# pqh22/ProxyTransformation

Hardware: AMD Instinct MI355X
Metric: scenes/sec (100k pts, 256 clusters, 64 proxies) (higher is better)
Workload: dtype f32; 1 GPU; cfg2: N=100000 pts, gs=8->M'=256 kept clusters, L=64 text + V=196 image proxies, d=256, eval forward; scenes_per_gpu=4, img_feat_dtype=bf16, input_sets_rotated=3, streams=1, lanes=1 (one forward at a time), setup_forwards=32

## Files before the change

include/proxyt.h:

```cpp
#ifndef PROXYT_H_
#define PROXYT_H_

#include <stddef.h>
#include <stdint.h>

#ifdef __cplusplus
extern "C" {
#endif

#define PTX_ABI_VERSION 13

#define PTX_API __attribute__((visibility("default")))

#define PTX_OK          0
#define PTX_EINVAL     -1
#define PTX_ELAUNCH    -2
#define PTX_ENOSPACE   -3
#define PTX_ETIMEOUT   -4
#define PTX_EGATE      -5

typedef struct PtxShape {
    int32_t B;
    int32_t N;
    int32_t grid_size;
// ... 14 lines not shown
    float   ln_eps;
} PtxShape;

typedef struct PtxSlotMlp {
    const float *conv_w;
    const float *conv_b;
    const float *bn_w, *bn_b, *bn_mean, *bn_var;
} PtxSlotMlp;

typedef struct PtxBlock {
    const float *norm1_w, *norm1_b;
    const float *pb_bias;
    const float *pc_bias;
    const float *pr_bias;
    const float *qkv_w;
    const float *qkv_b;
    const float *pp_w, *pp_b;
    const float *proj_w, *proj_b;
    const float *norm2_w, *norm2_b;
    const float *fc1_w, *fc1_b;
    const float *fc2_w, *fc2_b;
    const float *out_norm_w, *out_norm_b;
} PtxBlock;

typedef struct PtxBn1d { const float *w, *b, *mean, *var; } PtxBn1d;

typedef struct PtxWeights {
    PtxSlotMlp   offset;
    const float *offset_map_w;
    PtxSlotMlp   encoder;
    const float *cm_w, *cm_b;
    const float *pos;
    const float *q_w, *q_b, *k_w, *k_b, *v_w, *v_b, *c_w, *c_b;
    const float *norm_img_w, *norm_img_b;
    PtxBlock     text;
    PtxBlock     img;
    const float *text_trans_w, *text_trans_b;
    const float *img_trans_w, *img_trans_b;
    PtxBn1d      text_trans_norm, img_trans_norm;
} PtxWeights;

PTX_API int         ptx_abi_version(void);
PTX_API const char *ptx_last_error(void);

typedef struct PtxContext PtxContext;
PTX_API int ptx_context_create(PtxContext **ctx);
PTX_API int ptx_context_destroy(PtxContext *ctx);
PTX_API int ptx_context_check(PtxContext *ctx);
PTX_API int ptx_context_sync_check(PtxContext *ctx);
PTX_API int ptx_context_gates(const PtxContext *ctx);

PTX_API int         ptx_kernel_count(void);
PTX_API const char *ptx_kernel_name(int kid);
PTX_API int         ptx_timing_select(int kid);
PTX_API int         ptx_timing_read(int *launches, float *total_ms);
PTX_API int         ptx_timing_every(int n);
PTX_API int         ptx_timing_select_mask(uint64_t mask);
PTX_API int         ptx_timing_read_sites(int *launches, float *total_ms, int n);

PTX_API size_t ptx_prep_bytes(const PtxShape *s);
PTX_API size_t ptx_workspace_bytes(const PtxShape *s);

PTX_API int ptx_workspace_init(const PtxShape *s, void *workspace, size_t ws_bytes, void *stream);

PTX_API int ptx_prepare(const PtxShape *s, const PtxWeights *w, const float *lin,
                void *prep, size_t prep_bytes, void *stream);


PTX_API int ptx_grid_centers(const float *points, int B, int N, const float *lin, int gs, float margin,
                     float *minmax, float *centers, void *workspace, size_t ws_bytes, void *stream);

PTX_API int ptx_ball_query(const float *centers, const float *points, int B, int M, int N, int K,
                   float radius, int32_t *idx, float *cluster, int32_t *pad_count, void *stream);

PTX_API int ptx_linear(const float *x, const float *w, const float *bias, const float *residual, float *y,
               int rows, int n_out, int n_in, int gelu, void *stream);
PTX_API int ptx_linear_ln_partials(const float *x, const float *w, const float *bias, const float *residual, float *y, float *lnp,
               int rows, int n_out, int n_in, void *stream);
PTX_API size_t ptx_ln_linear_scratch_bytes(int n_out, int n_in);
PTX_API int ptx_ln_linear(const float *x, const float *lnp, const float *w, const float *gamma, const float *beta,
               const float *bias, float eps, int gelu, float *y, void *scratch, size_t scratch_bytes,
               int rows, int n_out, int n_in, void *stream);
PTX_API int ptx_gemm_policy(int min_tiles_128);

PTX_API int ptx_offset_net(const PtxShape *s, const PtxWeights *w, const void *prep,
                   const float *centers_in, const float *cluster, const float *minmax,
                   float *centers_out, float *offsets_out, void *stream);

PTX_API int ptx_select_clusters(const PtxShape *s, const int32_t *idx, const float *centers,
                        const float *cluster, const int32_t *pad_count,
                        const int32_t *order_override,
                        int32_t *order, int32_t *picks, int32_t *keep,
                        float *kcenter, float *kcluster, int32_t *kidx, int32_t *drop_idx,
                        uint32_t *tag, void *stream);

PTX_API int ptx_pointnet(const PtxShape *s, const PtxWeights *w, const void *prep, const float *kcenter,
                 const float *kcluster, float *point_proxy, void *stream);

PTX_API int ptx_img_proxy(const PtxShape *s, const PtxWeights *w, const void *prep, const void *img_feat,
                  float *img_proxy, void *workspace, size_t ws_bytes, void *stream);

PTX_API int ptx_proxy_block(const PtxShape *s, const PtxWeights *w, const void *prep, int which,
                    const float *point_proxy, const float *proxy, int Lp, const uint8_t *mask,
                    float *head_out, float *guide, void *workspace, size_t ws_bytes, void *stream);

PTX_API int ptx_affine_scatter(const PtxShape *s, const float *points, const uint32_t *tag,
                       const float *kcenter, const float *translate, const float *transform,
                       float *new_points, void *stream);

PTX_API int ptx_affine_compact(const PtxShape *s, const float *points, const uint32_t *tag,
                       const float *kcenter, const float *translate, const float *transform,
                       float *out, int32_t *counts, void *workspace, size_t ws_bytes, void *stream);

PTX_API size_t ptx_proxy_attention_scratch_bytes(int B, int n, int Lp, int heads, int C, int impl);
PTX_API int ptx_proxy_attention(const float *qkv, const float *pt, const uint8_t *mask, float *out, float *scratch, int B, int n,
                        int Lp, int heads, int C, int impl, void *stream);

typedef struct PtxDebug {
    float *centers0, *cluster1, *offsets, *centers, *cluster2;
    int32_t *idx2, *pad_count, *order, *picks, *keep, *kidx, *drop_idx;
    float *kcenter, *kcluster, *point_proxy, *img_proxy, *text_guide, *img_guide;
    float *translate, *transform;
    uint32_t *tag;
} PtxDebug;

PTX_API int ptx_forward(PtxContext *ctx, const PtxShape *s, const PtxWeights *w, const void *prep, const float *lin,
                const float *points, const float *const *points_list, const float *text_feats,
                const uint8_t *text_mask, const void *img_feat, const int32_t *order_override,
                const float *centers_override,
                float *out, int32_t *counts, void *workspace, size_t ws_bytes,
                const PtxDebug *debug, void *stream);

typedef struct PtxForwardOpts {
    const uint32_t *bbox_enc;
    int32_t compute_dtype;
    int32_t reserved[5];
} PtxForwardOpts;
PTX_API int ptx_forward_ex(PtxContext *ctx, const PtxShape *s, const PtxWeights *w, const void *prep, const float *lin,
                   const float *points, const float *const *points_list, const float *text_feats,
                   const uint8_t *text_mask, const void *img_feat, const int32_t *order_override,
                   const float *centers_override,
                   float *out, int32_t *counts, void *workspace, size_t ws_bytes,
                   const PtxDebug *debug, const PtxForwardOpts *opts, void *stream);

PTX_API int ptx_wait_counts(const int32_t *counts_host, int B, int64_t timeout_us);

PTX_API size_t ptx_ingest_workspace_bytes(int V, int H, int W);
PTX_API int ptx_ingest_index(const void *depth, int depth_dtype, int V, int H, int W, void *workspace, size_t ws_bytes,
                     int32_t *view_counts, void *stream);
PTX_API int ptx_ingest_gather(const void *depth, int depth_dtype, float depth_shift, int V, int H, int W, const float *inv_intrinsic,
                      const float *lu, const int32_t *piv, const int64_t *sel, int N, const float *aug, float *points,
                      uint32_t *bbox_enc, int32_t *status, const void *workspace, size_t ws_bytes, void *stream);

#define PTX_DRAW_EMPTY 1
#define PTX_DRAW_MAX_VIEWS 4096
PTX_API int ptx_ingest_draw(int V, int H, int W, int per_view, int N, uint64_t key, const void *workspace, size_t ws_bytes,
                    int64_t *sel, int32_t *status, void *stream);

#define PTX_VOX_BROKEN 0x7fffffff
PTX_API size_t ptx_voxel_workspace_bytes(int B, int Ncap);
PTX_API int ptx_voxelize(const float *points, const int32_t *counts, int B, int Ncap, float voxel_size, int32_t *coords,
                 float *feats, int32_t *inverse, int32_t *nvox_overflow, void *workspace, size_t ws_bytes, void *stream);
PTX_API int ptx_voxelize_ex(const float *points, const int32_t *counts, int B, int Ncap, float voxel_size, int32_t *coords,
                    float *feats, int32_t *inverse, int32_t *nvox_overflow, int32_t *scene_end, void *workspace, size_t ws_bytes,
                    void *stream);
PTX_API int ptx_voxelize_rep(const float *points, const int32_t *counts, int B, int Ncap, float voxel_size, int32_t *coords,
// ... 178 lines not shown
```

proxytransformation_amd/_abi.py:

```python
from __future__ import annotations

import ctypes as C
import os
from typing import Optional

_HERE = os.path.dirname(os.path.abspath(__file__))
LIB_PATH = os.path.join(_HERE, "libproxyt_hip.so")
ABI_VERSION = 13

c_float_p = C.c_void_p


class PtxShape(C.Structure):
    _fields_ = [(n, C.c_int32) for n in
                ("B", "N", "grid_size", "K", "Mt", "Mk", "L", "V", "C", "heads", "hidden",
                 "in_dim", "hw", "img_dtype")] + \
               [(n, C.c_float) for n in ("radius", "margin", "bn_eps", "ln_eps")]


class PtxSlotMlp(C.Structure):
    _fields_ = [(n, C.c_void_p) for n in ("conv_w", "conv_b", "bn_w", "bn_b", "bn_mean", "bn_var")]


class PtxBlock(C.Structure):
# ... 26 lines not shown
class PtxDebug(C.Structure):
    _fields_ = [(n, C.c_void_p) for n in DEBUG_FIELDS]


TB_PARAMS = ("ln1_w", "ln1_b", "pb", "pc", "pr", "qkv_w", "qkv_b", "pp_w", "pp_b", "proj_w", "proj_b", "ln2_w", "ln2_b",
             "fc1_w", "fc1_b", "fc2_w", "fc2_b", "ln3_w", "ln3_b", "head_w", "head_b", "bn_w", "bn_b")


class PtxTrainBlock(C.Structure):
    _fields_ = [(n, C.c_int32) for n in ("B", "n", "L", "C", "H", "heads", "s", "nout", "compute_dtype")] + \
               [(n, C.c_float) for n in ("eps1", "eps2", "eps3", "bn_eps", "bn_momentum", "p_attn", "p_drop", "p_path")] + \
               [("seed", C.c_uint64 * 6), ("x", C.c_void_p), ("proxy", C.c_void_p), ("mask", C.c_void_p),
                ("param", C.c_void_p * len(TB_PARAMS)), ("bn_run_mean", C.c_void_p), ("bn_run_var", C.c_void_p),
                ("out", C.c_void_p), ("save", C.c_void_p), ("save_floats", C.c_size_t), ("tmp", C.c_void_p),
                ("tmp_floats", C.c_size_t), ("dout", C.c_void_p), ("dx", C.c_void_p), ("dproxy", C.c_void_p),
                ("grad", C.c_void_p * len(TB_PARAMS)), ("dx_add", C.c_void_p)]


class PtxTrainImgPool(C.Structure):
    _fields_ = [(n, C.c_int32) for n in ("nimg", "Cin", "hw", "C", "heads", "img_dtype")] + \
               [(n, C.c_void_p) for n in ("img", "wc", "bc", "pos", "wq", "bq", "wk", "bk", "wv", "bv", "o", "save")] + \
               [("save_floats", C.c_size_t), ("tmp", C.c_void_p), ("tmp_floats", C.c_size_t)] + \
               [(n, C.c_void_p) for n in ("dout", "dimg", "dwc", "dbc", "dpos", "dwq", "dbq", "dwk", "dbk", "dwv", "dbv")] + \
               [(n, C.c_void_p) for n in ("cw", "cb", "lnw", "lnb")] + [("ln_eps", C.c_float)] + \
               [(n, C.c_void_p) for n in ("proxy", "dproxy", "dcw", "dcb", "dlnw", "dlnb")]


class PtxTrainSlotNet(C.Structure):
    _fields_ = [(n, C.c_void_p) for n in ("conv_w", "conv_b", "bn_w", "bn_b", "run_mean", "run_var")] + \
               [("eps", C.c_float), ("momentum", C.c_float), ("W", C.c_int32)]


TS_NGRAD = 9 + 13 + 2 * len(TB_PARAMS)
TS_IP0, TS_TB0, TS_IB0 = 9, 9 + 13, 9 + 13 + len(TB_PARAMS)


class PtxTrainStepLayout(C.Structure):
    _fields_ = [(n, C.c_size_t) for n in ("arena_fwd_bytes", "arena_bwd_bytes", "grads_floats", "idx2", "order", "picks", "keep", "kidx",
                                           "drop_idx", "centers", "translate", "transform", "point_proxy", "img_proxy", "kcenter",
                                           "opos")] + [("grad_off", C.c_int64 * TS_NGRAD)]


class PtxTrainStep(C.Structure):
    _fields_ = [("shape", PtxShape), ("points", C.c_void_p), ("lin", C.c_void_p), ("centers_override", C.c_void_p),
                ("order_override", C.c_void_p), ("text_feats", C.c_void_p), ("text_mask", C.c_void_p),
                ("off", PtxTrainSlotNet), ("enc", PtxTrainSlotNet), ("map_w", C.c_void_p),
                ("ip", PtxTrainImgPool), ("tb", PtxTrainBlock), ("ib", PtxTrainBlock),
                ("ws", C.c_void_p), ("ws_bytes", C.c_size_t), ("out", C.c_void_p), ("counts_host", C.c_void_p),
                ("arena_fwd", C.c_void_p), ("arena_fwd_bytes", C.c_size_t),
                ("side_stream", C.c_void_p), ("ev_fork", C.c_void_p), ("ev_join", C.c_void_p), ("ev_pp", C.c_void_p),
                ("ev_counts", C.c_void_p), ("blocks_apart", C.c_int32),
                ("douts", C.c_void_p), ("g_kcenter", C.c_void_p), ("g_translate", C.c_void_p), ("g_transform", C.c_void_p),
                ("arena_bwd", C.c_void_p), ("arena_bwd_bytes", C.c_size_t), ("grads", C.c_void_p), ("grads_floats", C.c_size_t),
                ("dtext", C.c_void_p), ("dimg", C.c_void_p)]


class PtxForwardOpts(C.Structure):
    _fields_ = [("bbox_enc", C.c_void_p), ("compute_dtype", C.c_int32), ("reserved", C.c_int32 * 5)]


_P, _I, _F, _Z = C.c_void_p, C.c_int, C.c_float, C.c_size_t
_SH, _W = C.POINTER(PtxShape), C.POINTER(PtxWeights)
SIGNATURES = {
    "ptx_abi_version": (C.c_int, []),
    "ptx_last_error": (C.c_char_p, []),
    "ptx_kernel_count": (C.c_int, []),
    "ptx_kernel_name": (C.c_char_p, [_I]),
    "ptx_timing_select": (_I, [_I]),
    "ptx_timing_every": (_I, [_I]),
    "ptx_timing_read": (_I, [C.POINTER(C.c_int), C.POINTER(C.c_float)]),
    "ptx_timing_select_mask": (_I, [C.c_uint64]),
    "ptx_timing_read_sites": (_I, [C.POINTER(C.c_int), C.POINTER(C.c_float), _I]),
    "ptx_prep_bytes": (_Z, [_SH]),
    "ptx_workspace_bytes": (_Z, [_SH]),
    "ptx_workspace_init": (_I, [_SH, _P, _Z, _P]),
    "ptx_prepare": (_I, [_SH, _W, _P, _P, _Z, _P]),
    "ptx_grid_centers": (_I, [_P, _I, _I, _P, _I, _F, _P, _P, _P, _Z, _P]),
    "ptx_ball_query": (_I, [_P, _P, _I, _I, _I, _I, _F, _P, _P, _P, _P]),
    "ptx_linear": (_I, [_P, _P, _P, _P, _P, _I, _I, _I, _I, _P]),
    "ptx_linear_ln_partials": (_I, [_P, _P, _P, _P, _P, _P, _I, _I, _I, _P]),
    "ptx_ln_linear_scratch_bytes": (_Z, [_I, _I]),
    "ptx_ln_linear": (_I, [_P, _P, _P, _P, _P, _P, _F, _I, _P, _P, _Z, _I, _I, _I, _P]),
    "ptx_gemm_policy": (_I, [_I]),
    "ptx_offset_net": (_I, [_SH, _W, _P, _P, _P, _P, _P, _P, _P]),
    "ptx_select_clusters": (_I, [_SH] + [_P] * 14),
    "ptx_pointnet": (_I, [_SH, _W, _P, _P, _P, _P, _P]),
    "ptx_img_proxy": (_I, [_SH, _W, _P, _P, _P, _P, _Z, _P]),
    "ptx_proxy_block": (_I, [_SH, _W, _P, _I, _P, _P, _I, _P, _P, _P, _P, _Z, _P]),
    "ptx_affine_scatter": (_I, [_SH, _P, _P, _P, _P, _P, _P, _P]),
    "ptx_affine_compact": (_I, [_SH, _P, _P, _P, _P, _P, _P, _P, _P, _Z, _P]),
    "ptx_wait_counts": (_I, [_P, _I, C.c_int64]),
    "ptx_context_create": (_I, [C.POINTER(C.c_void_p)]),
    "ptx_context_destroy": (_I, [_P]),
    "ptx_context_check": (_I, [_P]),
    "ptx_context_sync_check": (_I, [_P]),
    "ptx_context_gates": (_I, [_P]),
    "ptx_forward": (_I, [_P, _SH, _W, _P, _P, _P, _P, _P, _P, _P, _P, _P, _P, _P, _P, _Z,
                         C.POINTER(PtxDebug), _P]),
}

_L, _U64 = C.c_long, C.c_uint64
SIGNATURES.update({
    "ptx_forward_ex": (_I, [_P, _SH, _W, _P, _P, _P, _P, _P, _P, _P, _P, _P, _P, _P, _P, _Z,
                            C.POINTER(PtxDebug), C.POINTER(PtxForwardOpts), _P]),
    "ptx_proxy_attention": (_I, [_P, _P, _P, _P, _P, _I, _I, _I, _I, _I, _I, _P]),
    "ptx_proxy_attention_scratch_bytes": (_Z, [_I, _I, _I, _I, _I, _I]),
    "ptx_ingest_workspace_bytes": (_Z, [_I, _I, _I]),
    "ptx_ingest_index": (_I, [_P, _I, _I, _I, _I, _P, _Z, _P, _P]),
    "ptx_ingest_gather": (_I, [_P, _I, _F, _I, _I, _I, _P, _P, _P, _P, _I, _P, _P, _P, _P, _P, _Z, _P]),
    "ptx_ingest_draw": (_I, [_I, _I, _I, _I, _I, _U64, _P, _Z, _P, _P, _P]),
    "ptx_voxel_workspace_bytes": (_Z, [_I, _I]),
    "ptx_voxelize": (_I, [_P, _P, _I, _I, _F, _P, _P, _P, _P, _P, _Z, _P]),
    "ptx_voxelize_ex": (_I, [_P, _P, _I, _I, _F, _P, _P, _P, _P, _P, _P, _Z, _P]),
    "ptx_voxelize_rep": (_I, [_P, _P, _I, _I, _F, _P, _P, _P, _P, _P, _P, _P, _Z, _P]),
    "ptx_voxel_features_bwd": (_I, [_P, _I, _P, _P, _P, _I, _I, _P, _P]),
    "ptx_voxel_coarsen": (_I, [_P, _P, _I, _I, _F, _P, _P, _P, _P, _P, _Z, _P]),
    "ptx_point_sample_workspace_bytes": (_Z, [_I, _I, _I, _I]),
    "ptx_point_sample_prepare": (_I, [_P, _I, _I, _I, _I, _I, _P, _Z, _P]),
    "ptx_point_sample": (_I, [_P, _I, _P, _I, _I, _I, _I, _I, _P, _P, _F, _F, _F, _F, _I, _F, _F, _F, _I, _P, _P, _P, _Z, _P]),
    "ptx_point_sample_bwd_workspace_bytes": (_Z, [_I, _I, _I, _I, _I]),
    "ptx_point_sample_bwd": (_I, [_P, _I, _P, _P, _I, _I, _I, _I, _P, _P, _F, _F, _F, _F, _I, _F, _F, _F, _I, _P, _I, _P, _Z, _P]),
    "ptx_op_gemm": (_I, [_P, _P, _P, _I, _I, _I, _L, _L, _L, _L, _L, _L, _I, _I, _L, _L, _L, _L, _L, _L, _I, _I, _F, _I, _I, _L, _P]),
    "ptx_op_transpose": (_I, [_P, _I, _I, _P, _P]),
    "ptx_op_colsum": (_I, [_P, _P, _I, _I, _I, _F, _I, _P, _P, _I, _P]),
    "ptx_op_eltwise": (_I, [_I, _P, _P, _F, _L, _I, _P, _P]),
    "ptx_op_dropout": (_I, [_P, _L, _L, _F, _U64, _P, _P]),
    "ptx_op_layernorm_fwd": (_I, [_P, _P, _P, _P, _I, _I, _I, _F, _P, _P, _P]),
    "ptx_op_layernorm_bwd": (_I, [_P, _P, _P, _P, _I, _I, _P, _P, _P]),
    "ptx_op_bn_stats": (_I, [_P, _P, _I, _L, _F, _F, _P, _P, _P, _P]),
    "ptx_op_bn_apply": (_I, [_P, _P, _P, _P, _L, _I, _I, _P, _P]),
    "ptx_op_bn_bwd_prep": (_I, [_P, _P, _P, _P, _L, _I, _I, _P, _P, _P]),
    "ptx_op_bn_bwd_dx": (_I, [_P, _P, _P, _P, _P, _P, _L, _I, _P, _P]),
    "ptx_op_softmax_fwd": (_I, [_P, _P, _L, _I, _L, _P, _P]),
    "ptx_op_softmax_bwd": (_I, [_P, _P, _P, _L, _I, _L, _P, _P]),
    "ptx_op_slot_inputs": (_I, [_P, _P, _P, _L, _I, _P, _P, _P]),
    "ptx_op_slot_inputs_bwd": (_I, [_P, _P, _L, _I, _P, _P]),
    "ptx_op_slot_pool": (_I, [_P, _L, _I, _I, _I, _P, _P, _P]),
    "ptx_op_slot_pool_bwd": (_I, [_P, _P, _L, _I, _I, _I, _P, _P]),
    "ptx_op_slotnet_scratch_bytes": (_Z, [_I]),
    "ptx_op_slotnet_fwd": (_I, [_P, _P, _L, _I, _I, _P, _P, _P, _P, _F, _F, _P, _P, _I, _P, _P, _P, _P, _P, _Z, _P]),
    "ptx_op_slotnet_bwd": (_I, [_P, _P, _L, _I, _I, _P, _P, _P, _P, _P, _I, _P, _P, _P, _P, _P, _P, _P, _Z, _P]),
    "ptx_op_offset_apply": (_I, [_P, _P, _P, _L, _I, _F, _P, _P, _P]),
    "ptx_op_slotbias_fwd": (_I, [_P, _P, _P, _I, _I, _I, _P, _P]),
    "ptx_op_slotbias_bwd": (_I, [_P, _I, _I, _I, _P, _P, _P, _P]),
    "ptx_op_keep_rows": (_I, [_P, _P, _I, _I, _I, _I, _P, _P]),
    "ptx_op_rows_gather": (_I, [_P, _P, _L, _I, _P, _P]),
    "ptx_op_rows_scatter": (_I, [_P, _P, _L, _I, _P, _P]),
    "ptx_op_out_positions": (_I, [_P, _I, _I, _P, _P, _P, _P]),
    "ptx_op_affine_bwd": (_I, [_P, _P, _P, _P, _P, _P, _I, _I, _I, _I, _P, _P, _P, _P]),
    "ptx_op_affine_bwd_list": (_I, [_P, _P, _P, _P, _P, _P, _I, _I, _I, _I, _P, _P, _P, _P]),
    "ptx_op_tokens_finish": (_I, [_P, _P, _I, _I, _I, _P]),
    "ptx_op_tokens_finish_bwd": (_I, [_P, _I, _I, _I, _P]),
    "ptx_train_block_sizes": (_I, [C.POINTER(PtxTrainBlock), C.POINTER(_Z), C.POINTER(_Z), C.POINTER(_Z)]),
    "ptx_train_block_fwd": (_I, [C.POINTER(PtxTrainBlock), _P]),
    "ptx_train_block_bwd": (_I, [C.POINTER(PtxTrainBlock), _P]),
    "ptx_train_imgpool_sizes": (_I, [C.POINTER(PtxTrainImgPool), C.POINTER(_Z), C.POINTER(_Z), C.POINTER(_Z)]),
    "ptx_train_imgpool_fwd": (_I, [C.POINTER(PtxTrainImgPool), _P]),
    "ptx_train_imgpool_bwd": (_I, [C.POINTER(PtxTrainImgPool), _P]),
    "ptx_train_step_layout": (_I, [C.POINTER(PtxTrainStep), C.POINTER(PtxTrainStepLayout)]),
    "ptx_train_step_fwd": (_I, [C.POINTER(PtxTrainStep), _P]),
    "ptx_train_step_bwd": (_I, [C.POINTER(PtxTrainStep), _P]),
    "ptx_op_head_bwd_tmp_floats": (_Z, [_I, _I, _I]),
    "ptx_op_head_bwd": (_I, [_P, _P, _P, _P, _I, _I, _I, _P, _P, _P, _Z, _P]),
    "ptx_train_attn_tmp_floats": (_Z, [_I, _I, _I, _I, _I]),
    "ptx_train_attn_fwd": (_I, [_P, _P, _P, _I, _I, _I, _I, _I, _F, _U64, _P, _P, _P, _P, _P]),
    "ptx_train_attn_bwd": (_I, [_P, _P, _P, _I, _I, _I, _I, _I, _F, _U64, _P, _P, _P, _P, _P, _P, _P, _Z, _P]),
# ... 37 lines not shown
```

proxytransformation_amd/csrc/api.hip:

```cpp
#include <atomic>
#include <chrono>
#include <cmath>
#include <cstdlib>
#include <cstring>
#include <mutex>
#include <utility>
#include <vector>

#include "common.h"

namespace ptx {

static thread_local char g_err[512] = "";

void set_error(const char *fmt, ...)
{
    va_list ap;
    va_start(ap, fmt);
    vsnprintf(g_err, sizeof(g_err), fmt, ap);
    va_end(ap);
}

static const char *const kKernelNames[] = {
    "k_minmax", "k_cluster", "k_select", "k_tags",
// ... 306 lines not shown

template <typename T>
static inline T *at(void *base, size_t off) { return reinterpret_cast<T *>(static_cast<char *>(base) + off); }

__global__ void k_signal(uint32_t *flag, uint32_t seq)
{
    if (threadIdx.x == 0) __hip_atomic_store(flag, seq, __ATOMIC_RELAXED, __HIP_MEMORY_SCOPE_AGENT);
}
__global__ void k_gate(GateRef g)
{
    if (threadIdx.x == 0) gate_wait(g);
}

static GateRef gate_ref(const PtxContext *c, int word, uint32_t seq, uint32_t site, bool probe = false)
{
    const uint64_t ticks = probe ? c->probe_ticks : ((site == 2 || site == 7) ? 2 * c->gate_ticks : c->gate_ticks);
    return GateRef{c->gate + word, seq, c->gate_err, probe ? nullptr : c->gate + 48, ticks, site, probe ? 0 : c->gate_trap};
}

static int gate_check(PtxContext *c)
{
    if (c->gate_err == nullptr) return PTX_OK;
    const uint32_t e = *reinterpret_cast<volatile uint32_t *>(c->gate_err);
    if (e == 0u) return PTX_OK;
    static const char *const site_name[] = {"?", "fork (clustering stream waiting for the caller's stream)",
                                            "join (caller's stream waiting for the other chain)", "probe, fork direction",
                                            "probe, join direction", "?", "slot tags' fork (tag stream waiting for the selection)",
                                            "slot tags' join (caller's stream waiting for the tags)"};
    const unsigned site = (e >> 24) & 0x7fu;
    c->gates_on = false;
    *reinterpret_cast<volatile uint32_t *>(c->gate_err) = 0u;
    (void)hipStreamSynchronize(c->st);
    if (c->have_last) (void)hipStreamSynchronize(c->last_st);
    (void)hipMemset(c->gate + 48, 0, 4);
    set_error("stream gate timed out at the %s of forward #%u: the two chains of that forward were not ordered and its outputs "
              "were set to NaN; this context now orders its streams with events (PTX_GATE=0 selects them from the start)",
              site_name[site < 8 ? site : 0], e & 0xffffffu);
    return PTX_EGATE;
}

static int gate_probe_pair(PtxContext *c, hipStream_t waiter, hipStream_t releaser, int word, uint32_t site, bool *ok)
{
    const uint32_t seq = ++c->gate_seq;
    hipLaunchKernelGGL(k_gate, dim3(1), dim3(64), 0, waiter, gate_ref(c, word, seq, site, true));
    PTX_LAUNCHED("k_gate[probe]");
    hipLaunchKernelGGL(k_signal, dim3(1), dim3(64), 0, releaser, c->gate + word, seq);
    PTX_LAUNCHED("k_signal[probe]");
    PTX_HIP(hipStreamSynchronize(waiter));
    PTX_HIP(hipStreamSynchronize(releaser));
    *ok = *reinterpret_cast<volatile uint32_t *>(c->gate_err) == 0u;
    *reinterpret_cast<volatile uint32_t *>(c->gate_err) = 0u;
    return PTX_OK;
}
static int gate_probe(PtxContext *c, hipStream_t st)
{
    c->probed = true; c->probed_st = st; c->lo_ok = false;
    if (!c->gates_on) return PTX_OK;
    PTX_HIP(hipStreamSynchronize(st));
    PTX_HIP(hipStreamSynchronize(c->st));
    PTX_HIP(hipStreamSynchronize(c->lo));
    bool fork_ok = false, join_ok = false, t1 = false, t2 = false;
    PTX_TRY(gate_probe_pair(c, c->st, st, 40, 3, &fork_ok));
    PTX_TRY(gate_probe_pair(c, st, c->st, 44, 4, &join_ok));
    if (!fork_ok || !join_ok) { c->gates_on = false; return PTX_OK; }
    PTX_TRY(gate_probe_pair(c, c->lo, c->st, 40, 3, &t1));
    PTX_TRY(gate_probe_pair(c, st, c->lo, 44, 4, &t2));
    c->lo_ok = t1 && t2;
    return PTX_OK;
}

static int run_img_proxy(const PtxShape &s, const PtxWeights &w, const float *prep, const void *img,
                         float *img_proxy, void *ws, hipStream_t st, int phase = 0, bool need_ln = true,
                         int i0 = 0, int ni = -1, uint32_t *gate = nullptr, uint32_t gate_seq = 0)
{
    const PrepLayout P = prep_layout(s);
    const WsLayout L = ws_layout(s);
    const int C = s.C, hd = P.hd, nall = s.B * s.V, nimg = ni < 0 ? nall : ni;
    float *fm = at<float>(ws, L.fm) + (size_t)i0 * s.in_dim, *qkv0 = at<float>(ws, L.qkv0) + (size_t)i0 * 3 * C;
    float *we = at<float>(ws, L.we) + (size_t)i0 * s.heads * P.KT1, *gbuf = at<float>(ws, L.gbuf) + (size_t)i0 * s.heads * P.KT2p;
    float *obuf = at<float>(ws, L.obuf) + (size_t)i0 * C, *cbuf = at<float>(ws, L.cbuf) + (size_t)i0 * C;
    if (img_proxy) img_proxy += (size_t)i0 * C;
    const int dt = s.img_dtype;
    img = static_cast<const char *>(img) + (size_t)i0 * s.in_dim * s.hw * (dt == 0 ? 4 : 2);
    float *Gs = nullptr, *E = nullptr, *ML = nullptr;
    const int EW = P.KT2p - s.in_dim;
    const bool pooled32 = img_pool32_supported(dt, s.in_dim, s.hw, s.heads);
    const bool pooled = pooled32 || img_pool_supported(dt, s.in_dim, s.hw, s.heads);
    if (pooled) {
        img_pool_layout(at<float>(ws, L.pool), nall, s.in_dim, EW, &Gs, &E, &ML);
        Gs += (size_t)i0 * 2 * s.heads * s.in_dim; E += (size_t)i0 * s.heads * EW; ML += (size_t)i0 * s.heads * 5;
    }
    if (phase != 2) PTX_TIMED(KID_IMG_MEAN, st, launch_img_mean(img, dt, nimg, s.in_dim, s.hw, fm, st, gate, gate_seq));
    if (phase == 1) return PTX_OK;
    const bool chained = hd == 32 && nimg < 4096;
    {
        GemmBatch g{}; g.n = 1;
        g.p[0] = GemmProb{fm, prep + P.w3, qkv0, prep + P.b3, nullptr, nullptr, nullptr,
                          nimg, 3 * C, s.in_dim, s.in_dim, s.in_dim, 3 * C, 0, 0, 0, EPI_NONE};
        if (chained) {
            g.p[0].w2 = prep + P.t1; g.p[0].c2 = we; g.p[0].n2 = P.KT1; g.p[0].ldc2 = s.heads * P.KT1;
            g.p[0].chain_tiles = s.heads; g.p[0].w2_stride = (long)P.KT1 * hd; g.p[0].c2_stride = P.KT1;
        }
        PTX_TIMED(KID_IMG_QKV0, st, launch_gemm(g, st));
    }
    if (!chained) {
        for (int h0 = 0; h0 < s.heads; h0 += kMaxGroups) {
            GemmBatch g{}; g.n = std::min(kMaxGroups, s.heads - h0);
            for (int h = h0; h < h0 + g.n; ++h)
                g.p[h - h0] = GemmProb{qkv0 + h * hd, prep + P.t1 + (size_t)h * P.KT1 * hd, we + (size_t)h * P.KT1,
                                       nullptr, nullptr, nullptr, nullptr, nimg, P.KT1, hd, 3 * C, hd,
                                       s.heads * P.KT1, 0, 0, 0, EPI_NONE};
            PTX_TIMED(KID_IMG_WE, st, launch_gemm(g, st));
        }
    }
    if (pooled32) {
        PTX_TIMED_EXT(KID_IMG_SCORES, st, launch_img_pool32(static_cast<const float *>(img), we, qkv0, nimg, s.in_dim, s.hw, C, P.KT1, EW,
                                                        attn_scale(hd), Gs, E, ML, st));
    } else if (pooled) {
        PTX_TIMED_EXT(KID_IMG_SCORES, st, launch_img_pool(img, dt, we, qkv0, nimg, s.in_dim, s.hw, C, P.KT1,
                                                      EW, attn_scale(hd), Gs, E, ML, st));
    } else {
        PTX_TIMED(KID_IMG_SCORES, st, launch_img_scores(img, dt, we, qkv0, nimg, s.in_dim, s.hw, s.heads, C, P.KT1,
                                                        P.KT2p, attn_scale(hd), gbuf, st));
        PTX_TIMED(KID_IMG_GATHER, st, launch_img_gather(img, dt, nimg, s.in_dim, s.hw, s.heads, P.KT2p, gbuf, st));
    }
    for (int h0 = 0; h0 < s.heads; h0 += kMaxGroups) {
        GemmBatch g{}; g.n = std::min(kMaxGroups, s.heads - h0);
        for (int h = h0; h < h0 + g.n; ++h) {
            GemmProb &gp = g.p[h - h0];
            gp = GemmProb{gbuf + (size_t)h * P.KT2p, prep + P.t2 + (size_t)h * hd * P.KT2p, obuf + h * hd,
                          w.v_b + h * hd, nullptr, gbuf + (size_t)h * P.KT2p + s.in_dim,
                          qkv0 + 2 * C + h * hd, nimg, hd, P.KT2p, s.heads * P.KT2p, P.KT2p, C,
                          0, s.heads * P.KT2p, 3 * C, EPI_NONE};
            if (pooled) {
                gp.A = nullptr; gp.rs = nullptr;
                gp.pg = Gs + (size_t)h * s.in_dim; gp.ldg = 2 * s.heads * s.in_dim; gp.gslab = s.heads * s.in_dim;
                gp.pe = E + (size_t)h * EW; gp.lde = s.heads * EW;
                gp.pml = ML + (size_t)h * 5; gp.ldml = s.heads * 5;
                gp.kg = s.in_dim;
            }
        }
        PTX_TIMED(KID_IMG_O, st, launch_gemm(g, st));
    }
    {
        GemmBatch g{}; g.n = 1;
        g.p[0] = GemmProb{obuf, w.c_w, cbuf, w.c_b, nullptr, nullptr, nullptr,
                          nimg, C, C, C, C, C, 0, 0, 0, EPI_NONE};
        g.p[0].lnp_out = at<float>(ws, L.lnp_img) + (size_t)i0 * (C / 32) * 2;
        PTX_TIMED(KID_IMG_C, st, launch_gemm(g, st));
    }
    if (need_ln) {
        LnBatch lb{}; lb.n = 1; lb.C = C; lb.eps = s.ln_eps;
        lb.p[0] = LnProb{cbuf, img_proxy, w.norm_img_w, w.norm_img_b, nullptr, nimg, 1};
        PTX_TIMED(KID_IMG_LN, st, launch_ln_rows(lb, st));
    }
    return PTX_OK;
}

struct Branch {
    const PtxBlock *blk; const float *x_in; const float *proxy; int Lp; const uint8_t *mask;
    const float *head_w, *head_b, *head_ab; int nout; float *head_out; float *guide; int slot;
    bool late_proxy;
    const float *proxy_lnp, *pp_gw, *pp_gc;
    const float *fc1_gw, *fc1_gc;
    const float *prep;
};

static bool fused_attn_pays(const PtxShape &s, const Branch *br, int nb)
{
    (void)br;
    const long wgs = (long)s.B * s.heads * nb;
    return s.Mk <= 256 || wgs >= 96;
}

static int run_blocks(const PtxShape &s, const Branch *br, int nb, const float *point_proxy, void *ws,
                      hipStream_t st, int phase = 0, int cd = 0, GateRef *join = nullptr, GateRef *tags_join = nullptr,
                      bool skip_qkv = false)
{
    const WsLayout L = ws_layout(s);
    const int C = s.C, R = s.B * s.Mk;
    {
        GemmBatch g{}; g.n = 0;
        for (int i = 0; i < nb; ++i) {
            const int sl = br[i].slot;
            if (phase != 2 && phase != 3 && phase != 4 && !skip_qkv)
                g.p[g.n++] = GemmProb{br[i].x_in, br[i].blk->qkv_w, at<float>(ws, L.qkv[sl]), br[i].blk->qkv_b,
                                      nullptr, nullptr, nullptr, R, 3 * C, C, C, C, 3 * C, 0, 0, 0, EPI_NONE};
            const bool now = phase == 0 || (phase == 1 && !br[i].late_proxy) || ((phase == 2 || phase == 3) && br[i].late_proxy);
            if (now && phase != 4) {
                GemmProb &q = g.p[g.n++];
                q = GemmProb{br[i].proxy, br[i].blk->pp_w, at<float>(ws, L.pt[sl]), br[i].blk->pp_b,
                             nullptr, nullptr, nullptr, s.B * br[i].Lp, C, C, C, C, C, 0, 0, 0, EPI_NONE};
                if (br[i].proxy_lnp != nullptr) {
                    q.W = br[i].pp_gw; q.bias = nullptr;
                    q.lnp_in = br[i].proxy_lnp; q.ln_c = br[i].pp_gc;
                    q.ln_parts = C / 32; q.ln_C = C; q.ln_eps = s.ln_eps;
                }
            }
        }
        if (g.n > 0 && (phase == 2 || phase == 1) && join != nullptr && join->flag != nullptr) { g.tail_gate = *join; join->flag = nullptr; }
        if (g.n > 0) PTX_TIMED(phase == 2 || phase == 3 ? KID_BLK_PP : KID_BLK_QKV, st, launch_gemm(g, st, cd));
        if (phase == 1 || phase == 3) return PTX_OK;
    }
    FAttnBatch fa{}; fa.nb = nb; fa.B = s.B; fa.heads = s.heads; fa.hd = C / s.heads; fa.n = s.Mk; fa.C = C;
    fa.scale = attn_scale(C / s.heads); fa.compute_dtype = cd;
    fa.split = fattn_split_for(s.B, s.heads); fa.part = at<float>(ws, L.fa_part); fa.tickets = at<int>(ws, L.fa_ticket);
    for (int i = 0; i < nb; ++i) {
        const int sl = br[i].slot;
        fa.p[i] = FAttnProb{at<float>(ws, L.qkv[sl]), at<float>(ws, L.pt[sl]), br[i].mask, at<float>(ws, L.ao[sl]), br[i].Lp};
    }
    const bool fused = fused_attn_supported(fa) && (cd == 1 || fused_attn_pays(s, br, nb));
    if (fused) PTX_TIMED(KID_BLK_ATTN_F, st, launch_proxy_attn(fa, st));
    AttnBatch a{}; a.n = nb; a.B = s.B; a.heads = s.heads; a.hd = C / s.heads; a.scale = attn_scale(C / s.heads);
    for (int i = 0; i < nb && !fused; ++i) {
        const int sl = br[i].slot;
        float *qkv = at<float>(ws, L.qkv[sl]);
        a.p[i] = AttnProb{at<float>(ws, L.pt[sl]), qkv + C, qkv + 2 * C, at<float>(ws, L.pv[sl]), nullptr,
                          br[i].Lp, s.Mk, C, 3 * C, 3 * C, C,
                          (long)br[i].Lp * C, (long)s.Mk * 3 * C, (long)s.Mk * 3 * C, (long)br[i].Lp * C};
    }
    if (!fused) PTX_TIMED(KID_BLK_ATTN_A, st, launch_attn32(a, st));
    for (int i = 0; i < nb && !fused; ++i) {
// ... 245 lines not shown
                void *stream)
{
    (void)lin;
    PTX_REQUIRE(s && w && prep, "ptx_prepare: null argument");
    PTX_TRY(validate_shape(*s));
    if (prep_bytes < prep_layout(*s).total * sizeof(float)) { set_error("prep buffer too small"); return PTX_ENOSPACE; }
    return run_prepare(*s, *w, static_cast<float *>(prep), static_cast<hipStream_t>(stream));
}

int ptx_grid_centers(const float *points, int B, int N, const float *lin, int gs, float margin,
                     float *minmax, float *centers, void *workspace, size_t ws_bytes, void *stream)
{
    PTX_REQUIRE(points && lin && minmax && centers && workspace, "ptx_grid_centers: null argument");
    PTX_REQUIRE(ws_bytes >= (size_t)B * 6 * 4, "ptx_grid_centers: workspace needs %d bytes", B * 24);
    hipStream_t st = static_cast<hipStream_t>(stream);
    uint32_t *enc = static_cast<uint32_t *>(workspace);
    PTX_HIP(hipMemsetAsync(enc, 0, (size_t)B * 6 * 4, st));
    ScenePts sp;
    PTX_TRY(make_scene_pts(points, nullptr, B, N, &sp));
    PTX_TRY(launch_minmax(sp, B, N, enc, st));
    return launch_ball_query(nullptr, enc, lin, gs, margin, minmax, centers, sp, B, gs * gs * gs, N, 0,
                             0.0f, nullptr, nullptr, nullptr, st);
}

int ptx_ball_query(const float *centers, const float *points, int B, int M, int N, int K, float radius,
                   int32_t *idx, float *cluster, int32_t *pad_count, void *stream)
{
    PTX_REQUIRE(centers && points && idx && cluster, "ptx_ball_query: null argument");
    PTX_REQUIRE(B >= 1 && M >= 1 && N >= 1 && K >= 1, "ptx_ball_query: B=%d M=%d N=%d K=%d", B, M, N, K);
    ScenePts sp;
    PTX_TRY(make_scene_pts(points, nullptr, B, N, &sp));
    return launch_ball_query(centers, nullptr, nullptr, 0, 0.0f, nullptr, nullptr, sp, B, M, N, K, radius,
                             idx, cluster, pad_count, static_cast<hipStream_t>(stream));
}

int ptx_linear(const float *x, const float *w, const float *bias, const float *residual, float *y,
               int rows, int n_out, int n_in, int gelu, void *stream)
{
    PTX_REQUIRE(x && w && y, "ptx_linear: null argument");
    PTX_REQUIRE(rows >= 1 && n_out >= 1 && n_in >= 4, "ptx_linear: rows=%d n_out=%d n_in=%d", rows, n_out, n_in);
    GemmBatch g{}; g.n = 1;
    g.p[0] = GemmProb{x, w, y, bias, residual, nullptr, nullptr, rows, n_out, n_in, n_in, n_in, n_out, n_out, 0, 0,
                      gelu ? EPI_GELU : EPI_NONE};
    return launch_gemm(g, static_cast<hipStream_t>(stream));
}

int ptx_linear_ln_partials(const float *x, const float *w, const float *bias, const float *residual, float *y, float *lnp,
                           int rows, int n_out, int n_in, void *stream)
{
    PTX_REQUIRE(x && w && y && lnp, "ptx_linear_ln_partials: null argument");
    PTX_REQUIRE(rows >= 1 && n_out >= 1 && n_in >= 4, "ptx_linear_ln_partials: rows=%d n_out=%d n_in=%d", rows, n_out, n_in);
    GemmBatch g{}; g.n = 1;
    g.p[0] = GemmProb{x, w, y, bias, residual, nullptr, nullptr, rows, n_out, n_in, n_in, n_in, n_out, n_out, 0, 0, EPI_NONE};
    g.p[0].lnp_out = lnp;
    return launch_gemm(g, static_cast<hipStream_t>(stream));
}

size_t ptx_ln_linear_scratch_bytes(int n_out, int n_in)
{
    return n_out >= 1 && n_in >= 1 ? ((size_t)n_out * n_in + (size_t)n_out) * sizeof(float) : 0;
}

int ptx_ln_linear(const float *x, const float *lnp, const float *w, const float *gamma, const float *beta, const float *bias,
                  float eps, int gelu, float *y, void *scratch, size_t scratch_bytes, int rows, int n_out, int n_in, void *stream)
{
    PTX_REQUIRE(x && lnp && w && gamma && beta && y && scratch, "ptx_ln_linear: null argument");
    PTX_REQUIRE(rows >= 1 && n_out >= 1, "ptx_ln_linear: rows=%d n_out=%d", rows, n_out);
    PTX_REQUIRE(n_in >= 32 && n_in % 32 == 0 && n_in <= 512, "ptx_ln_linear: n_in=%d must be a multiple of 32, at most 512", n_in);
    PTX_REQUIRE(eps > 0.0f, "ptx_ln_linear: eps=%g", (double)eps);
    PTX_REQUIRE((reinterpret_cast<uintptr_t>(scratch) & 15) == 0 && scratch_bytes >= ptx_ln_linear_scratch_bytes(n_out, n_in),
                "ptx_ln_linear: scratch of %zu bytes (16-byte aligned) needed", ptx_ln_linear_scratch_bytes(n_out, n_in));
    hipStream_t st = static_cast<hipStream_t>(stream);
    float *wg = static_cast<float *>(scratch), *cv = wg + (size_t)n_out * n_in;
    PTX_TRY(launch_prep_lnfold(w, gamma, beta, bias, n_out, n_in, wg, cv, st));
    GemmBatch g{}; g.n = 1;
    g.p[0] = GemmProb{x, wg, y, nullptr, nullptr, nullptr, nullptr, rows, n_out, n_in, n_in, n_in, n_out, 0, 0, 0,
                      gelu ? EPI_GELU : EPI_NONE};
    g.p[0].lnp_in = lnp; g.p[0].ln_c = cv;
    g.p[0].ln_parts = n_in / 32; g.p[0].ln_C = n_in; g.p[0].ln_eps = eps;
    return launch_gemm(g, st);
}

int ptx_gemm_policy(int min_tiles_128) { return gemm_policy(min_tiles_128); }

int ptx_offset_net(const PtxShape *s, const PtxWeights *w, const void *prep, const float *centers_in,
                   const float *cluster, const float *minmax, float *centers_out, float *offsets_out,
                   void *stream)
{
    PTX_REQUIRE(s && w && prep && centers_in && cluster && minmax && centers_out, "ptx_offset_net: null argument");
    PTX_TRY(validate_shape(*s));
    const PrepLayout P = prep_layout(*s);
    const int M = s->grid_size * s->grid_size * s->grid_size;
    return launch_offset_net(static_cast<const float *>(prep) + P.off_ab, w->offset, w->offset_map_w, centers_in,
                             cluster, minmax, s->B * M, M, s->K, s->margin, centers_out, offsets_out,
                             static_cast<hipStream_t>(stream));
}

int ptx_select_clusters(const PtxShape *s, const int32_t *idx, const float *centers, const float *cluster,
                        const int32_t *pad_count, const int32_t *order_override, int32_t *order,
                        int32_t *picks, int32_t *keep, float *kcenter, float *kcluster, int32_t *kidx,
                        int32_t *drop_idx, uint32_t *tag, void *stream)
{
    PTX_REQUIRE(s && idx && centers && cluster && pad_count && order && picks && keep && kcenter && kcluster &&
                kidx && drop_idx, "ptx_select_clusters: null argument");
    PTX_TRY(validate_shape(*s));
    return launch_select(*s, idx, centers, cluster, pad_count, order_override, order, picks, keep, kcenter,
                         kcluster, kidx, drop_idx, tag, static_cast<hipStream_t>(stream));
}

int ptx_pointnet(const PtxShape *s, const PtxWeights *w, const void *prep, const float *kcenter,
                 const float *kcluster, float *point_proxy, void *stream)
{
    PTX_REQUIRE(s && w && prep && kcenter && kcluster && point_proxy, "ptx_pointnet: null argument");
    PTX_TRY(validate_shape(*s));
    const PrepLayout P = prep_layout(*s);
    return launch_pointnet(static_cast<const float *>(prep) + P.enc_ab, w->encoder, kcenter, kcluster,
                           s->B * s->Mk, s->Mk, s->K, s->C, point_proxy, nullptr, nullptr, nullptr, nullptr, nullptr,
                           nullptr, s->ln_eps, nullptr, 0, static_cast<hipStream_t>(stream));
}

int ptx_img_proxy(const PtxShape *s, const PtxWeights *w, const void *prep, const void *img_feat,
                  float *img_proxy, void *workspace, size_t ws_bytes, void *stream)
{
    PTX_REQUIRE(w && prep && img_feat && img_proxy, "ptx_img_proxy: null argument");
    PTX_TRY(check_bufs(s, workspace, ws_bytes));
    return run_img_proxy(*s, *w, static_cast<const float *>(prep), img_feat, img_proxy, workspace,
                         static_cast<hipStream_t>(stream));
}

int ptx_proxy_block(const PtxShape *s, const PtxWeights *w, const void *prep, int which,
                    const float *point_proxy, const float *proxy, int Lp, const uint8_t *mask,
                    float *head_out, float *guide, void *workspace, size_t ws_bytes, void *stream)
{
    PTX_REQUIRE(w && prep && point_proxy && proxy && head_out, "ptx_proxy_block: null argument");
    PTX_REQUIRE(which == 0 || which == 1, "ptx_proxy_block: which=%d", which);
    PTX_TRY(check_bufs(s, workspace, ws_bytes));
    PTX_REQUIRE(Lp >= 1 && Lp <= (s->L > s->V ? s->L : s->V), "ptx_proxy_block: Lp=%d exceeds max(L,V)", Lp);
    hipStream_t st = static_cast<hipStream_t>(stream);
    const PrepLayout P = prep_layout(*s);
    const WsLayout L = ws_layout(*s);
    const float *pf = static_cast<const float *>(prep);
    const PtxBlock &blk = which == 0 ? w->text : w->img;
    float *x_in = at<float>(workspace, L.x_in[which]);
    LnBatch lb{}; lb.n = 1; lb.C = s->C; lb.eps = s->ln_eps;
    lb.p[0] = LnProb{point_proxy, x_in, blk.norm1_w, blk.norm1_b, pf + (which == 0 ? P.posb_t : P.posb_i),
                     s->B * s->Mk, s->Mk};
    PTX_TRY(launch_ln_rows(lb, st));
    Branch br = make_branch(*s, *w, pf, which, x_in, proxy, Lp, mask, head_out, guide);
    return run_blocks(*s, &br, 1, point_proxy, workspace, st);
}

size_t ptx_proxy_attention_scratch_bytes(int B, int n, int Lp, int heads, int C, int impl)
{
    if (B < 1 || n < 1 || Lp < 1 || heads < 1 || C < heads) return 0;
    if (impl == 3) return 256 + (size_t)B * heads * 4 + (size_t)B * heads * kFaMaxSplit * n * kFaPartRow * sizeof(float);
    return (size_t)B * Lp * C * sizeof(float);
}

int ptx_proxy_attention(const float *qkv, const float *pt, const uint8_t *mask, float *out, float *scratch, int B, int n,
                        int Lp, int heads, int C, int impl, void *stream)
{
    PTX_REQUIRE(qkv && pt && out, "ptx_proxy_attention: null argument");
    PTX_REQUIRE(B >= 1 && n >= 1 && Lp >= 1 && heads >= 1 && C >= heads && C % heads == 0, "ptx_proxy_attention: B=%d n=%d Lp=%d heads=%d C=%d", B, n, Lp, heads, C);
    PTX_REQUIRE(impl >= 0 && impl <= 3, "ptx_proxy_attention: impl=%d", impl);
    hipStream_t st = static_cast<hipStream_t>(stream);
    const int hd = C / heads;
// ... 108 lines not shown
        PTX_HIP(hipEventRecord(side->fork, st));
        PTX_HIP(hipStreamWaitEvent(side->st, side->fork, 0));
    }
    float *img_proxy = at<float>(ws, L.img_proxy);
#ifdef PTX_TEST_HOOKS
    static const char *const fault = getenv("PTX_GATE_FAULT");
#else
    constexpr const char *fault = nullptr;
#endif
    const bool fault_fork = gated && fault && fault[0] == 'f', fault_join = gated && fault && fault[0] == 'j';
    auto launch_gate = [&](int kid, hipStream_t s_, const GateRef &g) -> int {
        hipLaunchKernelGGL(k_gate, dim3(1), dim3(64), 0, s_, g);
        PTX_LAUNCHED("k_gate");
        (void)kid;
        return PTX_OK;
    };
    if (gated) {
        const uint32_t seq = ++side->gate_seq;
        PTX_TRY(run_img_proxy(S, *w, pf, img_feat, img_proxy, ws, is, 1, true, 0, -1, fault_fork ? nullptr : side->gate, seq));
        PTX_TIMED(KID_GATE_FORK, cs, launch_gate(KID_GATE_FORK, cs, gate_ref(side, 0, seq, 1)));
    } else
    if (!img_late) PTX_TRY(run_img_proxy(S, *w, pf, img_feat, img_proxy, ws, is, 1));

    uint32_t *mm_ws = at<uint32_t>(ws, L.mm_enc), *tag = at<uint32_t>(ws, L.tag);
    const uint32_t *mm_enc = bbox_in ? bbox_in : mm_ws;
    const bool dbg = debug != nullptr;
    float *centers0 = dbg && debug->centers0 ? at<float>(ws, L.centers0) : nullptr;
    float *cluster1 = dbg && debug->cluster1 ? at<float>(ws, L.cluster1) : nullptr;
    float *offsets = dbg && debug->offsets ? at<float>(ws, L.offsets) : nullptr;
    float *centers = at<float>(ws, L.centers), *cluster2 = at<float>(ws, L.cluster2);
    int32_t *idx2 = at<int32_t>(ws, L.idx2), *pad_count = at<int32_t>(ws, L.pad_count);
    if (!bbox_in) PTX_TIMED(KID_MINMAX, cs, launch_minmax(sp, B, S.N, mm_ws, cs));
    const bool early = lc.early;
    const bool fork_ext = !capturing && (img_late || early);
    const bool cgate = cluster_on_caller && side->gates_on && side->lo_ok && !capturing;
    if (cgate) ++side->gate_seq;
    const bool fault_cjoin = cgate && fault && fault[0] == 'j', fault_ctags = cgate && fault && fault[0] == 't';
    const bool cg_join_select = cgate && early;
    const bool cg_join_qkv = cgate && !early;
    GateRef cjoin = (cg_join_select || cg_join_qkv) ? gate_ref(side, 52, side->gate_seq, 2) : GateRef{};
    PTX_TIMED(KID_CLUSTER, cs, launch_cluster(S, mm_enc, lin, sp, pf + P.off_ab, w->offset, w->offset_map_w,
                                              centers_override, nullptr, centers0, cluster1, offsets, centers, idx2,
                                              cluster2, pad_count, cs, fork_ext ? side->early_a : nullptr));

    if (img_late) {
        if (!fork_ext) PTX_HIP(hipEventRecord(side->fork, st));
        PTX_HIP(hipStreamWaitEvent(side->st, fork_ext ? side->early_a : side->fork, 0));
        PTX_TRY(run_img_proxy(S, *w, pf, img_feat, img_proxy, ws, is, 1));
    }
    float *point_proxy = at<float>(ws, L.point_proxy);
    float *xin_t = at<float>(ws, L.x_in[0]), *xin_i = at<float>(ws, L.x_in[1]);
    float *translate = at<float>(ws, L.head[0]), *transform = at<float>(ws, L.head[1]);
    float *guide_t = (debug && debug->text_guide) ? at<float>(ws, L.guide[0]) : nullptr;
    float *guide_i = (debug && debug->img_guide) ? at<float>(ws, L.guide[1]) : nullptr;
    Branch br[2] = {make_branch(S, *w, pf, 0, xin_t, text_feats, S.L, text_mask, translate, guide_t),
                    make_branch(S, *w, pf, 1, xin_i, at<float>(ws, L.cbuf), S.V, nullptr, transform, guide_i)};
    br[1].proxy_lnp = at<float>(ws, L.lnp_img);
    if (early) {
        if (!fork_ext) PTX_HIP(hipEventRecord(side->early_a, cs));
        PTX_HIP(hipStreamWaitEvent(side->lo, side->early_a, 0));
        float *pp_all = at<float>(ws, L.pp_all), *xa_t = at<float>(ws, L.xln_all[0]), *xa_i = at<float>(ws, L.xln_all[1]);
        int32_t *order_e = at<int32_t>(ws, L.order_e);
        PTX_TRY(launch_order(S, pad_count, order_override, order_e, side->lo));
        PTX_TRY(launch_pointnet(pf + P.enc_ab, w->encoder, centers, cluster2, B * S.Mt, S.Mt, K, S.C, pp_all, &w->text, &w->img, nullptr,
                                nullptr, xa_t, xa_i, S.ln_eps, order_e, M, side->lo, nullptr, 0, true));
        GemmBatch g{}; g.n = 2;
        g.p[0] = GemmProb{xa_t, w->text.qkv_w, at<float>(ws, L.g_all[0]), nullptr, nullptr, nullptr, nullptr, B * S.Mt, 3 * S.C, S.C, S.C, S.C,
                          3 * S.C, 0, 0, 0, EPI_NONE};
        g.p[1] = GemmProb{xa_i, w->img.qkv_w, at<float>(ws, L.g_all[1]), nullptr, nullptr, nullptr, nullptr, B * S.Mt, 3 * S.C, S.C, S.C, S.C,
                          3 * S.C, 0, 0, 0, EPI_NONE};
        PTX_TRY(launch_gemm(g, side->lo, compute_dtype));
        PTX_TRY(run_blocks(S, br, 2, point_proxy, ws, side->lo, 1, compute_dtype, nullptr, nullptr, true));
    }

    int32_t *order = at<int32_t>(ws, L.order), *picks = at<int32_t>(ws, L.picks), *keep = at<int32_t>(ws, L.keep);
    float *kcenter = at<float>(ws, L.kcenter);
    float *kcluster = dbg && debug->kcluster ? at<float>(ws, L.kcluster) : nullptr;
    int32_t *kidx = dbg && debug->kidx ? at<int32_t>(ws, L.kidx) : nullptr;
    int32_t *drop_idx = dbg && debug->drop_idx ? at<int32_t>(ws, L.drop_idx) : nullptr;
    int32_t *ksrc = at<int32_t>(ws, L.ksrc);
    const bool ext_event = !capturing;
    const bool tags_gated = gated && side->lo_ok && (lf.v[3] >= 0 ? lf.v[3] != 0 : est_image < 1.6 * est_cluster);
    const bool tags_tail = !cluster_on_caller && !tags_gated;
    PTX_TIMED(KID_SELECT, cs, launch_select_order(S, centers, pad_count, order_override, order, picks, keep, kcenter,
                                                  ksrc, bbox_in ? nullptr : mm_ws, cs, cluster_on_caller, ext_event && !tags_tail ? side->aux : nullptr,
                                                  cg_join_select ? &cjoin : nullptr));
    int32_t *tile_counts = at<int32_t>(ws, L.tile_counts);
    hipStream_t ts = tags_tail ? cs : side->lo;
    const bool slots_first = !cluster_on_caller && !tags_tail;
    auto enqueue_tags = [&]() -> int {
        if (tags_gated) {
            PTX_TIMED(KID_GATE_TAGS, ts, launch_gate(KID_GATE_TAGS, ts, gate_ref(side, 36, side->gate_seq, 6)));
        } else if (!tags_tail) {
            if (!ext_event) PTX_HIP(hipEventRecord(side->aux, cs));
            PTX_HIP(hipStreamWaitEvent(ts, side->aux, 0));
        }
        if (kcluster || kidx || drop_idx)
            PTX_TRY(launch_select_slots(S, idx2, cluster2, order, picks, keep, kcluster, kidx, drop_idx, nullptr, ts));
        PTX_TIMED(KID_TAGS, ts, launch_tags(S, idx2, order, picks, ksrc, tag, tile_counts, counts, at<int32_t>(ws, L.scene_acc), ts));
        if (tags_gated) {
            auto sig = [&]() -> int {
                hipLaunchKernelGGL(k_signal, dim3(1), dim3(64), 0, ts, side->gate + 38, side->gate_seq);
                PTX_LAUNCHED("k_signal[tags]");
                return PTX_OK;
            };
            PTX_TIMED(KID_SIGNAL_TAGS, ts, sig());
        } else if (cgate) {
            if (!fault_ctags) {
                hipLaunchKernelGGL(k_signal, dim3(1), dim3(64), 0, ts, side->gate + 56, side->gate_seq);
                PTX_LAUNCHED("k_signal[ctags]");
            }
        } else if (!tags_tail) PTX_HIP(hipEventRecord(side->tags, ts));
        return PTX_OK;
    };
    if (slots_first) PTX_TRY(enqueue_tags());

    const bool want_img_proxy = debug != nullptr && debug->img_proxy != nullptr;
    PTX_TRY(run_img_proxy(S, *w, pf, img_feat, img_proxy, ws, is, 2, want_img_proxy));

    bool joined_early = false;
    if (early) {
        const float *const gsrc[2] = {at<float>(ws, L.g_all[0]), at<float>(ws, L.g_all[1])};
        const float *const tb[2] = {pf + P.qkvb[0], pf + P.qkvb[1]};
        float *const qk[2] = {at<float>(ws, L.qkv[0]), at<float>(ws, L.qkv[1])};
        {
            PTX_TRY(run_blocks(S, br, 2, point_proxy, ws, is, 3, compute_dtype));
            PTX_HIP(hipEventRecord(side->join, is));
            PTX_HIP(hipStreamWaitEvent(side->lo, side->join, 0));
            joined_early = true;
        }
        if (cg_join_select) {
            if (!fault_cjoin) {
                hipLaunchKernelGGL(k_signal, dim3(1), dim3(64), 0, side->lo, side->gate + 52, side->gate_seq);
                PTX_LAUNCHED("k_signal[cjoin]");
            }
        } else {
            PTX_HIP(hipEventRecord(side->early_b, side->lo));
            PTX_HIP(hipStreamWaitEvent(cs, side->early_b, 0));
        }
        PTX_TIMED(KID_POINTNET, cs, launch_qkv_gather(at<float>(ws, L.pp_all), gsrc, tb, keep, B, S.Mt, S.Mk, S.C, point_proxy, qk, cs));
    } else
    PTX_TIMED(KID_POINTNET, cs, launch_pointnet(pf + P.enc_ab, w->encoder, kcenter, cluster2, B * S.Mk, S.Mk, K,
                                                S.C, point_proxy, &w->text, &w->img, pf + P.posb_t, pf + P.posb_i, xin_t,
                                                xin_i, S.ln_eps, ksrc, M, cs, tags_gated ? side->gate + 36 : nullptr, side->gate_seq));
    if (!slots_first && !tags_tail) PTX_TRY(enqueue_tags());

    if (!early) PTX_TRY(run_blocks(S, br, 2, point_proxy, ws, cs, 1, compute_dtype, cg_join_qkv ? &cjoin : nullptr));
    if (cg_join_qkv && cjoin.flag != nullptr) {
        set_error("ptx_forward: the join gate was not attached to the qkv launch");
        return PTX_ELAUNCH;
    }
    if (tags_tail) PTX_TRY(enqueue_tags());
    const bool pp_early = cluster_on_caller;
    GateRef join{};
    if (gated) {
        auto launch_signal = [&]() -> int {
            hipLaunchKernelGGL(k_signal, dim3(1), dim3(64), 0, cs, side->gate + 32, side->gate_seq);
            PTX_LAUNCHED("k_signal");
            return PTX_OK;
        };
        if (!fault_join) PTX_TIMED(KID_SIGNAL_JOIN, cs, launch_signal());
        join = gate_ref(side, 32, side->gate_seq, 2);
    } else {
    if (!cluster_on_caller) PTX_HIP(hipEventRecord(side->join, cs));
    if (pp_early && !joined_early) PTX_TRY(run_blocks(S, br, 2, point_proxy, ws, is, 3, compute_dtype));
    if (cg_join_qkv) {
        if (!fault_cjoin) {
            hipLaunchKernelGGL(k_signal, dim3(1), dim3(64), 0, is, side->gate + 52, side->gate_seq);
// ... 50 lines not shown
```

proxytransformation_amd/csrc/cluster.hip:

```cpp
#include <cstdlib>
#include <hip/hip_ext.h>

#include "common.h"

namespace ptx {

__global__ __launch_bounds__(256) void k_minmax(ScenePts points, int N,
                                                uint32_t *__restrict__ mm_enc)
{
    __shared__ float red[4][6];
    minmax_block<false>(points.p[blockIdx.y], N, mm_enc, blockIdx.y, blockIdx.x, gridDim.x, red);
}

int launch_minmax(const ScenePts &points, int B, int N, uint32_t *mm_enc, hipStream_t st)
{
    hipLaunchKernelGGL(k_minmax, dim3(minmax_chunks(N), B), dim3(256), 0, st, points, N, mm_enc);
    PTX_LAUNCHED("k_minmax");
    return PTX_OK;
}

constexpr int kBqUnroll = 4;

__device__ __forceinline__ void grid_centre(const uint32_t *__restrict__ mm_enc, const float *__restrict__ lin, int gs,
                                            float margin, int b, int m, float (&mn)[3], float (&mx)[3], float (&c)[3])
{
#pragma unroll
    for (int d = 0; d < 3; ++d) { mn[d] = ord2f(~mm_enc[b * 6 + d]); mx[d] = ord2f(mm_enc[b * 6 + 3 + d]); }
    const int ijk[3] = {m / (gs * gs), (m / gs) % gs, m % gs};
    const float two_margin = __fmul_rn(2.0f, margin);
#pragma unroll
    for (int d = 0; d < 3; ++d) {
        const float base = __fadd_rn(mn[d], margin);
        const float span = __fsub_rn(__fsub_rn(mx[d], mn[d]), two_margin);
        c[d] = __fadd_rn(base, __fmul_rn(lin[ijk[d]], span));
    }
}

constexpr int kBqPrivate = 4096;
constexpr int kBqTile = 512;
constexpr int kBqTileFloats = kBqTile * 3;

struct BqHits { int32_t *oi; float *oc; int K; int count; unsigned long long lt; };

__device__ __forceinline__ void bq_group(BqHits &h, int j, bool valid, float px, float py, float pz, float cx, float cy, float cz,
                                         float r2)
{
    const float d2 = dist2_nofma(cx, cy, cz, px, py, pz);
    const bool hit = valid && (d2 < r2);
    const unsigned long long mask = __ballot(hit);
    const int pos = h.count + __popcll(mask & h.lt);
    if (hit && pos < h.K) {
        if (h.oi) h.oi[pos] = j;
        h.oc[pos * 3] = px; h.oc[pos * 3 + 1] = py; h.oc[pos * 3 + 2] = pz;
    }
    h.count += __popcll(mask);
}

__device__ __forceinline__ int bq_scan(const float *__restrict__ p, int N, int K, float cx, float cy, float cz, float r2,
                                       int32_t *oi, float *oc, float *tiles = nullptr)
{
    const int lane = lane_id();
    BqHits h{oi, oc, K, 0, (1ull << lane) - 1ull};
    int n1 = N;
    if (tiles != nullptr) {
        const int start = kBqPrivate + (int)((reinterpret_cast<uintptr_t>(p) >> 2) & 3u);
        n1 = min(N, start);
    }
    for (int base = 0; base < n1 && h.count < K; base += 64 * kBqUnroll) {
        float px[kBqUnroll], py[kBqUnroll], pz[kBqUnroll];
#pragma unroll
        for (int u = 0; u < kBqUnroll; ++u) {
            const int j = base + u * 64 + lane;
            if (j < n1) { px[u] = p[(size_t)j * 3]; py[u] = p[(size_t)j * 3 + 1]; pz[u] = p[(size_t)j * 3 + 2]; }
            else        { px[u] = py[u] = pz[u] = 0.0f; }
        }
#pragma unroll
        for (int u = 0; u < kBqUnroll; ++u) {
            if (h.count < K) {
                const int j = base + u * 64 + lane;
                bq_group(h, j, j < n1, px[u], py[u], pz[u], cx, cy, cz, r2);
            }
        }
// ... 572 lines not shown
    for (int k = tid; k < Kd; k += T) {
        const int pk = k < kn ? s_picks[k] : -1;
        a.picks[(size_t)b * Kd + k] = pk;
        if (pk >= 0) s_flag[pk] = 1;
    }
    __syncthreads();

    if (wid == 0) {
        const unsigned long long lt = (1ull << lane) - 1ull;
        int n = 0;
        for (int t0 = 0; t0 < Mt && n < Mk; t0 += 64) {
            const int t = t0 + lane;
            const bool kp = t < Mt && s_flag[t] == 0;
            const unsigned long long mask = __ballot(kp);
            const int pos = n + __popcll(mask & lt);
            if (kp && pos < Mk) s_keep[pos] = t;
            n += __popcll(mask);
        }
    }
    __syncthreads();

    if (a.mm_clear != nullptr && tid < 6) a.mm_clear[b * 6 + tid] = 0u;
    for (int j = tid; j < Mk; j += T) {
        const int t = s_keep[j];
        a.keep[(size_t)b * Mk + j] = t;
        if (a.ksrc != nullptr) a.ksrc[(size_t)b * Mk + j] = s_order[t];
        a.kcenter[((size_t)b * Mk + j) * 3] = sx[t];
        a.kcenter[((size_t)b * Mk + j) * 3 + 1] = sy[t];
        a.kcenter[((size_t)b * Mk + j) * 3 + 2] = sz[t];
    }
    if (a.tail.flag != nullptr && b == 0 && tid == 0) gate_wait(a.tail);
}

__global__ __launch_bounds__(256) void k_select_slots(SelectArgs a)
{
    const int b = blockIdx.y;
    const int M = a.M, K = a.K, Mt = a.Mt, Mk = a.Mk, Kd = a.Kd;
    const int e = blockIdx.x * 256 + threadIdx.x;
    const int kn = Kd < Mt ? Kd : Mt;
    uint32_t *tag = a.tag ? a.tag + (size_t)b * a.N : nullptr;
    const int32_t *order = a.order + (size_t)b * Mt;
    if (e < Mk * K) {
        const int j = e / K, k = e - j * K;
        const int src = order[a.keep[(size_t)b * Mk + j]];
        const int id = a.idx[((size_t)b * M + src) * K + k];
        if (a.kidx) a.kidx[(size_t)b * Mk * K + e] = id;
        if (a.kcluster) {
            const float *cp = a.cluster + (((size_t)b * M + src) * K + k) * 3;
            float *op = a.kcluster + ((size_t)b * Mk * K + e) * 3;
            op[0] = cp[0]; op[1] = cp[1]; op[2] = cp[2];
        }
        if (tag && id >= 0) {
            const uint32_t v = (uint32_t)(e + 1);
            const uint32_t old = atomicMax(&tag[id], v);
            if (old & 0x80000000u) atomicMax(&tag[id], 0x80000000u | v);
        }
    } else if (e < (Mk + Kd) * K) {
        const int ed = e - Mk * K;
        const int kk = ed / K, k = ed - kk * K;
        const int pk = kk < kn ? a.picks[(size_t)b * Kd + kk] : -1;
        int id = -1;
        if (pk >= 0) id = a.idx[((size_t)b * M + order[pk]) * K + k];
        if (a.drop_idx) a.drop_idx[(size_t)b * Kd * K + ed] = id;
        if (tag && id >= 0) atomicOr(&tag[id], 0x80000000u);
    }
}

static size_t select_lds_bytes(const PtxShape &s)
{
    const int Kd = s.Mt - s.Mk;
    return sizeof(int) * ((size_t)s.Mt * 5 + s.Mk + (Kd > 0 ? Kd : 1) + 64 + 16 + 16);
}

static SelectArgs select_args(const PtxShape &s, const int32_t *idx, const float *centers, const float *cluster,
                              const int32_t *pad_count, const int32_t *order_override, int32_t *order,
                              int32_t *picks, int32_t *keep, float *kcenter, float *kcluster, int32_t *kidx,
                              int32_t *drop_idx, uint32_t *tag, uint32_t *mm_clear)
{
    return SelectArgs{idx, centers, cluster, pad_count, order_override, order, picks, keep, kcenter,
                      kcluster, kidx, drop_idx, tag, s.grid_size * s.grid_size * s.grid_size, s.K, s.Mt,
                      s.Mk, s.Mt - s.Mk, s.N, nullptr, mm_clear, GateRef{}};
}

int launch_select_order(const PtxShape &s, const float *centers, const int32_t *pad_count,
                        const int32_t *order_override, int32_t *order, int32_t *picks, int32_t *keep,
                        float *kcenter, int32_t *ksrc, uint32_t *mm_clear, hipStream_t st, bool critical,
                        hipEvent_t done, const GateRef *tail)
{
    SelectArgs a = select_args(s, nullptr, centers, nullptr, pad_count, order_override, order, picks, keep, kcenter,
                               nullptr, nullptr, nullptr, nullptr, mm_clear);
    a.ksrc = ksrc;
    if (tail != nullptr) a.tail = *tail;
    size_t lds = select_lds_bytes(s);
    PTX_REQUIRE(lds <= 160 * 1024, "select: Mt=%d needs %zu B of LDS (> 160 KiB)", s.Mt, lds);
    const bool alone = critical;
    if (alone && s.B <= 32 && lds < 150 * 1024) lds = 150 * 1024;
    const bool one = critical && s.Mt <= 384;
    const int per = cdiv(s.Mt, one ? 64 : 256);
    const dim3 grid(s.B), block(256);
#define PTX_SEL(P_)                                                                          \
    do {                                                                                     \
        if (lds > 64 * 1024) {                                                               \
            PTX_HIP(hipFuncSetAttribute(reinterpret_cast<const void *>(&k_select<P_, false>), \
                                        hipFuncAttributeMaxDynamicSharedMemorySize, (int)lds)); \
            if (one && P_ <= 6)                                                              \
                PTX_HIP(hipFuncSetAttribute(reinterpret_cast<const void *>(&k_select<(P_ <= 6 ? P_ : 1), true>), \
                                            hipFuncAttributeMaxDynamicSharedMemorySize, (int)lds)); \
        }                                                                                    \
         \
        if (one && P_ <= 6) hipExtLaunchKernelGGL((k_select<(P_ <= 6 ? P_ : 1), true>), grid, block, lds, st, nullptr, done, 0, a); \
        else hipExtLaunchKernelGGL((k_select<P_, false>), grid, block, lds, st, nullptr, done, 0, a); \
    } while (0)
    if (per <= 1) PTX_SEL(1);
    else if (per <= 2) PTX_SEL(2);
    else if (per <= 3) PTX_SEL(3);
    else if (per <= 4) PTX_SEL(4);
    else if (per <= 5) PTX_SEL(5);
    else if (per <= 6) PTX_SEL(6);
    else if (per <= 8) PTX_SEL(8);
    else if (per <= 12) PTX_SEL(12);
    else if (per <= 16) PTX_SEL(16);
    else { set_error("select: Mt=%d too large (max %d)", s.Mt, 256 * 16); return PTX_EINVAL; }
#undef PTX_SEL
    PTX_LAUNCHED("k_select");
    return PTX_OK;
}

int launch_select_slots(const PtxShape &s, const int32_t *idx, const float *cluster, const int32_t *order,
                        const int32_t *picks, const int32_t *keep, float *kcluster, int32_t *kidx,
                        int32_t *drop_idx, uint32_t *tag, hipStream_t st)
{
    SelectArgs a = select_args(s, idx, nullptr, cluster, nullptr, nullptr, const_cast<int32_t *>(order),
                               const_cast<int32_t *>(picks), const_cast<int32_t *>(keep), nullptr, kcluster, kidx,
                               drop_idx, tag, nullptr);
    hipLaunchKernelGGL(k_select_slots, dim3(cdiv(s.Mt * s.K, 256), s.B), dim3(256), 0, st, a);
    PTX_LAUNCHED("k_select_slots");
    return PTX_OK;
}

int launch_select(const PtxShape &s, const int32_t *idx, const float *centers, const float *cluster,
                  const int32_t *pad_count, const int32_t *order_override, int32_t *order,
                  int32_t *picks, int32_t *keep, float *kcenter, float *kcluster, int32_t *kidx,
                  int32_t *drop_idx, uint32_t *tag, hipStream_t st)
{
    PTX_TRY(launch_select_order(s, centers, pad_count, order_override, order, picks, keep, kcenter, nullptr, nullptr, st, true, nullptr));
    PTX_TRY(launch_select_slots(s, idx, cluster, order, picks, keep, kcluster, kidx, drop_idx, nullptr, st));
    if (tag == nullptr) return PTX_OK;
    return launch_tags(s, idx, order, picks, nullptr, tag, nullptr, nullptr, nullptr, st, keep);
}

__global__ __launch_bounds__(256) void k_tile_count(const uint32_t *__restrict__ tag, int N,
                                                    int32_t *__restrict__ tile_counts, int32_t *scene_acc,
                                                    int32_t *counts)
{
    const int b = blockIdx.y, tile = blockIdx.x;
    const uint32_t *tg = tag + (size_t)b * N;
    int c = 0;
#pragma unroll
    for (int r = 0; r < kTilePts / 256; ++r) {
        const int n = tile * kTilePts + r * 256 + threadIdx.x;
        if (n < N) c += (tg[n] >> 31) == 0;
    }
    c = wave_sum(c);
    __shared__ int red[4];
    if (lane_id() == 0) red[threadIdx.x >> 6] = c;
    __syncthreads();
    if (threadIdx.x == 0) {
        const int total = red[0] + red[1] + red[2] + red[3];
        tile_counts[b * gridDim.x + tile] = total;
        if (scene_acc != nullptr) {
            __hip_atomic_fetch_add(scene_acc + 2 * b, total, __ATOMIC_RELAXED, __HIP_MEMORY_SCOPE_AGENT);
            const int ticket = __hip_atomic_fetch_add(scene_acc + 2 * b + 1, 1, __ATOMIC_ACQ_REL, __HIP_MEMORY_SCOPE_AGENT);
            if (ticket == (int)gridDim.x - 1) {
                const int sum = __hip_atomic_exchange(scene_acc + 2 * b, 0, __ATOMIC_ACQUIRE, __HIP_MEMORY_SCOPE_AGENT);
                __hip_atomic_store(scene_acc + 2 * b + 1, 0, __ATOMIC_RELAXED, __HIP_MEMORY_SCOPE_AGENT);
                __hip_atomic_store(counts + b, sum, __ATOMIC_RELEASE, __HIP_MEMORY_SCOPE_SYSTEM);
            }
        }
    }
}

struct TagArgs {
    const int32_t *idx, *order, *picks, *ksrc;
    const int32_t *keep;
    uint32_t *tag; int32_t *tile_counts, *scene_acc, *counts;
    int M, K, Mt, Mk, Kd, N, ntiles;
};

template <int TILES>
__global__ __launch_bounds__(1024) void k_tags(TagArgs a)
{
    constexpr int kTagRange = TILES * kTilePts;
    extern __shared__ __attribute__((aligned(16))) uint32_t s_tag[];
    int *s_cnt = reinterpret_cast<int *>(s_tag + kTagRange);
    const int b = blockIdx.y, base = blockIdx.x * kTagRange, tid = threadIdx.x;
    const int M = a.M, K = a.K, Mt = a.Mt, Mk = a.Mk, Kd = a.Kd;
    const int kn = Kd < Mt ? Kd : Mt;
    for (int i = tid * 4; i < kTagRange; i += 1024 * 4) *reinterpret_cast<uint4 *>(s_tag + i) = make_uint4(0u, 0u, 0u, 0u);
    if (tid < TILES) s_cnt[tid] = 0;
    __syncthreads();
    const int32_t *idx = a.idx + (size_t)b * M * K;
    const int32_t *order = a.order + (size_t)b * Mt;
    for (int e0 = tid; e0 < Mk * K; e0 += 4 * 1024) {
        int id[4];
#pragma unroll
        for (int u = 0; u < 4; ++u) {
            const int e = e0 + u * 1024;
            const int ec = min(e, Mk * K - 1), j = ec / K, k = ec - j * K;
            const int src = a.ksrc != nullptr ? a.ksrc[(size_t)b * Mk + j] : order[a.keep[(size_t)b * Mk + j]];
            id[u] = e < Mk * K ? idx[(size_t)src * K + k] : -1;
        }
#pragma unroll
        for (int u = 0; u < 4; ++u) {
            const unsigned r = (unsigned)(id[u] - base);
            if (r < (unsigned)kTagRange) atomicMax(&s_tag[r], (uint32_t)(e0 + u * 1024 + 1));
        }
    }
    __syncthreads();
    for (int e0 = tid; e0 < Kd * K; e0 += 4 * 1024) {
        int id[4];
#pragma unroll
        for (int u = 0; u < 4; ++u) {
            const int ed = e0 + u * 1024;
            const int ec = min(ed, Kd * K - 1), kk = ec / K, k = ec - kk * K;
            const int pk = (ed < Kd * K && kk < kn) ? a.picks[(size_t)b * Kd + kk] : -1;
            id[u] = pk >= 0 ? idx[(size_t)order[pk] * K + k] : -1;
        }
#pragma unroll
// ... 254 lines not shown
```

proxytransformation_amd/csrc/common.h:

```cpp
#pragma once
#include <hip/hip_runtime.h>
#include <cstdarg>
#include <cstdint>
#include <cstdio>

#include "../../include/proxyt.h"

namespace ptx {

void set_error(const char *fmt, ...);
bool timing_ext_take(hipEvent_t *start, hipEvent_t *stop);

#define PTX_REQUIRE(cond, ...)                                   \
    do {                                                         \
        if (!(cond)) {                                           \
            ::ptx::set_error(__VA_ARGS__);                       \
            return PTX_EINVAL;                                   \
        }                                                        \
    } while (0)

#define PTX_HIP(expr)                                                              \
    do {                                                                           \
        hipError_t e_ = (expr);                                                    \
        if (e_ != hipSuccess) {                                                    \
// ... 132 lines not shown
            for (int d = 0; d < 3; ++d) {
                float v = p[(size_t)i * 3 + d];
                lo[d] = fminf(lo[d], v); hi[d] = fmaxf(hi[d], v);
            }
        }
    }
#pragma unroll
    for (int d = 0; d < 3; ++d) { lo[d] = wave_min(lo[d]); hi[d] = wave_max(hi[d]); }
    const int w = threadIdx.x >> 6;
    if (lane_id() == 0) {
#pragma unroll
        for (int d = 0; d < 3; ++d) { red[w][d] = lo[d]; red[w][3 + d] = hi[d]; }
    }
    __syncthreads();
    if (threadIdx.x < 6) {
        const int d = threadIdx.x;
        float v = red[0][d];
        for (int i = 1; i < 4; ++i) v = d < 3 ? fminf(v, red[i][d]) : fmaxf(v, red[i][d]);
        uint32_t old = 0u;
        if (d < 3) { if (v != INFINITY) old = atomicMax(&mm_enc[b * 6 + d], ~f2ord(v)); }
        else       { if (v != -INFINITY) old = atomicMax(&mm_enc[b * 6 + d], f2ord(v)); }
        if (WAIT) asm volatile("" :: "v"(old));
    }
}
inline int minmax_chunks(int N) { int c = (N + 256 * 16 - 1) / (256 * 16); return c < 1 ? 1 : (c > 256 ? 256 : c); }

__device__ __forceinline__ void mean_prologue(uint32_t *gate, uint32_t gate_seq)
{
    if (gate != nullptr && blockIdx.x == 0 && threadIdx.x == 0) __hip_atomic_store(gate, gate_seq, __ATOMIC_RELAXED, __HIP_MEMORY_SCOPE_AGENT);
}

struct PrepLayout {
    size_t off_ab, enc_ab;
    size_t ttn_ab, itn_ab;
    size_t posb_t, posb_i;
    size_t w3, b3;
    size_t t1;
    size_t t2;
    size_t ppg_w, ppg_c;
    size_t fc1g_w[2], fc1g_c[2];
    size_t mlp_w1p[2], mlp_w2p[2];
    size_t qkvb[2];
    size_t total;
    int KT1, KT2p, hd;
};
PrepLayout prep_layout(const PtxShape &s);

struct WsLayout {
    size_t zero_begin, zero_bytes;
    size_t mm_enc;
    size_t scene_acc;
    size_t tag;
    size_t fa_ticket;
    size_t mlp_ticket;
    size_t mm_ticket;
    size_t minmax, centers0, cluster1, offsets, centers, idx2, cluster2, pad_count;
    size_t order, picks, keep, ksrc, kcenter, kcluster, kidx, drop_idx, tile_counts;
    size_t point_proxy, x_in[2];
    size_t pp_all, xln_all[2], g_all[2];
    size_t order_e;
    size_t fm, qkv0, we, pool, gbuf, obuf, cbuf, img_proxy;
    size_t qkv[2], pt[2], pv[2], ao[2], x1[2], xn2[2], hbuf[2], x2[2], guide[2], head[2];
    size_t lnp_img, lnp_x1[2];
    size_t fa_part;
    size_t mlp_part;
    size_t total;
};
WsLayout ws_layout(const PtxShape &s);

int validate_shape(const PtxShape &s);

enum : int { EPI_NONE = 0, EPI_GELU = 1 };
struct GemmProb {
    const float *A; const float *W; float *C;
    const float *bias;
    const float *res;
    const float *rs;
    const float *ad;
    int R, N, K, lda, ldw, ldc, ldres, rs_stride, ldad, epi;
    const float *pg, *pe, *pml; int ldg, gslab, lde, ldml, kg;
    float *lnp_out;
    const float *lnp_in, *ln_c; int ln_parts, ln_C; float ln_eps;
    const float *w2; float *c2; int n2, ldc2, chain_tiles; long w2_stride, c2_stride;
};
constexpr int kMaxGroups = 8;
struct GemmBatch {
    GemmProb p[kMaxGroups]; int n; int rotate;
    GateRef tail_gate;
};
int launch_gemm(const GemmBatch &gb, hipStream_t st, int compute_dtype = 0);
int gemm_policy(int min_tiles_128);

struct LnProb { const float *x; float *y; const float *w; const float *b; const float *add; int R, add_rows; };
struct LnBatch { LnProb p[2]; int n; int C; float eps; };
int launch_ln_rows(const LnBatch &lb, hipStream_t st);

struct HeadProb {
    const float *x; const float *nw; const float *nb;
    const float *hw; const float *hb;
    const float *ab;
    float *out; float *guide; int R, nout;
};
struct HeadBatch { HeadProb p[2]; int n; int C; float eps; };
int launch_heads(const HeadBatch &hb, hipStream_t st);

struct AttnProb {
    const float *Q, *K, *V; float *O; const uint8_t *mask;
    int nq, nk, ldq, ldk, ldv, ldo;
    long sQ, sK, sV, sO;
};
struct AttnBatch { AttnProb p[2]; int n; int B, heads, hd; float scale; };
int launch_attn32(const AttnBatch &ab, hipStream_t st);

struct FAttnProb { const float *qkv, *pt; const uint8_t *mask; float *out; int Lp; };
struct FAttnBatch {
    FAttnProb p[2]; int nb, B, heads, hd, n, C; float scale; int compute_dtype;
    int split; float *part; int *tickets;
};
int fattn_split_for(int B, int heads);
constexpr int kFaMaxSplit = 4, kFaPartRow = 34;
bool fused_attn_supported(const FAttnBatch &ab);
int launch_proxy_attn(const FAttnBatch &ab, hipStream_t st);

struct MlpProb {
    const float *x1, *lnp;
    const void *w1p, *w2p;
    const float *fc1_c, *b2;
    float *x2; int R;
    const float *nw, *nb, *hw, *hb, *ab; float *head_out, *guide; int nout;
};
struct MlpBatch { MlpProb p[2]; int n; float ln_eps; float *part; int *tickets; int compute_dtype; };
bool mlp_fused_supported(int C, int hidden, int R, int compute_dtype);
size_t mlp_part_bytes(int R);
size_t mlp_ticket_bytes(int R);
int launch_mlp(const MlpBatch &mb, hipStream_t st);
int launch_prep_planes(const float *W, int rows, int K, void *out, hipStream_t st);
int launch_prep_lnfold(const float *W, const float *gamma, const float *beta, const float *bias, int N, int K, float *Wg,
                       float *cv, hipStream_t st);

int make_scene_pts(const float *stacked, const float *const *list, int B, int N, ScenePts *out);

int launch_minmax(const ScenePts &points, int B, int N, uint32_t *mm_enc, hipStream_t st);
int launch_ball_query(const float *centers, const uint32_t *mm_enc, const float *lin, int gs,
                      float margin, float *minmax_out, float *centers_out, const ScenePts &points,
                      int B, int M, int N, int K, float radius, int32_t *idx, float *cluster,
                      int32_t *pad_count, hipStream_t st);
int launch_offset_net(const float *ab, const PtxSlotMlp &mlp, const float *map_w,
                      const float *centers_in, const float *cluster, const float *minmax,
                      int BM, int M, int K, float margin, float *centers_out, float *offsets_out,
                      hipStream_t st);
int launch_pointnet(const float *ab, const PtxSlotMlp &mlp, const float *kcenter,
                    const float *kcluster, int BM, int Mk, int K, int width, float *point_proxy,
                    const PtxBlock *blk_t, const PtxBlock *blk_i, const float *posb_t,
                    const float *posb_i, float *xin_t, float *xin_i, float ln_eps,
                    const int32_t *ksrc, int Msrc, hipStream_t st, uint32_t *head_flag = nullptr, uint32_t head_seq = 0,
                    bool center_src = false);
int launch_order(const PtxShape &s, const int32_t *pad_count, const int32_t *order_override, int32_t *order, hipStream_t st);
int launch_qkv_gather(const float *pp_all, const float *const g[2], const float *const tb[2], const int32_t *ksrc, int B, int M, int Mk,
                      int C, float *point_proxy, float *const qkv[2], hipStream_t st);
int launch_cluster(const PtxShape &s, const uint32_t *mm_enc, const float *lin, const ScenePts &points,
                   const float *off_ab, const PtxSlotMlp &mlp, const float *map_w, const float *centers_override,
                   float *minmax_out, float *centers0, float *cluster1, float *offsets, float *centers,
                   int32_t *idx2, float *cluster2, int32_t *pad_count, hipStream_t st, hipEvent_t done = nullptr);
int launch_select(const PtxShape &s, const int32_t *idx, const float *centers, const float *cluster,
                  const int32_t *pad_count, const int32_t *order_override, int32_t *order,
                  int32_t *picks, int32_t *keep, float *kcenter, float *kcluster, int32_t *kidx,
                  int32_t *drop_idx, uint32_t *tag, hipStream_t st);
int launch_select_order(const PtxShape &s, const float *centers, const int32_t *pad_count,
                        const int32_t *order_override, int32_t *order, int32_t *picks, int32_t *keep,
                        float *kcenter, int32_t *ksrc, uint32_t *mm_clear, hipStream_t st, bool critical,
                        hipEvent_t done, const GateRef *tail = nullptr);
int launch_tags(const PtxShape &s, const int32_t *idx, const int32_t *order, const int32_t *picks, const int32_t *ksrc,
                uint32_t *tag, int32_t *tile_counts, int32_t *counts, int32_t *scene_acc, hipStream_t st,
                const int32_t *keep = nullptr);
int launch_select_slots(const PtxShape &s, const int32_t *idx, const float *cluster, const int32_t *order,
                        const int32_t *picks, const int32_t *keep, float *kcluster, int32_t *kidx,
                        int32_t *drop_idx, uint32_t *tag, hipStream_t st);
int launch_t_ln_fwd(const float *x, const float *w, const float *b, int R, int C, float eps, float *y, float *stats, hipStream_t st);
int t_ln_chunks(int R);
int launch_t_ln_bwd(const float *x, const float *stats, const float *w, const float *dy, int R, int C, float *dx, float *part, hipStream_t st);
int launch_tile_count(const uint32_t *tag, int B, int N, int32_t *tile_counts, int32_t *counts, int32_t *scene_acc,
                      hipStream_t st);
int launch_affine(const PtxShape &s, const ScenePts &points, uint32_t *tag, const float *kcenter,
                  const float *translate, const float *transform, float *out, int32_t *counts,
                  const int32_t *tile_counts, bool compact, bool clear_tag, hipStream_t st,
                  const uint32_t *poison = nullptr);

int launch_img_mean(const void *img, int dt, int nimg, int in_dim, int hw, float *fm, hipStream_t st,
                    uint32_t *gate = nullptr, uint32_t gate_seq = 0);
int launch_img_scores(const void *img, int dt, const float *we, const float *qkv0, int nimg, int in_dim,
                      int hw, int heads, int C, int KT1, int KT2p, float scale, float *gbuf, hipStream_t st);
int launch_img_gather(const void *img, int dt, int nimg, int in_dim, int hw, int heads, int KT2p, float *gbuf,
                      hipStream_t st);
bool img_pool_supported(int dt, int in_dim, int hw, int heads);
size_t img_pool_bytes(int nimg, int in_dim, int EW);
void img_pool_layout(float *scratch, int nimg, int in_dim, int EW, float **Gs, float **E, float **ML);
int launch_img_pool(const void *img, int dt, const float *we, const float *qkv0, int nimg, int in_dim, int hw, int C,
                    int KT1, int EW, float scale, float *Gs, float *E, float *ML, hipStream_t st);

bool img_pool32_supported(int dt, int in_dim, int hw, int heads);
int launch_img_pool32(const float *img, const float *we, const float *qkv0, int nimg, int in_dim, int hw, int C, int KT1, int EW,
                      float scale, float *Gs, float *E, float *ML, hipStream_t st);

int run_prepare(const PtxShape &s, const PtxWeights &w, float *prep, hipStream_t st);

}
```

proxytransformation_amd/csrc/gemm.hip:

```cpp
#include <atomic>
#include <cstdlib>

#include "common.h"
#include "split3.h"

namespace ptx {

constexpr int BK = 32, LDT = BK + 4;

__device__ __forceinline__ void pin4(float4 &v) { asm volatile("" : "+v"(v.x), "+v"(v.y), "+v"(v.z), "+v"(v.w)); }
__device__ __forceinline__ void ln_row_stats(const GemmProb &pr, int row, float &mu, float &rstd)
{
    const float2 *pp = reinterpret_cast<const float2 *>(pr.lnp_in) + (size_t)row * pr.ln_parts;
    constexpr int kMaxParts = 16;
    float2 v[kMaxParts];
#pragma unroll
    for (int t = 0; t < kMaxParts; ++t) v[t] = pp[min(t, pr.ln_parts - 1)];
    float s1 = 0.0f, s2 = 0.0f;
#pragma unroll
    for (int t = 0; t < kMaxParts; ++t) { s1 += t < pr.ln_parts ? v[t].x : 0.0f; s2 += t < pr.ln_parts ? v[t].y : 0.0f; }
    const float inv = 1.0f / (float)pr.ln_C;
    mu = s1 * inv;
    float between = 0.0f;
#pragma unroll
// ... 381 lines not shown
    if (ln) {
        if (tid < 128) {
            float mu, rs;
            ln_row_stats(pr, min(row0 + tid, pr.R - 1), mu, rs);
            s_mu[tid] = mu; s_rs[tid] = rs;
        }
        __syncthreads();
        mu0 = s_mu[sr]; mu1 = s_mu[sr + 64];
    }
    PTX_Y_STASH(P, 0, 0);
    __syncthreads();
#define PTX_Y_PIPE()                                                                       \
    do {                                                                                   \
        if (NP != 3 || !PTX_G128_PIPE) break;                                              \
        __builtin_amdgcn_sched_group_barrier(0x100, 12, 0);              \
        _Pragma("unroll") for (int g_ = 0; g_ < 12; ++g_) {                                \
            __builtin_amdgcn_sched_group_barrier(0x008, 2, 0);                             \
            __builtin_amdgcn_sched_group_barrier(0x002, 8, 0);                             \
            __builtin_amdgcn_sched_group_barrier(0x200, 1, 0);                             \
        }                                                                                  \
    } while (0)
#define PTX_Y_MACRO(S, T, u_)                                                              \
    PTX_Y_COMPUTE(0);                                                                      \
    PTX_Y_STASH(S, 1, 1);                                                                  \
    PTX_Y_PIPE();                                                                          \
    __syncthreads();                                                                       \
    if ((u_) + 2 < NM || rep + 1 < nrep) PTX_Y_FETCH(S, mbase + (u_) + 2);                 \
    __builtin_amdgcn_sched_barrier(0);                                                     \
    PTX_Y_COMPUTE(1);                                                                      \
    if ((u_) + 1 < NM || rep + 1 < nrep) PTX_Y_STASH(T, 0, 0);                             \
    PTX_Y_PIPE();                                                                          \
    __syncthreads();
    int mbase = 0;
    for (int rep = 0; rep < nrep; ++rep) {
#pragma unroll
        for (int u = 0; u < NM; u += 2) {
            PTX_Y_MACRO(P, Q, u)
            PTX_Y_MACRO(Q, P, u + 1)
        }
        mbase += NM;
    }
#undef PTX_Y_MACRO
#undef PTX_Y_PIPE
    (void)total;
    float *scratch = reinterpret_cast<float *>(smem) + wid * (32 * 33);
#pragma unroll
    for (int q = 0; q < 4; ++q) {
        const int i = q >> 1, j = q & 1;
        const int n = col0 + wc * 64 + j * 32 + li, nc = min(n, pr.N - 1);
        const bool ncol = n < pr.N;
        const float bias = pr.bias ? pr.bias[nc] : 0.0f;
        float lnc = 0.0f;
        if (ln) lnc = pr.ln_c[nc];
        float resv[16], adv[16], rsv[16];
#pragma unroll
        for (int r = 0; r < 16; ++r) {
            const int row = min(row0 + wr * 64 + i * 32 + (r & 3) + 8 * (r >> 2) + 4 * hh, pr.R - 1);
            resv[r] = pr.res ? pr.res[(size_t)row * pr.ldres + nc] : 0.0f;
            adv[r] = pr.rs ? pr.ad[(size_t)row * pr.ldad + nc] : 0.0f;
            rsv[r] = pr.rs ? pr.rs[(size_t)row * pr.rs_stride] : 0.0f;
        }
        float fin[16];
#pragma unroll
        for (int r = 0; r < 16; ++r) {
            const int rl = wr * 64 + i * 32 + (r & 3) + 8 * (r >> 2) + 4 * hh, row = row0 + rl;
            float v = acc[q][r] + bias;
            if (ln) v = fmaf(s_rs[rl], acc[q][r], lnc);
            if (pr.epi == EPI_GELU) v = gelu_erf(v);
            const bool ok = ncol && row < pr.R;
            if (pr.rs) v = fmaf(rsv[r], adv[r], v);
            if (pr.res) v += resv[r];
            if (ok) pr.C[(size_t)row * pr.ldc + n] = v;
            fin[r] = ok ? v : 0.0f;
        }
        if (pr.lnp_out != nullptr)
            ln_tile_partials(pr, fin, scratch, row0 + wr * 64 + i * 32, (col0 >> 5) + wc * 2 + j, (pr.N + 31) >> 5);
    }
    PTX_TAIL_GATE(gb, tid == 0);
}
#undef PTX_Y_FETCH
#undef PTX_Y_STASH
#undef PTX_Y_COMPUTE

template <int SK, int AMODE, bool CHAIN = false, bool LN = false>
__global__ __launch_bounds__(SK * 64) void k_gemm32(GemmBatch gb)
{
    const GemmProb pr = gb.p[blockIdx.z];
    const int row0 = blockIdx.x * 32, col0 = blockIdx.y * 32;
    if (row0 >= pr.R || col0 >= pr.N) return;
    extern __shared__ __attribute__((aligned(16))) float lds[];
    const int lane = threadIdx.x & 63;
    const int wv = __builtin_amdgcn_readfirstlane(threadIdx.x >> 6);
    float *base = lds + (size_t)wv * (4 * 32 * LDT);
    const int li = lane & 31, hh = lane >> 5;
    const int nk = (pr.K + BK - 1) / BK, per = (nk + SK - 1) / SK;
    const int it0 = wv * per, it1 = min(nk, it0 + per);
    const int r0 = lane >> 3, kq = (lane & 7) * 4;
    const size_t a0 = (size_t)min(row0 + r0, pr.R - 1) * pr.lda, a1 = (size_t)min(row0 + r0 + 8, pr.R - 1) * pr.lda;
    const size_t a2 = (size_t)min(row0 + r0 + 16, pr.R - 1) * pr.lda, a3 = (size_t)min(row0 + r0 + 24, pr.R - 1) * pr.lda;
    const size_t w0 = (size_t)min(col0 + r0, pr.N - 1) * pr.ldw, w1 = (size_t)min(col0 + r0 + 8, pr.N - 1) * pr.ldw;
    const size_t w2 = (size_t)min(col0 + r0 + 16, pr.N - 1) * pr.ldw, w3 = (size_t)min(col0 + r0 + 24, pr.N - 1) * pr.ldw;
    const float4 z4 = make_float4(0.f, 0.f, 0.f, 0.f);
    float4 aA0, aA1, aA2, aA3, wA0, wA1, wA2, wA3, aB0, aB1, aB2, aB3, wB0, wB1, wB2, wB3;
    float4 gA0 = z4, gA1 = z4, gA2 = z4, gA3 = z4, gB0 = z4, gB1 = z4, gB2 = z4, gB3 = z4;
    int kA = 0, kB = 0;
    (void)kA; (void)kB;
    size_t g0 = 0, g1 = 0, g2 = 0, g3 = 0, e0 = 0, e1 = 0, e2 = 0, e3 = 0;
    float fc0[4] = {0.f, 0.f, 0.f, 0.f}, fc1[4] = {0.f, 0.f, 0.f, 0.f}, fct[4] = {0.f, 0.f, 0.f, 0.f};
    float *cts = lds + (size_t)SK * (4 * 32 * LDT);
    float *lnst = cts + 32 + wv * 64;
    const bool ln = LN && pr.lnp_in != nullptr;
    float mu4[4] = {0.0f, 0.0f, 0.0f, 0.0f};
    if (AMODE == 1) {
#pragma unroll
        for (int i = 0; i < 4; ++i) {
            const int row = min(row0 + r0 + 8 * i, pr.R - 1);
            const float *ml = pr.pml + (size_t)row * pr.ldml;
            const float m0 = ml[0], l0 = ml[1], m1 = ml[2], l1 = ml[3], s0 = ml[4];
            const float m = fmaxf(fmaxf(m0, m1), s0);
            const float x0 = __expf(m0 - m), x1 = __expf(m1 - m), xt = __expf(s0 - m);
            const float inv = 1.0f / ((l0 * x0 + l1 * x1) + xt);
            fc0[i] = x0 * inv; fc1[i] = x1 * inv; fct[i] = xt * inv;
            if (wv == 0 && (lane & 7) == 0) cts[r0 + 8 * i] = fct[i];
        }
        g0 = (size_t)min(row0 + r0, pr.R - 1) * pr.ldg; g1 = (size_t)min(row0 + r0 + 8, pr.R - 1) * pr.ldg;
        g2 = (size_t)min(row0 + r0 + 16, pr.R - 1) * pr.ldg; g3 = (size_t)min(row0 + r0 + 24, pr.R - 1) * pr.ldg;
        e0 = (size_t)min(row0 + r0, pr.R - 1) * pr.lde; e1 = (size_t)min(row0 + r0 + 8, pr.R - 1) * pr.lde;
        e2 = (size_t)min(row0 + r0 + 16, pr.R - 1) * pr.lde; e3 = (size_t)min(row0 + r0 + 24, pr.R - 1) * pr.lde;
    }
#define PTX_FETCH(S, j_)                                                                  \
    do {                                                                                  \
        int jj_ = min((j_), cnt - 1) + rot;                                               \
        jj_ -= jj_ >= cnt ? cnt : 0;                                                      \
        const int k_ = (it0 + jj_) * BK + kq, kc_ = min(k_, pr.K - 4);                    \
        const bool ok_ = k_ < pr.K;                                                       \
        if (AMODE == 0) {                                                                 \
            a##S##0 = *reinterpret_cast<const float4 *>(pr.A + a0 + kc_);                 \
            a##S##1 = *reinterpret_cast<const float4 *>(pr.A + a1 + kc_);                 \
            a##S##2 = *reinterpret_cast<const float4 *>(pr.A + a2 + kc_);                 \
            a##S##3 = *reinterpret_cast<const float4 *>(pr.A + a3 + kc_);                 \
        } else if (kc_ < pr.kg) {               \
            a##S##0 = *reinterpret_cast<const float4 *>(pr.pg + g0 + kc_);                \
            a##S##1 = *reinterpret_cast<const float4 *>(pr.pg + g1 + kc_);                \
            a##S##2 = *reinterpret_cast<const float4 *>(pr.pg + g2 + kc_);                \
            a##S##3 = *reinterpret_cast<const float4 *>(pr.pg + g3 + kc_);                \
            g##S##0 = *reinterpret_cast<const float4 *>(pr.pg + g0 + pr.gslab + kc_);     \
            g##S##1 = *reinterpret_cast<const float4 *>(pr.pg + g1 + pr.gslab + kc_);     \
            g##S##2 = *reinterpret_cast<const float4 *>(pr.pg + g2 + pr.gslab + kc_);     \
            g##S##3 = *reinterpret_cast<const float4 *>(pr.pg + g3 + pr.gslab + kc_);     \
        } else {                                                                          \
            a##S##0 = *reinterpret_cast<const float4 *>(pr.pe + e0 + (kc_ - pr.kg));      \
            a##S##1 = *reinterpret_cast<const float4 *>(pr.pe + e1 + (kc_ - pr.kg));      \
            a##S##2 = *reinterpret_cast<const float4 *>(pr.pe + e2 + (kc_ - pr.kg));      \
            a##S##3 = *reinterpret_cast<const float4 *>(pr.pe + e3 + (kc_ - pr.kg));      \
        }                                                                                 \
        k##S = kc_;                                                                       \
        w##S##0 = *reinterpret_cast<const float4 *>(pr.W + w0 + kc_);                     \
        w##S##1 = *reinterpret_cast<const float4 *>(pr.W + w1 + kc_);                     \
        w##S##2 = *reinterpret_cast<const float4 *>(pr.W + w2 + kc_);                     \
        w##S##3 = *reinterpret_cast<const float4 *>(pr.W + w3 + kc_);                     \
        if (!ok_) { w##S##0 = z4; w##S##1 = z4; w##S##2 = z4; w##S##3 = z4; }             \
    } while (0)
#define PTX_MERGE(S, i_)                                                                  \
    do {                                                                                  \
        if (k##S < pr.kg) {                                                               \
            a##S##i_ = make_float4(a##S##i_.x * fc0[i_] + g##S##i_.x * fc1[i_], a##S##i_.y * fc0[i_] + g##S##i_.y * fc1[i_], \
                                   a##S##i_.z * fc0[i_] + g##S##i_.z * fc1[i_], a##S##i_.w * fc0[i_] + g##S##i_.w * fc1[i_]); \
        } else {                                                                          \
            const int t_ = k##S - pr.kg;       \
            a##S##i_.x *= t_ == 0 ? fct[i_] : (t_ <= 128 ? fc0[i_] : fc1[i_]);           \
            a##S##i_.y *= t_ + 1 <= 128 ? fc0[i_] : fc1[i_];                              \
            a##S##i_.z *= t_ + 2 <= 128 ? fc0[i_] : fc1[i_];                              \
            a##S##i_.w *= t_ + 3 <= 128 ? fc0[i_] : fc1[i_];                              \
        }                                                                                 \
    } while (0)
#define PTX_STASH(S, buf_)                                                                \
    do {                                                                                  \
        float *A_s = base + (buf_) * (2 * 32 * LDT) + r0 * LDT + kq, *W_s = A_s + 32 * LDT; \
        if (AMODE == 1) { PTX_MERGE(S, 0); PTX_MERGE(S, 1); PTX_MERGE(S, 2); PTX_MERGE(S, 3); } \
        if (LN) { sub4(a##S##0, mu4[0]); sub4(a##S##1, mu4[1]); sub4(a##S##2, mu4[2]); sub4(a##S##3, mu4[3]); } \
        *reinterpret_cast<float4 *>(A_s) = a##S##0;                                       \
        *reinterpret_cast<float4 *>(A_s + 8 * LDT) = a##S##1;                             \
        *reinterpret_cast<float4 *>(A_s + 16 * LDT) = a##S##2;                            \
        *reinterpret_cast<float4 *>(A_s + 24 * LDT) = a##S##3;                            \
        *reinterpret_cast<float4 *>(W_s) = w##S##0;                                       \
        *reinterpret_cast<float4 *>(W_s + 8 * LDT) = w##S##1;                             \
        *reinterpret_cast<float4 *>(W_s + 16 * LDT) = w##S##2;                            \
        *reinterpret_cast<float4 *>(W_s + 24 * LDT) = w##S##3;                            \
    } while (0)
#define PTX_COMPUTE(buf_)                                                                 \
    do {                                                                                  \
        const float *A_ = base + (buf_) * (2 * 32 * LDT) + li * LDT + hh * 4, *W_ = A_ + 32 * LDT; \
        _Pragma("unroll") for (int kk = 0; kk < BK / 8; ++kk) {                           \
            const float4 a4 = *reinterpret_cast<const float4 *>(A_ + kk * 8);             \
            const float4 b4 = *reinterpret_cast<const float4 *>(W_ + kk * 8);             \
            acc = __builtin_amdgcn_mfma_f32_32x32x2f32(a4.x, b4.x, acc, 0, 0, 0);         \
            acc = __builtin_amdgcn_mfma_f32_32x32x2f32(a4.y, b4.y, acc, 0, 0, 0);         \
            acc = __builtin_amdgcn_mfma_f32_32x32x2f32(a4.z, b4.z, acc, 0, 0, 0);         \
            acc = __builtin_amdgcn_mfma_f32_32x32x2f32(a4.w, b4.w, acc, 0, 0, 0);         \
        }                                                                                 \
    } while (0)
    const int n = col0 + li;
    float bias = 0.0f, lnc = 0.0f, resv[16], adv[16], rsv[16];
#pragma unroll
    for (int r = 0; r < 16; ++r) { resv[r] = 0.0f; adv[r] = 0.0f; rsv[r] = 0.0f; }
    const bool has_ad = AMODE == 1 || pr.rs != nullptr;
    if (wv == 0) {
        const int nc = min(n, pr.N - 1);
        if (pr.bias) bias = pr.bias[nc];
        if (ln) lnc = pr.ln_c[nc];
#pragma unroll
        for (int r = 0; r < 16; ++r) {
            const int row = min(row0 + (r & 3) + 8 * (r >> 2) + 4 * hh, pr.R - 1);
            if (pr.res) resv[r] = pr.res[(size_t)row * pr.ldres + nc];
            if (has_ad) adv[r] = pr.ad[(size_t)row * pr.ldad + nc];
            if (AMODE != 1 && has_ad) rsv[r] = pr.rs[(size_t)row * pr.rs_stride];
        }
    }
    f32x16 acc;
#pragma unroll
    for (int i = 0; i < 16; ++i) acc[i] = 0.0f;
    const int cnt = it1 - it0;
    const int rot = (cnt > 1 && gb.rotate) ? (int)((blockIdx.x + 3u * blockIdx.y) % (unsigned)cnt) : 0;
    if (cnt > 0) {
        PTX_FETCH(A, 0);
        PTX_FETCH(B, 1);
        if (ln) {
            if (lane < 32) {
                float mu, rs;
                ln_row_stats(pr, min(row0 + lane, pr.R - 1), mu, rs);
                lnst[2 * lane] = mu; lnst[2 * lane + 1] = rs;
            }
#pragma unroll
            for (int i = 0; i < 4; ++i) mu4[i] = lnst[2 * (r0 + 8 * i)];
        }
        PTX_STASH(A, 0);
        for (int j = 0; j < cnt; j += 2) {
            PTX_FETCH(A, j + 2);
            PTX_COMPUTE(0);
            PTX_STASH(B, 1);
            if (j + 1 >= cnt) break;
            PTX_FETCH(B, j + 3);
            PTX_COMPUTE(1);
            PTX_STASH(A, 0);
        }
    }
#undef PTX_FETCH
#undef PTX_STASH
#undef PTX_COMPUTE
    const bool chain = CHAIN && pr.w2 != nullptr && (int)blockIdx.y < pr.chain_tiles;
    if (SK > 1) {
        __syncthreads();
        if (wv > 0) {
#pragma unroll
            for (int r = 0; r < 16; ++r) base[r * 64 + lane] = acc[r];
        }
        __syncthreads();
        if (wv > 0 && !chain) return;
        if (wv == 0) {
#pragma unroll
            for (int w = 1; w < SK; ++w) {
                const float *o = lds + (size_t)w * (4 * 32 * LDT);
#pragma unroll
                for (int r = 0; r < 16; ++r) acc[r] += o[r * 64 + lane];
            }
        }
    }
    if (wv == 0) {
        const bool ncol = n < pr.N;
        float fin[16];
#pragma unroll
        for (int r = 0; r < 16; ++r) {
            const int rl = (r & 3) + 8 * (r >> 2) + 4 * hh, row = row0 + rl;
            float v = acc[r] + bias;
            if (ln) v = fmaf(lnst[2 * rl + 1], acc[r], lnc);
            if (pr.epi == EPI_GELU) v = gelu_erf(v);
            const bool ok = ncol && row < pr.R;
            if (ok) {
                if (AMODE == 1) v = fmaf(cts[rl], adv[r], v);
                else if (pr.rs) v = fmaf(rsv[r], adv[r], v);
                if (pr.res) v += resv[r];
                pr.C[(size_t)row * pr.ldc + n] = v;
            }
            fin[r] = ok ? v : 0.0f;
        }
        if (pr.lnp_out != nullptr)
            ln_tile_partials(pr, fin, lds, row0, col0 >> 5, (pr.N + 31) >> 5);
        if (chain) {
#pragma unroll
            for (int r = 0; r < 16; ++r) lds[((r & 3) + 8 * (r >> 2) + 4 * hh) * LDT + li] = fin[r];
        }
    }
    PTX_TAIL_GATE(gb, threadIdx.x == 0);
    if (!chain) return;
    if (CHAIN) {
        __syncthreads();
        const float *W2 = pr.w2 + (size_t)blockIdx.y * pr.w2_stride;
        float *C2 = pr.c2 + (size_t)blockIdx.y * pr.c2_stride;
        float4 ya[4];
#pragma unroll
        for (int kk = 0; kk < 4; ++kk) ya[kk] = *reinterpret_cast<const float4 *>(lds + li * LDT + kk * 8 + hh * 4);
        const int nt2 = (pr.n2 + 31) >> 5;
        auto load_w2 = [&](int t, float4 (&wb)[4]) {
            const float *wr = W2 + (size_t)min(t * 32 + li, pr.n2 - 1) * 32 + hh * 4;
#pragma unroll
            for (int kk = 0; kk < 4; ++kk) wb[kk] = *reinterpret_cast<const float4 *>(wr + kk * 8);
        };
        float4 wb[4], wn[4];
        load_w2(min(wv, nt2 - 1), wb);
        for (int t = wv; t < nt2; t += SK) {
            const int m = t * 32 + li;
            load_w2(min(t + SK, nt2 - 1), wn);
            f32x16 c2;
#pragma unroll
            for (int i = 0; i < 16; ++i) c2[i] = 0.0f;
#pragma unroll
            for (int kk = 0; kk < 4; ++kk) {
                c2 = __builtin_amdgcn_mfma_f32_32x32x2f32(ya[kk].x, wb[kk].x, c2, 0, 0, 0);
                c2 = __builtin_amdgcn_mfma_f32_32x32x2f32(ya[kk].y, wb[kk].y, c2, 0, 0, 0);
                c2 = __builtin_amdgcn_mfma_f32_32x32x2f32(ya[kk].z, wb[kk].z, c2, 0, 0, 0);
                c2 = __builtin_amdgcn_mfma_f32_32x32x2f32(ya[kk].w, wb[kk].w, c2, 0, 0, 0);
            }
            if (m < pr.n2) {
#pragma unroll
                for (int r = 0; r < 16; ++r) {
                    const int row = row0 + (r & 3) + 8 * (r >> 2) + 4 * hh;
                    if (row < pr.R) C2[(size_t)row * pr.ldc2 + m] = c2[r];
                }
            }
#pragma unroll
            for (int kk = 0; kk < 4; ++kk) wb[kk] = wn[kk];
        }
    }
}

template <int SK, int AMODE, bool CHAIN = false, bool LN = false>
static int launch_gemm32(const GemmBatch &gb, int rmax, int nmax, hipStream_t st)
{
    const size_t lds = sizeof(float) * (SK * 4 * 32 * LDT + 32 + 64 * SK);
    if (lds > 64 * 1024)
        PTX_HIP(hipFuncSetAttribute(reinterpret_cast<const void *>(&k_gemm32<SK, AMODE, CHAIN, LN>),
                                    hipFuncAttributeMaxDynamicSharedMemorySize, (int)lds));
    hipLaunchKernelGGL((k_gemm32<SK, AMODE, CHAIN, LN>), dim3(cdiv(rmax, 32), cdiv(nmax, 32), gb.n), dim3(SK * 64), lds, st, gb);
    return PTX_OK;
}

static std::atomic<int> g_gemm128_min_tiles{256};
int gemm_policy(int min_tiles_128)
{
    return min_tiles_128 < 0 ? g_gemm128_min_tiles.load() : g_gemm128_min_tiles.exchange(min_tiles_128);
}

int launch_gemm(const GemmBatch &gb_in, hipStream_t st, int compute_dtype)
{
    GemmBatch gb = gb_in;
    gb.rotate = 0;
    PTX_REQUIRE(gb.n >= 1 && gb.n <= kMaxGroups, "gemm: %d groups", gb.n);
    int rmax = 0, nmax = 0, kmin = 1 << 30, kmax = 0;
    long tiles32 = 0;
    bool any_ln = false;
    for (int g = 0; g < gb.n; ++g) {
        const GemmProb &p = gb.p[g];
        PTX_REQUIRE((p.A || p.pg) && p.W && p.C, "gemm: null operand in group %d", g);
        PTX_REQUIRE((p.pg != nullptr) == (gb.p[0].pg != nullptr), "gemm: mixed A modes in one batch");
        PTX_REQUIRE(p.pg == nullptr || (p.pe && p.pml && p.ad && p.kg % BK == 0 && p.kg <= p.K && p.ldg % 4 == 0 &&
                                        p.gslab % 4 == 0 && p.lde % 4 == 0),
                    "gemm: bad pooled-A description in group %d", g);
        PTX_REQUIRE(p.R >= 1 && p.N >= 1 && p.K >= 4, "gemm: empty problem in group %d", g);
        PTX_REQUIRE(p.K % 4 == 0 && p.lda % 4 == 0 && p.ldw % 4 == 0,
                    "gemm: K=%d lda=%d ldw=%d must be multiples of 4", p.K, p.lda, p.ldw);
        PTX_REQUIRE(((reinterpret_cast<uintptr_t>(p.A) | reinterpret_cast<uintptr_t>(p.W) | reinterpret_cast<uintptr_t>(p.pg) |
                      reinterpret_cast<uintptr_t>(p.pe)) & 15) == 0,
                    "gemm: operands of group %d are not 16-byte aligned", g);
        PTX_REQUIRE(p.rs == nullptr || p.ad != nullptr, "gemm: row scale without addend");
        PTX_REQUIRE(p.lnp_in == nullptr || (p.ln_c && p.ln_parts >= 1 && p.ln_parts <= 16 && p.ln_C == 32 * p.ln_parts &&
                                            p.K == p.ln_C && p.pg == nullptr && p.bias == nullptr),
                    "gemm: bad LayerNorm-consumer description in group %d", g);
        any_ln = any_ln || p.lnp_in != nullptr;
        rmax = p.R > rmax ? p.R : rmax;
        nmax = p.N > nmax ? p.N : nmax;
        kmin = p.K < kmin ? p.K : kmin;
        kmax = p.K > kmax ? p.K : kmax;
        tiles32 += (long)cdiv(p.R, 32) * cdiv(p.N, 32);
    }
    if (gb.p[0].w2 != nullptr) {
        PTX_REQUIRE(gb.n == 1 && gb.p[0].pg == nullptr && gb.p[0].c2 && gb.p[0].n2 >= 1 && gb.p[0].chain_tiles >= 1 &&
                    gb.p[0].chain_tiles * 32 <= gb.p[0].N && gb.p[0].K >= 4 * BK && gb.p[0].lnp_out == nullptr && !any_ln,
                    "gemm: bad chained-product description");
        PTX_TRY((launch_gemm32<4, 0, true>(gb, rmax, nmax, st)));
        PTX_LAUNCHED("k_gemm");
        return PTX_OK;
    }
    constexpr int g64_min = 1024;
    long tiles128 = 0;
    for (int g = 0; g < gb.n; ++g) tiles128 += (long)cdiv(gb.p[g].R, 128) * cdiv(gb.p[g].N, 128);
    const int min128 = g_gemm128_min_tiles.load(std::memory_order_relaxed);
    const bool enough = tiles128 >= min128 && (min128 == 1 || 2 * tiles128 >= 3 * (long)min128 || kmin >= 512);
    const bool use128 = gb.p[0].pg == nullptr && kmin == kmax && kmin % 256 == 0 && kmin <= 4096 && min128 > 0 && enough;
    if (use128) {
        const dim3 grid(cdiv(rmax, 128), cdiv(nmax, 128), gb.n);
        const int nrep = kmin / (32 * PTX_G128_NM);
        if (compute_dtype == 1) {
            if (any_ln) hipLaunchKernelGGL((k_gemm128x<PTX_G128_NM, 1, true>), grid, dim3(256), 0, st, gb, nrep);
            else        hipLaunchKernelGGL((k_gemm128x<PTX_G128_NM, 1>), grid, dim3(256), 0, st, gb, nrep);
        } else {
            if (any_ln) hipLaunchKernelGGL((k_gemm128x<PTX_G128_NM, 3, true>), grid, dim3(256), 0, st, gb, nrep);
            else        hipLaunchKernelGGL((k_gemm128x<PTX_G128_NM, 3>), grid, dim3(256), 0, st, gb, nrep);
        }
        PTX_LAUNCHED("k_gemm128x");
        return PTX_OK;
    }
    if (compute_dtype == 1 && gb.p[0].pg == nullptr && kmin == kmax && kmin % 128 == 0 && kmin / 128 <= 8) {
        const dim3 grid(cdiv(rmax, 64), cdiv(nmax, 64), gb.n);
        const int nkg = kmin / 128;
        if (any_ln && nkg == 1) hipLaunchKernelGGL((k_gemm64x<1, 1, 1, true>), grid, dim3(256), 0, st, gb);
        else if (any_ln && nkg == 2) hipLaunchKernelGGL((k_gemm64x<2, 1, 1, true>), grid, dim3(256), 0, st, gb);
        else if (any_ln && nkg == 4) hipLaunchKernelGGL((k_gemm64x<4, 1, 1, true>), grid, dim3(256), 0, st, gb);
        else if (any_ln) { set_error("gemm: LayerNorm consumer with K=%d in bf16 mode", kmin); return PTX_EINVAL; }
        else if (nkg == 1) hipLaunchKernelGGL((k_gemm64x<1, 1, 1>), grid, dim3(256), 0, st, gb);
        else if (nkg == 2) hipLaunchKernelGGL((k_gemm64x<2, 1, 1>), grid, dim3(256), 0, st, gb);
        else if (nkg == 4) hipLaunchKernelGGL((k_gemm64x<4, 1, 1>), grid, dim3(256), 0, st, gb);
        else if (nkg == 8) hipLaunchKernelGGL((k_gemm64x<8, 1, 1>), grid, dim3(256), 0, st, gb);
        else if (nkg == 6) hipLaunchKernelGGL((k_gemm64x<2, 3, 1>), grid, dim3(256), 0, st, gb);
        else { set_error("gemm: K=%d in bf16 mode", kmin); return PTX_EINVAL; }
        PTX_LAUNCHED("k_gemm64x<bf16>");
        return PTX_OK;
    }
    if (gb.p[0].pg != nullptr) {
        PTX_TRY((launch_gemm32<4, 1>(gb, rmax, nmax, st)));
    } else if (tiles32 >= g64_min) {
        const dim3 grid(cdiv(rmax, 64), cdiv(nmax, 64), gb.n);
        const int nkg = (kmin == kmax && kmin % 128 == 0) ? kmin / 128 : 0;
        if (any_ln && nkg == 1) hipLaunchKernelGGL((k_gemm64x<1, 1, 3, true>), grid, dim3(256), 0, st, gb);
        else if (any_ln && nkg == 2) hipLaunchKernelGGL((k_gemm64x<2, 1, 3, true>), grid, dim3(256), 0, st, gb);
        else if (any_ln && nkg == 4) hipLaunchKernelGGL((k_gemm64x<4, 1, 3, true>), grid, dim3(256), 0, st, gb);
        else if (any_ln) hipLaunchKernelGGL(k_gemm64<true>, grid, dim3(256), 0, st, gb);
        else if (nkg == 1) hipLaunchKernelGGL((k_gemm64x<1, 1>), grid, dim3(256), 0, st, gb);
        else if (nkg == 2) hipLaunchKernelGGL((k_gemm64x<2, 1>), grid, dim3(256), 0, st, gb);
        else if (nkg == 4) hipLaunchKernelGGL((k_gemm64x<4, 1>), grid, dim3(256), 0, st, gb);
        else if (nkg == 8) hipLaunchKernelGGL((k_gemm64x<8, 1>), grid, dim3(256), 0, st, gb);
        else if (nkg == 6) hipLaunchKernelGGL((k_gemm64x<2, 3>), grid, dim3(256), 0, st, gb);
        else if (nkg == 12) hipLaunchKernelGGL((k_gemm64x<4, 3>), grid, dim3(256), 0, st, gb);
        else if (nkg == 16) hipLaunchKernelGGL((k_gemm64x<8, 2>), grid, dim3(256), 0, st, gb);
        else if (nkg == 32) hipLaunchKernelGGL((k_gemm64x<8, 4>), grid, dim3(256), 0, st, gb);
        else hipLaunchKernelGGL(k_gemm64<false>, grid, dim3(256), 0, st, gb);
    } else {
        const int nk = cdiv(kmin, BK);
        int sk = 1;
        while (sk < 4 && tiles32 * sk < 4096 && nk >= 4 * sk) sk *= 2;
        if (any_ln) {
            if (sk == 1) PTX_TRY((launch_gemm32<1, 0, false, true>(gb, rmax, nmax, st)));
            else if (sk == 2) PTX_TRY((launch_gemm32<2, 0, false, true>(gb, rmax, nmax, st)));
            else PTX_TRY((launch_gemm32<4, 0, false, true>(gb, rmax, nmax, st)));
        } else if (sk == 1) PTX_TRY((launch_gemm32<1, 0>(gb, rmax, nmax, st)));
        else if (sk == 2) PTX_TRY((launch_gemm32<2, 0>(gb, rmax, nmax, st)));
        else PTX_TRY((launch_gemm32<4, 0>(gb, rmax, nmax, st)));
    }
    PTX_LAUNCHED("k_gemm");
    return PTX_OK;
}

constexpr int kMaxPerLane = 8;

__device__ __forceinline__ void ln_row(const float *x, int C, float eps, float (&v)[kMaxPerLane],
                                       float &mean, float &rstd)
{
    const int lane = lane_id();
    float s = 0.0f;
#pragma unroll
    for (int q = 0; q < kMaxPerLane; ++q) {
        const int c = lane + 64 * q;
        v[q] = c < C ? x[c] : 0.0f;
        s += v[q];
    }
    mean = wave_sum(s) / (float)C;
    float var = 0.0f;
#pragma unroll
    for (int q = 0; q < kMaxPerLane; ++q) {
        const int c = lane + 64 * q;
        const float d = c < C ? v[q] - mean : 0.0f;
        var = fmaf(d, d, var);
    }
    rstd = 1.0f / sqrtf(wave_sum(var) / (float)C + eps);
}

__global__ __launch_bounds__(256) void k_ln_rows(LnBatch lb)
{
    const LnProb p = lb.p[blockIdx.y];
    const int row = __builtin_amdgcn_readfirstlane(blockIdx.x * 4 + (threadIdx.x >> 6));
    if (row >= p.R) return;
    float v[kMaxPerLane], mean, rstd;
    ln_row(p.x + (size_t)row * lb.C, lb.C, lb.eps, v, mean, rstd);
    const int lane = lane_id();
#pragma unroll
    for (int q = 0; q < kMaxPerLane; ++q) {
        const int c = lane + 64 * q;
        if (c < lb.C) {
            float y = (v[q] - mean) * rstd * p.w[c] + p.b[c];
            if (p.add) y += p.add[(size_t)(row % p.add_rows) * lb.C + c];
            p.y[(size_t)row * lb.C + c] = y;
        }
    }
}

int launch_ln_rows(const LnBatch &lb, hipStream_t st)
{
    PTX_REQUIRE(lb.C % 64 == 0 && lb.C <= 64 * kMaxPerLane, "layer norm: C=%d unsupported", lb.C);
    int rmax = 0;
    for (int g = 0; g < lb.n; ++g) rmax = lb.p[g].R > rmax ? lb.p[g].R : rmax;
    if (rmax == 0) return PTX_OK;
    hipLaunchKernelGGL(k_ln_rows, dim3(cdiv(rmax, 4), lb.n), dim3(256), 0, st, lb);
    PTX_LAUNCHED("k_ln_rows");
    return PTX_OK;
}

constexpr int kHeadRows = 4;

template <int Q>
__global__ __launch_bounds__(256) void k_heads(HeadBatch hb)
{
    const HeadProb p = hb.p[blockIdx.y];
    const int row0 = __builtin_amdgcn_readfirstlane((blockIdx.x * 4 + (threadIdx.x >> 6)) * kHeadRows);
    if (row0 >= p.R) return;
    const int lane = lane_id();
    constexpr int kMaxOut = 9;
    float hbias = 0.0f, bn_a = 0.0f, bn_b = 0.0f;
    if (lane < p.nout) { hbias = p.hb[lane]; bn_a = p.ab[lane]; bn_b = p.ab[p.nout + lane]; }
    float nw[Q], nb[Q], hwt[kMaxOut][Q];
#pragma unroll
    for (int q = 0; q < Q; ++q) { nw[q] = p.nw[lane + 64 * q]; nb[q] = p.nb[lane + 64 * q]; }
#pragma unroll
    for (int o = 0; o < kMaxOut; ++o)
#pragma unroll
        for (int q = 0; q < Q; ++q) hwt[o][q] = o < p.nout ? p.hw[(size_t)o * hb.C + lane + 64 * q] : 0.0f;
    float x[kHeadRows][Q];
#pragma unroll
// ... 55 lines not shown
```

proxytransformation_amd/csrc/imgpool.hip:

```cpp
#include <cstdlib>
#include <hip/hip_ext.h>

#include "common.h"
#include "imgstore.h"

namespace ptx {

typedef __bf16 bf16x8 __attribute__((ext_vector_type(8)));

constexpr int kPoolHeads = 8;
constexpr int kPoolNtImages = 4096;
constexpr int kPoolWPad = 544;
constexpr int kPoolPPad = 136;

typedef _Float16 f16x8 __attribute__((ext_vector_type(8)));

template <int DT>
__device__ __forceinline__ void split3(float x, unsigned short &q1, unsigned short &q2, unsigned short &q3)
{
    if (DT == 1) {
        const unsigned int u1 = __float_as_uint(x) & 0xffff0000u;
        const float r1 = x - __uint_as_float(u1);
        const unsigned int u2 = __float_as_uint(r1) & 0xffff0000u;
        const float r2 = r1 - __uint_as_float(u2);
// ... 19 lines not shown
__device__ __forceinline__ int pow2_scale_exp(float amax)
{
    const int e = (int)((__float_as_uint(amax) >> 23) & 0xffu) - 127;
    return (amax > 0.0f && e > -100 && e < 100) ? 13 - e : 0;
}
__device__ __forceinline__ float pow2f(int k) { return __uint_as_float((unsigned int)(127 + k) << 23); }
constexpr float kPoolEScale = 16384.0f;

__device__ __forceinline__ u32x4 shr_elems(const u32x4 &v, int k)
{
    const int ws = k >> 1;
    unsigned int w[8] = {v[0], v[1], v[2], v[3], 0u, 0u, 0u, 0u};
    u32x4 o;
#pragma unroll
    for (int q = 0; q < 4; ++q) {
        unsigned int lo = 0u, hi = 0u;
#pragma unroll
        for (int s = 0; s < 4; ++s) {
            if (ws == s) { lo = w[q + s]; hi = w[q + s + 1]; }
        }
        o[q] = (k & 1) ? ((lo >> 16) | (hi << 16)) : lo;
    }
    return o;
}

struct PoolArgs {
    const unsigned short *img; const float *we, *qkv0;
    int nimg, in_dim, hw, C, KT1, EW; float scale;
    float *Gs;
    float *E;
    float *ML;
};

template <int DT, bool NT>
__global__ __launch_bounds__(512) void k_img_pool(PoolArgs a)
{
    constexpr int heads = kPoolHeads;
    extern __shared__ __attribute__((aligned(16))) unsigned char smem[];
    float *partial = reinterpret_cast<float *>(smem);
    unsigned short *wpart = reinterpret_cast<unsigned short *>(partial + 8 * heads * 128);
    unsigned short *parts = wpart + 24 * kPoolWPad;
    const int in_dim = a.in_dim, hw = a.hw;
    const int xcd = blockIdx.x & 7, slot = blockIdx.x >> 3;
    const int T = slot & 1, imr = (slot >> 1) * 8 + xcd;
    if (imr >= a.nimg) return;
    const int im = a.nimg - 1 - imr;
    const int slab = im * 2 + T;
    const int tid = threadIdx.x, lane = lane_id();
    const int wid = __builtin_amdgcn_readfirstlane(tid >> 6);
    const int n = lane & 15, kq = lane >> 4;
    const float *wim = a.we + (size_t)im * heads * a.KT1;
    const unsigned short *f = a.img + (size_t)im * in_dim * hw;
    const int px = 128 * T + 8 * n;
    const bool full = px + 8 <= hw;
    const int cw = 64 * wid;
    float wv[heads];
#pragma unroll
    for (int h = 0; h < heads; ++h) wv[h] = wim[(size_t)h * a.KT1 + tid];
    u32x4 L[2][8];
    const bool tensor_end = im == a.nimg - 1 && cw + 64 == in_dim;
#pragma unroll
    for (int kb = 0; kb < 2; ++kb) {
        const unsigned short *r = f + (size_t)(cw + 32 * kb + 8 * kq) * hw + px;
#pragma unroll
        for (int i = 0; i < 8; ++i) {
            if (kb == 1 && i == 7 && tensor_end) {
                const bool lastrow = kq == 3 && !full;
                const int back = lastrow ? px + 8 - hw : 0;
                const int bk = back > 8 ? px - (hw - 8) : back;
                u32x4 v = __builtin_nontemporal_load(reinterpret_cast<const u4u2 *>(r + (size_t)i * hw - bk));
                L[kb][i] = lastrow ? (back >= 8 ? u32x4{0u, 0u, 0u, 0u} : shr_elems(v, back)) : v;
            } else {
                L[kb][i] = __builtin_nontemporal_load(reinterpret_cast<const u4u2 *>(r + (size_t)i * hw));
            }
        }
    }
    float ev[2];
#pragma unroll
    for (int u = 0; u < 2; ++u) {
        const int p = 128 * T + lane + 64 * u;
        ev[u] = p < hw ? wim[(size_t)wid * a.KT1 + in_dim + 1 + p] : 0.0f;
    }
    float sq = 0.0f, sk = 0.0f;
    if (T == 0) {
        const int hd = a.C / heads;
        const float *qv = a.qkv0 + (size_t)im * 3 * a.C + wid * hd;
        if (lane < hd) { sq = qv[lane]; sk = qv[a.C + lane]; }
    }
    {
        const int c = tid;
#pragma unroll
        for (int h = 0; h < heads; ++h) {
            if (DT == 2) {
                const int k = pow2_scale_exp(wave_max(fabsf(wv[h])));
                wv[h] *= pow2f(k);
                if (lane == 0) *reinterpret_cast<float *>(wpart + (size_t)h * kPoolWPad + in_dim + 2 * wid) = pow2f(-k);
            }
            unsigned short q1, q2, q3;
            split3<DT>(wv[h], q1, q2, q3);
            wpart[(size_t)h * kPoolWPad + c] = q1;
            wpart[(size_t)(8 + h) * kPoolWPad + c] = q2;
            wpart[(size_t)(16 + h) * kPoolWPad + c] = q3;
        }
    }
    __syncthreads();

    {
        f32x4 acc[8];
#pragma unroll
        for (int j = 0; j < 8; ++j) acc[j] = f32x4{0.f, 0.f, 0.f, 0.f};
        const bool lo = n < heads;
#pragma unroll
        for (int kb = 0; kb < 2; ++kb) {
            u32x4 af[3];
#pragma unroll
            for (int pt = 0; pt < 3; ++pt) {
                u32x4 t = *reinterpret_cast<const u32x4 *>(wpart + (size_t)(pt * 8 + (n & 7)) * kPoolWPad + cw + 32 * kb + 8 * kq);
                if (!lo) t = u32x4{0u, 0u, 0u, 0u};
                af[pt] = t;
            }
#pragma unroll
            for (int j = 0; j < 8; ++j) {
                const unsigned int sel = (j & 1) ? 0x07060302u : 0x05040100u;
                u32x4 b;
#pragma unroll
                for (int qd = 0; qd < 4; ++qd) b[qd] = __builtin_amdgcn_perm(L[kb][2 * qd + 1][j >> 1], L[kb][2 * qd][j >> 1], sel);
#pragma unroll
                for (int pt = 0; pt < 3; ++pt) acc[j] = mfma16<DT>(af[pt], b, acc[j]);
            }
        }
        if (kq < 2) {
#pragma unroll
            for (int r = 0; r < 4; ++r) {
                float us = 1.0f;
                if (DT == 2) us = *reinterpret_cast<const float *>(wpart + (size_t)(4 * kq + r) * kPoolWPad + in_dim + 2 * wid);
                float *d = partial + ((size_t)wid * heads + 4 * kq + r) * 128 + 8 * n;
                *reinterpret_cast<float4 *>(d) = make_float4(acc[0][r] * us, acc[1][r] * us, acc[2][r] * us, acc[3][r] * us);
                *reinterpret_cast<float4 *>(d + 4) = make_float4(acc[4][r] * us, acc[5][r] * us, acc[6][r] * us, acc[7][r] * us);
            }
        }
    }
    __syncthreads();

    {
        const int h = wid;
        float e[2], mloc = -INFINITY, sv[2];
#pragma unroll
        for (int u = 0; u < 2; ++u) {
            const int p = lane + 64 * u;
            float s = 0.0f;
#pragma unroll
            for (int w = 0; w < 8; ++w) s += partial[((size_t)w * heads + h) * 128 + p];
            sv[u] = 128 * T + p < hw ? s + ev[u] : -INFINITY;
            mloc = fmaxf(mloc, sv[u]);
        }
        const float m = wave_max(mloc);
#pragma unroll
        for (int u = 0; u < 2; ++u) e[u] = 128 * T + lane + 64 * u < hw ? expf(sv[u] - m) : 0.0f;
        const float l = wave_sum(e[0] + e[1]);
        float *erow = a.E + ((size_t)im * heads + h) * a.EW;
        const float s0 = T == 0 ? wave_sum(sq * sk) * a.scale : 0.0f;
        if (lane == 0) {
            float *ml = a.ML + ((size_t)im * heads + h) * 5;
            ml[2 * T] = m;
            ml[2 * T + 1] = l;
            if (T == 0) { ml[4] = s0; erow[0] = 1.0f; }
        }
#pragma unroll
        for (int u = 0; u < 2; ++u) {
            const int p = lane + 64 * u;
            const int t = 1 + 128 * T + p;
            if (t <= hw || (T == (hw > 128 ? 1 : 0) && t < a.EW)) erow[t] = t <= hw ? e[u] : 0.0f;
            unsigned short q1, q2, q3;
            split3<DT>(DT == 2 ? e[u] * kPoolEScale : e[u], q1, q2, q3);
            parts[(size_t)h * kPoolPPad + p] = q1;
            parts[(size_t)(8 + h) * kPoolPPad + p] = q2;
            parts[(size_t)(16 + h) * kPoolPPad + p] = q3;
        }
    }
    __syncthreads();

    {
        const int ps = n & 3, hh = n >> 2;
        const int src = ((ps + 4 * kq) + 16 * (n >> 2)) * 4;
        u32x4 bfr[2][3];
#pragma unroll
        for (int hg = 0; hg < 2; ++hg)
#pragma unroll
            for (int pt = 0; pt < 3; ++pt)
                bfr[hg][pt] = *reinterpret_cast<const u32x4 *>(parts + (size_t)(pt * 8 + 4 * hg + hh) * kPoolPPad + 8 * (ps + 4 * kq));
        const unsigned m0 = ps == 0 ? ~0u : 0u, m1 = ps == 1 ? ~0u : 0u, m2 = ps == 2 ? ~0u : 0u, m3 = ps == 3 ? ~0u : 0u;
        float *G = partial;
#pragma unroll
        for (int kb = 0; kb < 2; ++kb) {
#pragma unroll
            for (int i = 0; i < 8; ++i)
#pragma unroll
                for (int d = 0; d < 4; ++d) L[kb][i][d] = (unsigned int)__builtin_amdgcn_ds_bpermute(src, (int)L[kb][i][d]);
            float xs[2][8];
#pragma unroll
            for (int ig = 0; ig < 4; ++ig) {
                f32x4 c[2][2];
#pragma unroll
                for (int ii = 0; ii < 2; ++ii)
#pragma unroll
                    for (int hg = 0; hg < 2; ++hg) c[ii][hg] = f32x4{0.f, 0.f, 0.f, 0.f};
#pragma unroll
                for (int pt = 0; pt < 3; ++pt)
#pragma unroll
                    for (int ii = 0; ii < 2; ++ii)
#pragma unroll
                        for (int hg = 0; hg < 2; ++hg) c[ii][hg] = mfma16<DT>(L[kb][2 * ig + ii], bfr[hg][pt], c[ii][hg]);
#pragma unroll
                for (int ii = 0; ii < 2; ++ii)
#pragma unroll
                    for (int hg = 0; hg < 2; ++hg) {
                        const f32x4 &acc = c[ii][hg];
                        float x = __uint_as_float((__float_as_uint(acc[0]) & m0) | (__float_as_uint(acc[1]) & m1) |
                                                  (__float_as_uint(acc[2]) & m2) | (__float_as_uint(acc[3]) & m3));
                        x += __int_as_float(__builtin_amdgcn_mov_dpp(__float_as_int(x), 0xB1, 0xF, 0xF, true));
                        x += __int_as_float(__builtin_amdgcn_mov_dpp(__float_as_int(x), 0x4E, 0xF, 0xF, true));
                        xs[hg][2 * ig + ii] = DT == 2 ? x * (1.0f / kPoolEScale) : x;
                    }
            }
            if (ps == 0) {
#pragma unroll
                for (int hg = 0; hg < 2; ++hg)
#pragma unroll
                    for (int q = 0; q < 2; ++q)
                        *reinterpret_cast<f32x4 *>(G + (size_t)(4 * hg + hh) * in_dim + cw + 32 * kb + 8 * kq + 4 * q) =
                            f32x4{xs[hg][4 * q], xs[hg][4 * q + 1], xs[hg][4 * q + 2], xs[hg][4 * q + 3]};
            }
        }
    }
    __syncthreads();
    {
        const float *G = partial;
        float *dst = a.Gs + (size_t)slab * heads * in_dim;
        for (int i = tid * 4; i < heads * in_dim; i += 512 * 4)
        {
            const f32x4 v = *reinterpret_cast<const f32x4 *>(G + i);
            if (NT) asm volatile("global_store_dwordx4 %0, %1, off sc1 nt" :: "v"(dst + i), "v"(v) : "memory");
            else    asm volatile("global_store_dwordx4 %0, %1, off sc1" :: "v"(dst + i), "v"(v) : "memory");
        }
    }
}

bool img_pool_supported(int dt, int in_dim, int hw, int heads)
{
// ... 35 lines not shown
```

proxytransformation_amd/csrc/imgpool32.hip:

```cpp
#include <hip/hip_ext.h>

#include "common.h"

namespace ptx {

typedef float p32_f4u __attribute__((ext_vector_type(4), aligned(4)));
typedef float p32_f4 __attribute__((ext_vector_type(4)));

constexpr int kP32Heads = 8;
constexpr int kP32Tile = 32;
constexpr int kP32Tiles = 128 / kP32Tile;
constexpr int kP32TRow = 36;

struct Pool32Args {
    const float *img; const float *we, *qkv0;
    int nimg, in_dim, hw, C, KT1, EW; float scale;
    float *Gs, *E, *ML;
};

__global__ __launch_bounds__(512) __attribute__((amdgpu_waves_per_eu(4, 4))) void k_img_pool32(Pool32Args a)
{
    constexpr int heads = kP32Heads, TP = kP32Tile;
    extern __shared__ __attribute__((aligned(16))) float p32_sm[];
    float *W_s = p32_sm;
    float *S_s = W_s + 512 * heads;
    float *E_s = S_s + 8 * heads * TP;
    float *sc_s = E_s + heads * TP;
    float *T_s = sc_s + 16;
    const int in_dim = a.in_dim, hw = a.hw;
    const int xcd = blockIdx.x & 7, slot = blockIdx.x >> 3;
    const int H = slot & 1, imr = (slot >> 1) * 8 + xcd;
    if (imr >= a.nimg) return;
    const int im = a.nimg - 1 - imr;
    const int tid = threadIdx.x, lane = lane_id();
    const int wid = __builtin_amdgcn_readfirstlane(tid >> 6);
    const int n = lane & 7, kq = lane >> 3;
    const int mr = lane & 15, mk = lane >> 4;
    const float *wim = a.we + (size_t)im * heads * a.KT1;
    const float *f = a.img + (size_t)im * in_dim * hw;
    float *T_w = T_s + (size_t)wid * (16 * kP32TRow);
    float wv[heads];
#pragma unroll
    for (int h = 0; h < heads; ++h) wv[h] = wim[(size_t)h * a.KT1 + tid];
    float ev[kP32Tiles];
#pragma unroll
    for (int t = 0; t < kP32Tiles; ++t) {
        const int p = 128 * H + TP * t + (lane & (TP - 1));
        ev[t] = p < hw ? wim[(size_t)wid * a.KT1 + in_dim + 1 + p] : 0.0f;
    }
    float sq = 0.0f, sk = 0.0f;
    if (H == 0) {
        const int hd = a.C / heads;
        const float *qv = a.qkv0 + (size_t)im * 3 * a.C + wid * hd;
        if (lane < hd) { sq = qv[lane]; sk = qv[a.C + lane]; }
    }
    const char *fb = reinterpret_cast<const char *>(f);
    const unsigned row_off = (unsigned)(64 * wid + kq) * (unsigned)hw * 4u, row_step = 8u * (unsigned)hw * 4u;
    const bool tensor_end = im == a.nimg - 1 && wid == 7 && kq == 7;
    {
        *reinterpret_cast<p32_f4 *>(W_s + tid * heads) = p32_f4{wv[0], wv[1], wv[2], wv[3]};
        *reinterpret_cast<p32_f4 *>(W_s + tid * heads + 4) = p32_f4{wv[4], wv[5], wv[6], wv[7]};
        if (tid < 16) sc_s[tid] = 0.0f;
    }
    p32_f4 D[4];
#pragma unroll
    for (int q = 0; q < 4; ++q) D[q] = p32_f4{0.f, 0.f, 0.f, 0.f};
    float m_run = -INFINITY, l_run = 0.0f, e_t[kP32Tiles];
#pragma unroll
    for (int t = 0; t < kP32Tiles; ++t) e_t[t] = 0.0f;

#pragma unroll
    for (int t = 0; t < kP32Tiles; ++t) {
        const int px0 = 128 * H + TP * t;
        p32_f4u L[8];
        {
            const int p = px0 + 4 * n;
            const int pc = p < hw ? p : 0;
            const unsigned off0 = row_off + (unsigned)pc * 4u;
#pragma unroll
            for (int i = 0; i < 8; ++i) {
                const float *rowp = reinterpret_cast<const float *>(fb + (off0 + (unsigned)i * row_step)) - pc;
                if (i == 7 && tensor_end && pc + 4 > hw) {
                    const p32_f4u v = *reinterpret_cast<const p32_f4u *>(rowp + hw - 4);
                    const int back = pc + 4 - hw;
                    L[i] = back == 1 ? p32_f4u{v[1], v[2], v[3], 0.f} : back == 2 ? p32_f4u{v[2], v[3], 0.f, 0.f} : p32_f4u{v[3], 0.f, 0.f, 0.f};
                } else {
                    L[i] = __builtin_nontemporal_load(reinterpret_cast<const p32_f4u *>(rowp + pc));
                }
            }
        }
        __syncthreads();
#pragma unroll
        for (int hb = 0; hb < heads; hb += 4) {
            float acc[4][4];
#pragma unroll
            for (int h = 0; h < 4; ++h) { acc[h][0] = acc[h][1] = acc[h][2] = acc[h][3] = 0.0f; }
#pragma unroll
            for (int i = 0; i < 8; ++i) {
                const p32_f4 w4 = *reinterpret_cast<const p32_f4 *>(W_s + (64 * wid + 8 * i + kq) * heads + hb);
                const p32_f4u v = L[i];
#pragma unroll
                for (int h = 0; h < 4; ++h) {
                    acc[h][0] = fmaf(w4[h], v[0], acc[h][0]); acc[h][1] = fmaf(w4[h], v[1], acc[h][1]);
                    acc[h][2] = fmaf(w4[h], v[2], acc[h][2]); acc[h][3] = fmaf(w4[h], v[3], acc[h][3]);
                }
            }
#pragma unroll
            for (int h = 0; h < 4; ++h)
#pragma unroll
                for (int c = 0; c < 4; ++c) {
                    float x = acc[h][c];
                    x += PTX_ROR_F(x, 8);
                    x += __shfl_xor(x, 16, 64);
                    x += __shfl_xor(x, 32, 64);
                    acc[h][c] = x;
                }
            if (kq == 0) {
#pragma unroll
                for (int h = 0; h < 4; ++h)
                    *reinterpret_cast<p32_f4 *>(S_s + ((size_t)wid * heads + hb + h) * TP + 4 * n) = p32_f4{acc[h][0], acc[h][1], acc[h][2], acc[h][3]};
            }
            __builtin_amdgcn_sched_barrier(0);
        }
        __syncthreads();
        {
            const int h = wid, pl = lane & (TP - 1);
            float s = 0.0f;
#pragma unroll
            for (int w = 0; w < 8; ++w) s += S_s[((size_t)w * heads + h) * TP + pl];
            const bool valid = lane < TP && px0 + pl < hw;
            const float sv = valid ? s + ev[t] : -INFINITY;
            const float m_new = fmaxf(m_run, wave_max(sv));
            const float resc = expf(m_run - m_new);
            const float e = valid ? expf(sv - m_new) : 0.0f;
            l_run = l_run * resc + wave_sum(e);
            m_run = m_new;
#pragma unroll
            for (int u = 0; u < kP32Tiles; ++u) e_t[u] = u < t ? e_t[u] * resc : (u == t ? e : 0.0f);
            if (lane < TP) E_s[h * TP + lane] = e;
            if (lane == 0) sc_s[h] = resc;
            if (t == kP32Tiles - 1) {
                float *erow = a.E + ((size_t)im * heads + h) * a.EW;
#pragma unroll
                for (int u = 0; u < kP32Tiles; ++u) {
                    const int tok = 1 + 128 * H + TP * u + lane;
                    if (lane < TP && tok < a.EW) erow[tok] = e_t[u];
                }
                const float s0 = H == 0 ? wave_sum(sq * sk) * a.scale : 0.0f;
                if (lane == 0) {
                    float *ml = a.ML + ((size_t)im * heads + h) * 5;
                    ml[2 * H] = m_run; ml[2 * H + 1] = l_run;
                    if (H == 0) { ml[4] = s0; erow[0] = 1.0f; }
                }
            }
        }
        __syncthreads();
        {
            const float resc = sc_s[mr];
#pragma unroll
            for (int q = 0; q < 4; ++q) { D[q][0] *= resc; D[q][1] *= resc; D[q][2] *= resc; D[q][3] *= resc; }
#pragma unroll
            for (int q = 0; q < 4; ++q) {
#pragma unroll
                for (int ii = 0; ii < 2; ++ii)
                    *reinterpret_cast<p32_f4 *>(T_w + (8 * ii + kq) * kP32TRow + 4 * n) = p32_f4{L[2 * q + ii][0], L[2 * q + ii][1], L[2 * q + ii][2], L[2 * q + ii][3]};
                __builtin_amdgcn_wave_barrier();
                __builtin_amdgcn_fence(__ATOMIC_RELEASE, "wavefront");
#pragma unroll
                for (int pb = 0; pb < TP / 16; ++pb) {
                    const p32_f4 a4 = *reinterpret_cast<const p32_f4 *>(T_w + mr * kP32TRow + 16 * pb + 4 * mk);
                    p32_f4 e4 = *reinterpret_cast<const p32_f4 *>(E_s + (mr & 7) * TP + 16 * pb + 4 * mk);
                    if (mr >= heads) e4 = p32_f4{0.f, 0.f, 0.f, 0.f};
#pragma unroll
                    for (int c = 0; c < 4; ++c) D[q] = __builtin_amdgcn_mfma_f32_16x16x4f32(a4[c], e4[c], D[q], 0, 0, 0);
                }
                __builtin_amdgcn_wave_barrier();
                __builtin_amdgcn_fence(__ATOMIC_ACQUIRE, "wavefront");
            }
        }
    }
    __syncthreads();
    float *G = W_s;
    if (mr < heads) {
#pragma unroll
        for (int q = 0; q < 4; ++q)
            *reinterpret_cast<p32_f4 *>(G + (size_t)mr * in_dim + 64 * wid + 16 * q + 4 * mk) = D[q];
    }
    __syncthreads();
    {
        float *dst = a.Gs + (size_t)(im * 2 + H) * heads * in_dim;
        for (int i = tid * 4; i < heads * in_dim; i += 512 * 4) {
            const p32_f4 v = *reinterpret_cast<const p32_f4 *>(G + i);
            asm volatile("global_store_dwordx4 %0, %1, off sc1" :: "v"(dst + i), "v"(v) : "memory");
        }
    }
}

bool img_pool32_supported(int dt, int in_dim, int hw, int heads)
{
    return dt == 0 && heads == kP32Heads && in_dim == 512 && hw > 128 && hw <= 255;
}

int launch_img_pool32(const float *img, const float *we, const float *qkv0, int nimg, int in_dim, int hw, int C, int KT1, int EW,
                      float scale, float *Gs, float *E, float *ML, hipStream_t st)
{
    PTX_REQUIRE(EW % 4 == 0 && EW >= hw + 1 && hw > 128 && hw <= 255 && in_dim == 512, "img pool (fp32): hw=%d EW=%d in_dim=%d", hw, EW, in_dim);
    PTX_REQUIRE((reinterpret_cast<uintptr_t>(img) & 15) == 0, "img_feat must be 16-byte aligned");
    Pool32Args pa{img, we, qkv0, nimg, in_dim, hw, C, KT1, EW, scale, Gs, E, ML};
    const size_t lds = sizeof(float) * (512 * kP32Heads + 8 * kP32Heads * kP32Tile + kP32Heads * kP32Tile + 16 + 8 * 16 * kP32TRow);
    const dim3 grid(cdiv(nimg, 8) * 16);
    hipEvent_t ta = nullptr, tb = nullptr;
    (void)timing_ext_take(&ta, &tb);
    hipExtLaunchKernelGGL(k_img_pool32, grid, dim3(512), lds, st, ta, tb, 0, pa);
    PTX_LAUNCHED("k_img_pool32");
    return PTX_OK;
}

}
```

proxytransformation_amd/csrc/prep.hip:

```cpp
#include "common.h"

namespace ptx {

__global__ void k_prep_bn(const float *w, const float *b, const float *mean, const float *var,
                          int n, float eps, float *ab)
{
    const int i = blockIdx.x * blockDim.x + threadIdx.x;
    if (i >= n) return;
    const float alpha = w[i] / sqrtf(var[i] + eps);
    ab[i] = alpha;
    ab[n + i] = b[i] - mean[i] * alpha;
}

__global__ void k_prep_posbias(const float *pb, const float *pc, const float *pr, int Mk, int s, int C,
                               float *out)
{
    const int i = blockIdx.x * blockDim.x + threadIdx.x;
    if (i >= Mk * C) return;
    const int j = i / C, yx = i - j * C, y = yx / s, x = yx - y * s;
    const float sc = 4.0f / (float)s;
    float sy = sc * ((float)y + 0.5f) - 0.5f; if (sy < 0.f) sy = 0.f;
    float sx = sc * ((float)x + 0.5f) - 0.5f; if (sx < 0.f) sx = 0.f;
    const int y0 = (int)sy, x0 = (int)sx;
    const int y1 = y0 + (y0 < 3 ? 1 : 0), x1 = x0 + (x0 < 3 ? 1 : 0);
    const float ly1 = sy - (float)y0, ly0 = 1.f - ly1, lx1 = sx - (float)x0, lx0 = 1.f - lx1;
    const float *p = pb + (size_t)j * 16;
    const float v = ly0 * (lx0 * p[y0 * 4 + x0] + lx1 * p[y0 * 4 + x1]) +
                    ly1 * (lx0 * p[y1 * 4 + x0] + lx1 * p[y1 * 4 + x1]);
    out[i] = v + (pc[(size_t)j * s + y] + pr[(size_t)j * s + x]);
}

__global__ void k_prep_w3(const float *qw, const float *kw, const float *vw, const float *qb,
                          const float *cw, const float *cb, const float *pos, int C, int in_dim,
                          float *w3, float *b3)
{
    const int i = blockIdx.x * blockDim.x + threadIdx.x;
    if (i >= 3 * C * (in_dim + 1)) return;
    const int n = i / (in_dim + 1), c = i - n * (in_dim + 1);
    const int part = n / C, r = n - part * C;
    const float *wrow = (part == 0 ? qw : (part == 1 ? kw : vw)) + (size_t)r * C;
    float s = 0.0f;
    if (c < in_dim) {
        for (int j = 0; j < C; ++j) s = fmaf(wrow[j], cw[(size_t)j * in_dim + c], s);
        w3[(size_t)n * in_dim + c] = s;
    } else {
        for (int j = 0; j < C; ++j) s = fmaf(wrow[j], cb[j] + pos[j], s);
        b3[n] = s + (part == 0 ? qb[r] : 0.0f);
    }
}

__global__ void k_prep_t1(const float *kw, const float *cw, const float *cb, const float *pos, int C,
                          int in_dim, int hw, int heads, float scale, float *t1)
{
    const int hd = C / heads, KT1 = in_dim + hw + 1;
    const int i = blockIdx.x * blockDim.x + threadIdx.x;
    if (i >= heads * KT1 * hd) return;
    const int h = i / (KT1 * hd), rem = i - h * KT1 * hd, t = rem / hd, d = rem - t * hd;
    const float *wk = kw + (size_t)(h * hd + d) * C;
    float s = 0.0f;
    if (t < in_dim) {
        for (int j = 0; j < C; ++j) s = fmaf(wk[j], cw[(size_t)j * in_dim + t], s);
    } else if (t > in_dim) {
        const float *pi = pos + (size_t)(t - in_dim) * C;
        for (int j = 0; j < C; ++j) s = fmaf(wk[j], cb[j] + pi[j], s);
    }
    t1[i] = s * scale;
}

__global__ void k_prep_t2(const float *vw, const float *cw, const float *cb, const float *pos, int C,
                          int in_dim, int hw, int heads, int KT2p, float *t2)
{
    const int hd = C / heads;
    const int i = blockIdx.x * blockDim.x + threadIdx.x;
    if (i >= heads * hd * KT2p) return;
    const int h = i / (hd * KT2p), rem = i - h * hd * KT2p, d = rem / KT2p, t = rem - d * KT2p;
    const float *wv = vw + (size_t)(h * hd + d) * C;
    float s = 0.0f;
    if (t < in_dim) {
        for (int j = 0; j < C; ++j) s = fmaf(wv[j], cw[(size_t)j * in_dim + t], s);
    } else if (t > in_dim && t <= in_dim + hw) {
        const float *pi = pos + (size_t)(t - in_dim) * C;
        for (int j = 0; j < C; ++j) s = fmaf(wv[j], cb[j] + pi[j], s);
    }
    t2[i] = s;
}

__global__ void k_prep_lnfold(const float *W, const float *gamma, const float *beta, const float *bias, int N, int K,
                              float *Wg, float *cv)
{
    const int n = blockIdx.x * (blockDim.x >> 6) + (threadIdx.x >> 6);
    if (n >= N) return;
    const int lane = threadIdx.x & 63;
    float c1 = 0.0f;
    for (int k = lane; k < K; k += 64) {
        const float wv = W[(size_t)n * K + k];
        Wg[(size_t)n * K + k] = wv * gamma[k];
        c1 = fmaf(wv, beta[k], c1);
    }
    c1 = wave_sum(c1);
    if (lane == 0) cv[n] = c1 + (bias ? bias[n] : 0.0f);
}

int launch_prep_lnfold(const float *W, const float *gamma, const float *beta, const float *bias, int N, int K, float *Wg,
                       float *cv, hipStream_t st)
{
    hipLaunchKernelGGL(k_prep_lnfold, dim3(cdiv(N, 4)), dim3(256), 0, st, W, gamma, beta, bias, N, K, Wg, cv);
    PTX_LAUNCHED("k_prep_lnfold");
    return PTX_OK;
}

int run_prepare(const PtxShape &s, const PtxWeights &w, float *prep, hipStream_t st)
{
    const PrepLayout P = prep_layout(s);
    const int C = s.C, T = 256;
    hipLaunchKernelGGL(k_prep_bn, dim3(1), dim3(T), 0, st, w.offset.bn_w, w.offset.bn_b,
                       w.offset.bn_mean, w.offset.bn_var, kSlotHidden, s.bn_eps, prep + P.off_ab);
    hipLaunchKernelGGL(k_prep_bn, dim3(cdiv(C, T)), dim3(T), 0, st, w.encoder.bn_w, w.encoder.bn_b,
                       w.encoder.bn_mean, w.encoder.bn_var, C, s.bn_eps, prep + P.enc_ab);
    hipLaunchKernelGGL(k_prep_bn, dim3(1), dim3(T), 0, st, w.text_trans_norm.w, w.text_trans_norm.b,
                       w.text_trans_norm.mean, w.text_trans_norm.var, 3, s.bn_eps, prep + P.ttn_ab);
    hipLaunchKernelGGL(k_prep_bn, dim3(1), dim3(T), 0, st, w.img_trans_norm.w, w.img_trans_norm.b,
                       w.img_trans_norm.mean, w.img_trans_norm.var, 9, s.bn_eps, prep + P.itn_ab);
    PTX_LAUNCHED("k_prep_bn");
    int sd = 1;
    while (sd * sd < C) ++sd;
    const int nb = s.Mk * C;
    hipLaunchKernelGGL(k_prep_posbias, dim3(cdiv(nb, T)), dim3(T), 0, st, w.text.pb_bias, w.text.pc_bias,
                       w.text.pr_bias, s.Mk, sd, C, prep + P.posb_t);
    hipLaunchKernelGGL(k_prep_posbias, dim3(cdiv(nb, T)), dim3(T), 0, st, w.img.pb_bias, w.img.pc_bias,
                       w.img.pr_bias, s.Mk, sd, C, prep + P.posb_i);
    PTX_LAUNCHED("k_prep_posbias");
    hipLaunchKernelGGL(k_prep_w3, dim3(cdiv(3 * C * (s.in_dim + 1), T)), dim3(T), 0, st, w.q_w, w.k_w, w.v_w,
                       w.q_b, w.cm_w, w.cm_b, w.pos, C, s.in_dim, prep + P.w3, prep + P.b3);
    PTX_LAUNCHED("k_prep_w3");
    const float scale = (float)(1.0 / sqrt((double)P.hd));
    hipLaunchKernelGGL(k_prep_t1, dim3(cdiv(s.heads * P.KT1 * P.hd, T)), dim3(T), 0, st, w.k_w, w.cm_w,
                       w.cm_b, w.pos, C, s.in_dim, s.hw, s.heads, scale, prep + P.t1);
    PTX_LAUNCHED("k_prep_t1");
    hipLaunchKernelGGL(k_prep_t2, dim3(cdiv(s.heads * P.hd * P.KT2p, T)), dim3(T), 0, st, w.v_w, w.cm_w,
                       w.cm_b, w.pos, C, s.in_dim, s.hw, s.heads, P.KT2p, prep + P.t2);
    PTX_LAUNCHED("k_prep_t2");
    PTX_TRY(launch_prep_lnfold(w.img.pp_w, w.norm_img_w, w.norm_img_b, w.img.pp_b, C, C, prep + P.ppg_w, prep + P.ppg_c, st));
    const PtxBlock *blk[2] = {&w.text, &w.img};
    for (int i = 0; i < 2; ++i)
        PTX_TRY(launch_prep_lnfold(blk[i]->fc1_w, blk[i]->norm2_w, blk[i]->norm2_b, blk[i]->fc1_b, s.hidden, C,
// ... 18 lines not shown
```

Before: 18370 scenes/s.

## Fold token-0 image attention into chained QKV GEMM and add FPS wave policy

In the image-proxy path, when the chained and pooled kernels both apply, the first GEMM computes only the Q columns instead of full QKV. The token-0 score is produced inside the chained GEMM as split partial sums written to a new S0 buffer. The pooled output GEMM then rebuilds the token-0 value contribution from the mean features and the V bias, so the pooling kernels no longer need qkv0. A runtime policy also controls whether select/FPS uses the one-wave path, and the prep t1 kernel now fills the column at t == in_dim. This shrinks GEMM width and memory traffic, but adds more template variants, cross-wave reductions and extra loads in the merge step.

```diff
diff --git a/include/proxyt.h b/include/proxyt.h
--- a/include/proxyt.h
+++ b/include/proxyt.h
@@ -120,6 +120,7 @@
                const float *bias, float eps, int gelu, float *y, void *scratch, size_t scratch_bytes,
                int rows, int n_out, int n_in, void *stream);
 PTX_API int ptx_gemm_policy(int min_tiles_128);
+PTX_API int ptx_fps_policy(int waves);
 
 PTX_API int ptx_offset_net(const PtxShape *s, const PtxWeights *w, const void *prep,
                    const float *centers_in, const float *cluster, const float *minmax,
diff --git a/proxytransformation_amd/_abi.py b/proxytransformation_amd/_abi.py
--- a/proxytransformation_amd/_abi.py
+++ b/proxytransformation_amd/_abi.py
@@ -132,6 +132,7 @@
     "ptx_ln_linear_scratch_bytes": (_Z, [_I, _I]),
     "ptx_ln_linear": (_I, [_P, _P, _P, _P, _P, _P, _F, _I, _P, _P, _Z, _I, _I, _I, _P]),
     "ptx_gemm_policy": (_I, [_I]),
+    "ptx_fps_policy": (_I, [_I]),
     "ptx_offset_net": (_I, [_SH, _W, _P, _P, _P, _P, _P, _P, _P]),
     "ptx_select_clusters": (_I, [_SH] + [_P] * 14),
     "ptx_pointnet": (_I, [_SH, _W, _P, _P, _P, _P, _P]),
diff --git a/proxytransformation_amd/csrc/api.hip b/proxytransformation_amd/csrc/api.hip
--- a/proxytransformation_amd/csrc/api.hip
+++ b/proxytransformation_amd/csrc/api.hip
@@ -412,25 +412,29 @@
     if (img_proxy) img_proxy += (size_t)i0 * C;
     const int dt = s.img_dtype;
     img = static_cast<const char *>(img) + (size_t)i0 * s.in_dim * s.hw * (dt == 0 ? 4 : 2);
-    float *Gs = nullptr, *E = nullptr, *ML = nullptr;
+    float *Gs = nullptr, *E = nullptr, *ML = nullptr, *S0 = nullptr;
     const int EW = P.KT2p - s.in_dim;
     const bool pooled32 = img_pool32_supported(dt, s.in_dim, s.hw, s.heads);
     const bool pooled = pooled32 || img_pool_supported(dt, s.in_dim, s.hw, s.heads);
     if (pooled) {
         img_pool_layout(at<float>(ws, L.pool), nall, s.in_dim, EW, &Gs, &E, &ML);
+        S0 = ML + (size_t)nall * s.heads * 5 + (size_t)i0 * s.heads * 2;
         Gs += (size_t)i0 * 2 * s.heads * s.in_dim; E += (size_t)i0 * s.heads * EW; ML += (size_t)i0 * s.heads * 5;
     }
     if (phase != 2) PTX_TIMED(KID_IMG_MEAN, st, launch_img_mean(img, dt, nimg, s.in_dim, s.hw, fm, st, gate, gate_seq));
     if (phase == 1) return PTX_OK;
     const bool chained = hd == 32 && nimg < 4096;
+    constexpr int kToken0Split = 2;
+    const bool fold0 = chained && pooled;
     {
         GemmBatch g{}; g.n = 1;
         g.p[0] = GemmProb{fm, prep + P.w3, qkv0, prep + P.b3, nullptr, nullptr, nullptr,
-                          nimg, 3 * C, s.in_dim, s.in_dim, s.in_dim, 3 * C, 0, 0, 0, EPI_NONE};
+                          nimg, fold0 ? C : 3 * C, s.in_dim, s.in_dim, s.in_dim, 3 * C, 0, 0, 0, EPI_NONE};
         if (chained) {
             g.p[0].w2 = prep + P.t1; g.p[0].c2 = we; g.p[0].n2 = P.KT1; g.p[0].ldc2 = s.heads * P.KT1;
             g.p[0].chain_tiles = s.heads; g.p[0].w2_stride = (long)P.KT1 * hd; g.p[0].c2_stride = P.KT1;
         }
+        if (fold0) { g.p[0].ps0 = S0; g.p[0].lds0 = 2 * s.heads; g.p[0].chain_split = kToken0Split; }
         PTX_TIMED(KID_IMG_QKV0, st, launch_gemm(g, st));
     }
     if (!chained) {
@@ -444,10 +448,10 @@
         }
     }
     if (pooled32) {
-        PTX_TIMED_EXT(KID_IMG_SCORES, st, launch_img_pool32(static_cast<const float *>(img), we, qkv0, nimg, s.in_dim, s.hw, C, P.KT1, EW,
+        PTX_TIMED_EXT(KID_IMG_SCORES, st, launch_img_pool32(static_cast<const float *>(img), we, fold0 ? nullptr : qkv0, nimg, s.in_dim, s.hw, C, P.KT1, EW,
                                                         attn_scale(hd), Gs, E, ML, st));
     } else if (pooled) {
-        PTX_TIMED_EXT(KID_IMG_SCORES, st, launch_img_pool(img, dt, we, qkv0, nimg, s.in_dim, s.hw, C, P.KT1,
+        PTX_TIMED_EXT(KID_IMG_SCORES, st, launch_img_pool(img, dt, we, fold0 ? nullptr : qkv0, nimg, s.in_dim, s.hw, C, P.KT1,
                                                       EW, attn_scale(hd), Gs, E, ML, st));
     } else {
         PTX_TIMED(KID_IMG_SCORES, st, launch_img_scores(img, dt, we, qkv0, nimg, s.in_dim, s.hw, s.heads, C, P.KT1,
@@ -468,6 +472,10 @@
                 gp.pe = E + (size_t)h * EW; gp.lde = s.heads * EW;
                 gp.pml = ML + (size_t)h * 5; gp.ldml = s.heads * 5;
                 gp.kg = s.in_dim;
+                if (fold0) {
+                    gp.pfm = fm; gp.ldfm = s.in_dim; gp.ps0 = S0 + 2 * h; gp.lds0 = 2 * s.heads;
+                    gp.ad = prep + P.b3 + 2 * C + h * hd; gp.ldad = 0;
+                }
             }
         }
         PTX_TIMED(KID_IMG_O, st, launch_gemm(g, st));
@@ -879,6 +887,7 @@
 }
 
 int ptx_gemm_policy(int min_tiles_128) { return gemm_policy(min_tiles_128); }
+int ptx_fps_policy(int waves) { return fps_policy(waves); }
 
 int ptx_offset_net(const PtxShape *s, const PtxWeights *w, const void *prep, const float *centers_in,
                    const float *cluster, const float *minmax, float *centers_out, float *offsets_out,
@@ -1153,8 +1162,10 @@
     const bool ext_event = !capturing;
     const bool tags_gated = gated && side->lo_ok && (lf.v[3] >= 0 ? lf.v[3] != 0 : est_image < 1.6 * est_cluster);
     const bool tags_tail = !cluster_on_caller && !tags_gated;
+    const bool fps_one = cluster_on_caller;
+    hipEvent_t select_done = ext_event && !tags_tail && !tags_gated ? side->aux : nullptr;
     PTX_TIMED(KID_SELECT, cs, launch_select_order(S, centers, pad_count, order_override, order, picks, keep, kcenter,
-                                                  ksrc, bbox_in ? nullptr : mm_ws, cs, cluster_on_caller, ext_event && !tags_tail ? side->aux : nullptr,
+                                                  ksrc, bbox_in ? nullptr : mm_ws, cs, cluster_on_caller, fps_one, select_done,
                                                   cg_join_select ? &cjoin : nullptr));
     int32_t *tile_counts = at<int32_t>(ws, L.tile_counts);
     hipStream_t ts = tags_tail ? cs : side->lo;
diff --git a/proxytransformation_amd/csrc/cluster.hip b/proxytransformation_amd/csrc/cluster.hip
--- a/proxytransformation_amd/csrc/cluster.hip
+++ b/proxytransformation_amd/csrc/cluster.hip
@@ -1,3 +1,4 @@
+#include <atomic>
 #include <cstdlib>
 #include <hip/hip_ext.h>
 
@@ -736,9 +737,15 @@
                       s.Mk, s.Mt - s.Mk, s.N, nullptr, mm_clear, GateRef{}};
 }
 
+static std::atomic<int> g_fps_waves{0};
+int fps_policy(int waves)
+{
+    return waves < 0 ? g_fps_waves.load() : g_fps_waves.exchange(waves == 1 || waves == 4 ? waves : 0);
+}
+
 int launch_select_order(const PtxShape &s, const float *centers, const int32_t *pad_count,
                         const int32_t *order_override, int32_t *order, int32_t *picks, int32_t *keep,
-                        float *kcenter, int32_t *ksrc, uint32_t *mm_clear, hipStream_t st, bool critical,
+                        float *kcenter, int32_t *ksrc, uint32_t *mm_clear, hipStream_t st, bool critical, bool fps_one,
                         hipEvent_t done, const GateRef *tail)
 {
     SelectArgs a = select_args(s, nullptr, centers, nullptr, pad_count, order_override, order, picks, keep, kcenter,
@@ -749,7 +756,8 @@
     PTX_REQUIRE(lds <= 160 * 1024, "select: Mt=%d needs %zu B of LDS (> 160 KiB)", s.Mt, lds);
     const bool alone = critical;
     if (alone && s.B <= 32 && lds < 150 * 1024) lds = 150 * 1024;
-    const bool one = critical && s.Mt <= 384;
+    const int pol = g_fps_waves.load(std::memory_order_relaxed);
+    const bool one = (pol == 1 || (pol == 0 && fps_one)) && s.Mt <= 384;
     const int per = cdiv(s.Mt, one ? 64 : 256);
     const dim3 grid(s.B), block(256);
 #define PTX_SEL(P_)                                                                          \
@@ -797,7 +805,7 @@
                   int32_t *picks, int32_t *keep, float *kcenter, float *kcluster, int32_t *kidx,
                   int32_t *drop_idx, uint32_t *tag, hipStream_t st)
 {
-    PTX_TRY(launch_select_order(s, centers, pad_count, order_override, order, picks, keep, kcenter, nullptr, nullptr, st, true, nullptr));
+    PTX_TRY(launch_select_order(s, centers, pad_count, order_override, order, picks, keep, kcenter, nullptr, nullptr, st, true, true, nullptr));
     PTX_TRY(launch_select_slots(s, idx, cluster, order, picks, keep, kcluster, kidx, drop_idx, nullptr, st));
     if (tag == nullptr) return PTX_OK;
     return launch_tags(s, idx, order, picks, nullptr, tag, nullptr, nullptr, nullptr, st, keep);
diff --git a/proxytransformation_amd/csrc/common.h b/proxytransformation_amd/csrc/common.h
--- a/proxytransformation_amd/csrc/common.h
+++ b/proxytransformation_amd/csrc/common.h
@@ -238,6 +238,7 @@
     float *lnp_out;
     const float *lnp_in, *ln_c; int ln_parts, ln_C; float ln_eps;
     const float *w2; float *c2; int n2, ldc2, chain_tiles; long w2_stride, c2_stride;
+    const float *pfm; int ldfm; float *ps0; int lds0, chain_split;
 };
 constexpr int kMaxGroups = 8;
 struct GemmBatch {
@@ -324,8 +325,9 @@
                   int32_t *drop_idx, uint32_t *tag, hipStream_t st);
 int launch_select_order(const PtxShape &s, const float *centers, const int32_t *pad_count,
                         const int32_t *order_override, int32_t *order, int32_t *picks, int32_t *keep,
-                        float *kcenter, int32_t *ksrc, uint32_t *mm_clear, hipStream_t st, bool critical,
+                        float *kcenter, int32_t *ksrc, uint32_t *mm_clear, hipStream_t st, bool critical, bool fps_one,
                         hipEvent_t done, const GateRef *tail = nullptr);
+int fps_policy(int waves);
 int launch_tags(const PtxShape &s, const int32_t *idx, const int32_t *order, const int32_t *picks, const int32_t *ksrc,
                 uint32_t *tag, int32_t *tile_counts, int32_t *counts, int32_t *scene_acc, hipStream_t st,
                 const int32_t *keep = nullptr);
diff --git a/proxytransformation_amd/csrc/gemm.hip b/proxytransformation_amd/csrc/gemm.hip
--- a/proxytransformation_amd/csrc/gemm.hip
+++ b/proxytransformation_amd/csrc/gemm.hip
@@ -487,11 +487,14 @@
 #undef PTX_Y_STASH
 #undef PTX_Y_COMPUTE
 
-template <int SK, int AMODE, bool CHAIN = false, bool LN = false>
+template <int SK, int AMODE, int CHAIN = 0, bool LN = false>
 __global__ __launch_bounds__(SK * 64) void k_gemm32(GemmBatch gb)
 {
     const GemmProb pr = gb.p[blockIdx.z];
-    const int row0 = blockIdx.x * 32, col0 = blockIdx.y * 32;
+    constexpr bool POOLED = AMODE >= 1, FOLD = AMODE == 2, CFOLD = CHAIN == 2;
+    const int csplit = CFOLD && pr.chain_split > 1 ? pr.chain_split : 1;
+    const int ty = CFOLD ? (int)blockIdx.y / csplit : (int)blockIdx.y, half = CFOLD ? (int)blockIdx.y - ty * csplit : 0;
+    const int row0 = blockIdx.x * 32, col0 = ty * 32;
     if (row0 >= pr.R || col0 >= pr.N) return;
     extern __shared__ __attribute__((aligned(16))) float lds[];
     const int lane = threadIdx.x & 63;
@@ -508,20 +511,24 @@
     const float4 z4 = make_float4(0.f, 0.f, 0.f, 0.f);
     float4 aA0, aA1, aA2, aA3, wA0, wA1, wA2, wA3, aB0, aB1, aB2, aB3, wB0, wB1, wB2, wB3;
     float4 gA0 = z4, gA1 = z4, gA2 = z4, gA3 = z4, gB0 = z4, gB1 = z4, gB2 = z4, gB3 = z4;
+    float4 fA0 = z4, fA1 = z4, fA2 = z4, fA3 = z4, fB0 = z4, fB1 = z4, fB2 = z4, fB3 = z4;
     int kA = 0, kB = 0;
     (void)kA; (void)kB;
-    size_t g0 = 0, g1 = 0, g2 = 0, g3 = 0, e0 = 0, e1 = 0, e2 = 0, e3 = 0;
+    size_t g0 = 0, g1 = 0, g2 = 0, g3 = 0, e0 = 0, e1 = 0, e2 = 0, e3 = 0, f0 = 0, f1 = 0, f2 = 0, f3 = 0;
     float fc0[4] = {0.f, 0.f, 0.f, 0.f}, fc1[4] = {0.f, 0.f, 0.f, 0.f}, fct[4] = {0.f, 0.f, 0.f, 0.f};
     float *cts = lds + (size_t)SK * (4 * 32 * LDT);
     float *lnst = cts + 32 + wv * 64;
     const bool ln = LN && pr.lnp_in != nullptr;
     float mu4[4] = {0.0f, 0.0f, 0.0f, 0.0f};
-    if (AMODE == 1) {
+    if (POOLED) {
 #pragma unroll
         for (int i = 0; i < 4; ++i) {
             const int row = min(row0 + r0 + 8 * i, pr.R - 1);
             const float *ml = pr.pml + (size_t)row * pr.ldml;
-            const float m0 = ml[0], l0 = ml[1], m1 = ml[2], l1 = ml[3], s0 = ml[4];
+            const float m0 = ml[0], l0 = ml[1], m1 = ml[2], l1 = ml[3];
+            float s0;
+            if (FOLD) { const float *sp = pr.ps0 + (size_t)row * pr.lds0; s0 = sp[0] + sp[1]; }
+            else s0 = ml[4];
             const float m = fmaxf(fmaxf(m0, m1), s0);
             const float x0 = __expf(m0 - m), x1 = __expf(m1 - m), xt = __expf(s0 - m);
             const float inv = 1.0f / ((l0 * x0 + l1 * x1) + xt);
@@ -532,6 +539,10 @@
         g2 = (size_t)min(row0 + r0 + 16, pr.R - 1) * pr.ldg; g3 = (size_t)min(row0 + r0 + 24, pr.R - 1) * pr.ldg;
         e0 = (size_t)min(row0 + r0, pr.R - 1) * pr.lde; e1 = (size_t)min(row0 + r0 + 8, pr.R - 1) * pr.lde;
         e2 = (size_t)min(row0 + r0 + 16, pr.R - 1) * pr.lde; e3 = (size_t)min(row0 + r0 + 24, pr.R - 1) * pr.lde;
+        if (FOLD) {
+            f0 = (size_t)min(row0 + r0, pr.R - 1) * pr.ldfm; f1 = (size_t)min(row0 + r0 + 8, pr.R - 1) * pr.ldfm;
+            f2 = (size_t)min(row0 + r0 + 16, pr.R - 1) * pr.ldfm; f3 = (size_t)min(row0 + r0 + 24, pr.R - 1) * pr.ldfm;
+        }
     }
 #define PTX_FETCH(S, j_)                                                                  \
     do {                                                                                  \
@@ -553,6 +564,12 @@
             g##S##1 = *reinterpret_cast<const float4 *>(pr.pg + g1 + pr.gslab + kc_);     \
             g##S##2 = *reinterpret_cast<const float4 *>(pr.pg + g2 + pr.gslab + kc_);     \
             g##S##3 = *reinterpret_cast<const float4 *>(pr.pg + g3 + pr.gslab + kc_);     \
+            if (FOLD) {    \
+                f##S##0 = *reinterpret_cast<const float4 *>(pr.pfm + f0 + kc_);           \
+                f##S##1 = *reinterpret_cast<const float4 *>(pr.pfm + f1 + kc_);           \
+                f##S##2 = *reinterpret_cast<const float4 *>(pr.pfm + f2 + kc_);           \
+                f##S##3 = *reinterpret_cast<const float4 *>(pr.pfm + f3 + kc_);           \
+            }                                                                             \
         } else {                                                                          \
             a##S##0 = *reinterpret_cast<const float4 *>(pr.pe + e0 + (kc_ - pr.kg));      \
             a##S##1 = *reinterpret_cast<const float4 *>(pr.pe + e1 + (kc_ - pr.kg));      \
@@ -571,6 +588,9 @@
         if (k##S < pr.kg) {                                                               \
             a##S##i_ = make_float4(a##S##i_.x * fc0[i_] + g##S##i_.x * fc1[i_], a##S##i_.y * fc0[i_] + g##S##i_.y * fc1[i_], \
                                    a##S##i_.z * fc0[i_] + g##S##i_.z * fc1[i_], a##S##i_.w * fc0[i_] + g##S##i_.w * fc1[i_]); \
+            if (FOLD)      \
+                a##S##i_ = make_float4(a##S##i_.x + f##S##i_.x * fct[i_], a##S##i_.y + f##S##i_.y * fct[i_], \
+                                       a##S##i_.z + f##S##i_.z * fct[i_], a##S##i_.w + f##S##i_.w * fct[i_]); \
         } else {                                                                          \
             const int t_ = k##S - pr.kg;       \
             a##S##i_.x *= t_ == 0 ? fct[i_] : (t_ <= 128 ? fc0[i_] : fc1[i_]);           \
@@ -582,7 +602,7 @@
 #define PTX_STASH(S, buf_)                                                                \
     do {                                                                                  \
         float *A_s = base + (buf_) * (2 * 32 * LDT) + r0 * LDT + kq, *W_s = A_s + 32 * LDT; \
-        if (AMODE == 1) { PTX_MERGE(S, 0); PTX_MERGE(S, 1); PTX_MERGE(S, 2); PTX_MERGE(S, 3); } \
+        if (POOLED) { PTX_MERGE(S, 0); PTX_MERGE(S, 1); PTX_MERGE(S, 2); PTX_MERGE(S, 3); } \
         if (LN) { sub4(a##S##0, mu4[0]); sub4(a##S##1, mu4[1]); sub4(a##S##2, mu4[2]); sub4(a##S##3, mu4[3]); } \
         *reinterpret_cast<float4 *>(A_s) = a##S##0;                                       \
         *reinterpret_cast<float4 *>(A_s + 8 * LDT) = a##S##1;                             \
@@ -609,7 +629,7 @@
     float bias = 0.0f, lnc = 0.0f, resv[16], adv[16], rsv[16];
 #pragma unroll
     for (int r = 0; r < 16; ++r) { resv[r] = 0.0f; adv[r] = 0.0f; rsv[r] = 0.0f; }
-    const bool has_ad = AMODE == 1 || pr.rs != nullptr;
+    const bool has_ad = POOLED || pr.rs != nullptr;
     if (wv == 0) {
         const int nc = min(n, pr.N - 1);
         if (pr.bias) bias = pr.bias[nc];
@@ -619,14 +639,14 @@
             const int row = min(row0 + (r & 3) + 8 * (r >> 2) + 4 * hh, pr.R - 1);
             if (pr.res) resv[r] = pr.res[(size_t)row * pr.ldres + nc];
             if (has_ad) adv[r] = pr.ad[(size_t)row * pr.ldad + nc];
-            if (AMODE != 1 && has_ad) rsv[r] = pr.rs[(size_t)row * pr.rs_stride];
+            if (!POOLED && has_ad) rsv[r] = pr.rs[(size_t)row * pr.rs_stride];
         }
     }
     f32x16 acc;
 #pragma unroll
     for (int i = 0; i < 16; ++i) acc[i] = 0.0f;
     const int cnt = it1 - it0;
-    const int rot = (cnt > 1 && gb.rotate) ? (int)((blockIdx.x + 3u * blockIdx.y) % (unsigned)cnt) : 0;
+    const int rot = (cnt > 1 && gb.rotate) ? (int)((blockIdx.x + 3u * (unsigned)ty) % (unsigned)cnt) : 0;
     if (cnt > 0) {
         PTX_FETCH(A, 0);
         PTX_FETCH(B, 1);
@@ -653,7 +673,7 @@
 #undef PTX_FETCH
 #undef PTX_STASH
 #undef PTX_COMPUTE
-    const bool chain = CHAIN && pr.w2 != nullptr && (int)blockIdx.y < pr.chain_tiles;
+    const bool chain = CHAIN && pr.w2 != nullptr && ty < pr.chain_tiles;
     if (SK > 1) {
         __syncthreads();
         if (wv > 0) {
@@ -682,10 +702,10 @@
             if (pr.epi == EPI_GELU) v = gelu_erf(v);
             const bool ok = ncol && row < pr.R;
             if (ok) {
-                if (AMODE == 1) v = fmaf(cts[rl], adv[r], v);
+                if (POOLED) v = fmaf(cts[rl], adv[r], v);
                 else if (pr.rs) v = fmaf(rsv[r], adv[r], v);
                 if (pr.res) v += resv[r];
-                pr.C[(size_t)row * pr.ldc + n] = v;
+                if (!CFOLD || half == 0) pr.C[(size_t)row * pr.ldc + n] = v;
             }
             fin[r] = ok ? v : 0.0f;
         }
@@ -700,22 +720,34 @@
     if (!chain) return;
     if (CHAIN) {
         __syncthreads();
-        const float *W2 = pr.w2 + (size_t)blockIdx.y * pr.w2_stride;
-        float *C2 = pr.c2 + (size_t)blockIdx.y * pr.c2_stride;
+        const float *W2 = pr.w2 + (size_t)ty * pr.w2_stride;
+        float *C2 = pr.c2 + (size_t)ty * pr.c2_stride;
         float4 ya[4];
 #pragma unroll
         for (int kk = 0; kk < 4; ++kk) ya[kk] = *reinterpret_cast<const float4 *>(lds + li * LDT + kk * 8 + hh * 4);
         const int nt2 = (pr.n2 + 31) >> 5;
+        const int tper = (nt2 + csplit - 1) / csplit, tlo = half * tper, thi = min(nt2, tlo + tper);
         auto load_w2 = [&](int t, float4 (&wb)[4]) {
             const float *wr = W2 + (size_t)min(t * 32 + li, pr.n2 - 1) * 32 + hh * 4;
 #pragma unroll
             for (int kk = 0; kk < 4; ++kk) wb[kk] = *reinterpret_cast<const float4 *>(wr + kk * 8);
         };
+        auto load_fm = [&](int t, float (&fb)[16]) {
+            const int mc = min(t * 32 + li, pr.K - 1);
+#pragma unroll
+            for (int r = 0; r < 16; ++r)
+                fb[r] = pr.A[min(row0 + (r & 3) + 8 * (r >> 2) + 4 * hh, pr.R - 1) * pr.lda + mc];
+        };
         float4 wb[4], wn[4];
-        load_w2(min(wv, nt2 - 1), wb);
-        for (int t = wv; t < nt2; t += SK) {
+        float fb[16], fn[16], s0a[16];
+#pragma unroll
+        for (int r = 0; r < 16; ++r) { fb[r] = 0.0f; fn[r] = 0.0f; s0a[r] = 0.0f; }
+        load_w2(min(tlo + wv, thi - 1), wb);
+        if (CFOLD) load_fm(min(tlo + wv, thi - 1), fb);
+        for (int t = tlo + wv; t < thi; t += SK) {
             const int m = t * 32 + li;
-            load_w2(min(t + SK, nt2 - 1), wn);
+            load_w2(min(t + SK, thi - 1), wn);
+            if (CFOLD) load_fm(min(t + SK, thi - 1), fn);
             f32x16 c2;
 #pragma unroll
             for (int i = 0; i < 16; ++i) c2[i] = 0.0f;
@@ -733,20 +765,45 @@
                     if (row < pr.R) C2[(size_t)row * pr.ldc2 + m] = c2[r];
                 }
             }
+            if (CFOLD) {
+                const float one = m == pr.K ? 1.0f : 0.0f;
+#pragma unroll
+                for (int r = 0; r < 16; ++r) { s0a[r] = fmaf(c2[r], m < pr.K ? fb[r] : one, s0a[r]); fb[r] = fn[r]; }
+            }
 #pragma unroll
             for (int kk = 0; kk < 4; ++kk) wb[kk] = wn[kk];
         }
-    }
-}
-
-template <int SK, int AMODE, bool CHAIN = false, bool LN = false>
-static int launch_gemm32(const GemmBatch &gb, int rmax, int nmax, hipStream_t st)
+        if (CFOLD) {
+#pragma unroll
+            for (int r = 0; r < 16; ++r) {
+                float x = s0a[r];
+                x += __shfl_xor(x, 16, 64); x += __shfl_xor(x, 8, 64); x += __shfl_xor(x, 4, 64);
+                x += __shfl_xor(x, 2, 64); x += __shfl_xor(x, 1, 64);
+                if (li == 0) base[32 * LDT + (r & 3) + 8 * (r >> 2) + 4 * hh] = x;
+            }
+            __syncthreads();
+            if (wv == 0 && lane < 32) {
+                float sum = lds[32 * LDT + lane];
+#pragma unroll
+                for (int w = 1; w < SK; ++w) sum += lds[(size_t)w * (4 * 32 * LDT) + 32 * LDT + lane];
+                if (row0 + lane < pr.R) {
+                    float *sp = pr.ps0 + (size_t)(row0 + lane) * pr.lds0 + 2 * ty;
+                    sp[half] = sum;
+                    if (csplit == 1) sp[1] = 0.0f;
+                }
+            }
+        }
+    }
+}
+
+template <int SK, int AMODE, int CHAIN = 0, bool LN = false>
+static int launch_gemm32(const GemmBatch &gb, int rmax, int nmax, hipStream_t st, int ysplit = 1)
 {
     const size_t lds = sizeof(float) * (SK * 4 * 32 * LDT + 32 + 64 * SK);
     if (lds > 64 * 1024)
         PTX_HIP(hipFuncSetAttribute(reinterpret_cast<const void *>(&k_gemm32<SK, AMODE, CHAIN, LN>),
                                     hipFuncAttributeMaxDynamicSharedMemorySize, (int)lds));
-    hipLaunchKernelGGL((k_gemm32<SK, AMODE, CHAIN, LN>), dim3(cdiv(rmax, 32), cdiv(nmax, 32), gb.n), dim3(SK * 64), lds, st, gb);
+    hipLaunchKernelGGL((k_gemm32<SK, AMODE, CHAIN, LN>), dim3(cdiv(rmax, 32), cdiv(nmax, 32) * ysplit, gb.n), dim3(SK * 64), lds, st, gb);
     return PTX_OK;
 }
 
@@ -792,7 +849,16 @@
         PTX_REQUIRE(gb.n == 1 && gb.p[0].pg == nullptr && gb.p[0].c2 && gb.p[0].n2 >= 1 && gb.p[0].chain_tiles >= 1 &&
                     gb.p[0].chain_tiles * 32 <= gb.p[0].N && gb.p[0].K >= 4 * BK && gb.p[0].lnp_out == nullptr && !any_ln,
                     "gemm: bad chained-product description");
-        PTX_TRY((launch_gemm32<4, 0, true>(gb, rmax, nmax, st)));
+        if (gb.p[0].ps0 != nullptr) {
+            const GemmProb &p = gb.p[0];
+            const int split = p.chain_split > 1 ? p.chain_split : 1;
+            PTX_REQUIRE(p.chain_tiles * 32 == p.N && p.lds0 >= 2 * p.chain_tiles && split <= 2 && p.n2 > p.K &&
+                        cdiv(p.n2, 32) >= split && (long)p.R * p.lda < (1l << 31),
+                        "gemm: bad token-0 description of the chained product");
+            PTX_TRY((launch_gemm32<4, 0, 2>(gb, rmax, nmax, st, split)));
+        } else {
+            PTX_TRY((launch_gemm32<4, 0, 1>(gb, rmax, nmax, st)));
+        }
         PTX_LAUNCHED("k_gemm");
         return PTX_OK;
     }
@@ -832,7 +898,15 @@
         return PTX_OK;
     }
     if (gb.p[0].pg != nullptr) {
-        PTX_TRY((launch_gemm32<4, 1>(gb, rmax, nmax, st)));
+        bool fold = gb.p[0].pfm != nullptr;
+        for (int g = 0; g < gb.n; ++g) {
+            const GemmProb &p = gb.p[g];
+            PTX_REQUIRE((p.pfm != nullptr) == fold && (!fold || (p.ps0 != nullptr && p.ldfm % 4 == 0 &&
+                                                                 (reinterpret_cast<uintptr_t>(p.pfm) & 15) == 0)),
+                        "gemm: bad token-0 description in pooled group %d", g);
+        }
+        if (fold) PTX_TRY((launch_gemm32<4, 2>(gb, rmax, nmax, st)));
+        else PTX_TRY((launch_gemm32<4, 1>(gb, rmax, nmax, st)));
     } else if (tiles32 >= g64_min) {
         const dim3 grid(cdiv(rmax, 64), cdiv(nmax, 64), gb.n);
         const int nkg = (kmin == kmax && kmin % 128 == 0) ? kmin / 128 : 0;
@@ -854,9 +928,9 @@
         int sk = 1;
         while (sk < 4 && tiles32 * sk < 4096 && nk >= 4 * sk) sk *= 2;
         if (any_ln) {
-            if (sk == 1) PTX_TRY((launch_gemm32<1, 0, false, true>(gb, rmax, nmax, st)));
-            else if (sk == 2) PTX_TRY((launch_gemm32<2, 0, false, true>(gb, rmax, nmax, st)));
-            else PTX_TRY((launch_gemm32<4, 0, false, true>(gb, rmax, nmax, st)));
+            if (sk == 1) PTX_TRY((launch_gemm32<1, 0, 0, true>(gb, rmax, nmax, st)));
+            else if (sk == 2) PTX_TRY((launch_gemm32<2, 0, 0, true>(gb, rmax, nmax, st)));
+            else PTX_TRY((launch_gemm32<4, 0, 0, true>(gb, rmax, nmax, st)));
         } else if (sk == 1) PTX_TRY((launch_gemm32<1, 0>(gb, rmax, nmax, st)));
         else if (sk == 2) PTX_TRY((launch_gemm32<2, 0>(gb, rmax, nmax, st)));
         else PTX_TRY((launch_gemm32<4, 0>(gb, rmax, nmax, st)));
diff --git a/proxytransformation_amd/csrc/imgpool.hip b/proxytransformation_amd/csrc/imgpool.hip
--- a/proxytransformation_amd/csrc/imgpool.hip
+++ b/proxytransformation_amd/csrc/imgpool.hip
@@ -125,7 +125,8 @@
         ev[u] = p < hw ? wim[(size_t)wid * a.KT1 + in_dim + 1 + p] : 0.0f;
     }
     float sq = 0.0f, sk = 0.0f;
-    if (T == 0) {
+    const bool own_s0 = T == 0 && a.qkv0 != nullptr;
+    if (own_s0) {
         const int hd = a.C / heads;
         const float *qv = a.qkv0 + (size_t)im * 3 * a.C + wid * hd;
         if (lane < hd) { sq = qv[lane]; sk = qv[a.C + lane]; }
@@ -202,12 +203,13 @@
         for (int u = 0; u < 2; ++u) e[u] = 128 * T + lane + 64 * u < hw ? expf(sv[u] - m) : 0.0f;
         const float l = wave_sum(e[0] + e[1]);
         float *erow = a.E + ((size_t)im * heads + h) * a.EW;
-        const float s0 = T == 0 ? wave_sum(sq * sk) * a.scale : 0.0f;
+        const float s0 = own_s0 ? wave_sum(sq * sk) * a.scale : 0.0f;
         if (lane == 0) {
             float *ml = a.ML + ((size_t)im * heads + h) * 5;
             ml[2 * T] = m;
             ml[2 * T + 1] = l;
-            if (T == 0) { ml[4] = s0; erow[0] = 1.0f; }
+            if (own_s0) ml[4] = s0;
+            if (T == 0) erow[0] = 1.0f;
         }
 #pragma unroll
         for (int u = 0; u < 2; ++u) {
diff --git a/proxytransformation_amd/csrc/imgpool32.hip b/proxytransformation_amd/csrc/imgpool32.hip
--- a/proxytransformation_amd/csrc/imgpool32.hip
+++ b/proxytransformation_amd/csrc/imgpool32.hip
@@ -49,7 +49,8 @@
         ev[t] = p < hw ? wim[(size_t)wid * a.KT1 + in_dim + 1 + p] : 0.0f;
     }
     float sq = 0.0f, sk = 0.0f;
-    if (H == 0) {
+    const bool own_s0 = H == 0 && a.qkv0 != nullptr;
+    if (own_s0) {
         const int hd = a.C / heads;
         const float *qv = a.qkv0 + (size_t)im * 3 * a.C + wid * hd;
         if (lane < hd) { sq = qv[lane]; sk = qv[a.C + lane]; }
@@ -146,11 +147,12 @@
                     const int tok = 1 + 128 * H + TP * u + lane;
                     if (lane < TP && tok < a.EW) erow[tok] = e_t[u];
                 }
-                const float s0 = H == 0 ? wave_sum(sq * sk) * a.scale : 0.0f;
+                const float s0 = own_s0 ? wave_sum(sq * sk) * a.scale : 0.0f;
                 if (lane == 0) {
                     float *ml = a.ML + ((size_t)im * heads + h) * 5;
                     ml[2 * H] = m_run; ml[2 * H + 1] = l_run;
-                    if (H == 0) { ml[4] = s0; erow[0] = 1.0f; }
+                    if (own_s0) ml[4] = s0;
+                    if (H == 0) erow[0] = 1.0f;
                 }
             }
         }
diff --git a/proxytransformation_amd/csrc/prep.hip b/proxytransformation_amd/csrc/prep.hip
--- a/proxytransformation_amd/csrc/prep.hip
+++ b/proxytransformation_amd/csrc/prep.hip
@@ -60,7 +60,7 @@
     float s = 0.0f;
     if (t < in_dim) {
         for (int j = 0; j < C; ++j) s = fmaf(wk[j], cw[(size_t)j * in_dim + t], s);
-    } else if (t > in_dim) {
+    } else {
         const float *pi = pos + (size_t)(t - in_dim) * C;
         for (int j = 0; j < C; ++j) s = fmaf(wk[j], cb[j] + pi[j], s);
     }
```

Result: slower. 17420 scenes/s (-5.2%).
